# taindp98/Endoscopy-Image-Classification

Hardware: AMD Instinct MI355X
Metric: unlabeled images/sec/node (FixMatch ViT-S, 224², μ=7) (higher is better)
Workload: dtype bf16; 1 GPU; F1: FixMatch ViT-S/16 step, global B=64 labeled + mu*B=448 unlabeled weak/strong pairs (64 + 448 per GPU, strong scaling), 224^2, C=23, tau=0.95, lambda_u=1, Adam 1e-3, EMA 0.999; global_batch=960, seq_len=197, parallelism=dp1, hipgraph=False

## Files before the change

endoscopy-image-classification_amd/csrc/attention.hip:

```cpp
#include <type_traits>

#include "common.h"

namespace {

struct AttnArgs {
  const bf16* qkv; bf16* o; float* lse; float* delta;
  const bf16* dout; bf16* dqkv;
  int ldqkv, ldo, lddo, lddqkv;
  int T, H;
  float scale;
};

__device__ __forceinline__ int aswz(int r, int c) { return c ^ (((r >> 1) & 3) << 1); }

template <int NW = 4>
__device__ __forceinline__ void stage_head(char* lds, const bf16* src, int ld, int T, int TP) {
  const int lane = threadIdx.x & 63, w = threadIdx.x >> 6;
  for (int i = w; i < TP / 8; i += NW) {
    const int row = i * 8 + (lane >> 3);
    const int sr = row < T ? row : T - 1;
    glds16(src + (size_t)sr * ld + aswz(row, lane & 7) * 8, lds + i * 1024);
  }
}
// ... 1276 lines not shown
      bf16x4 tk4[NDT];
#pragma unroll
      for (int dt = 0; dt < NDT; ++dt) tk4[dt] = lds_trT4(Ks, t * 16, (d0 + dt) * 16, g, r);
      const bf16x4 dsf = lds_trS4(img, t * 16, seg, half, g, r);
#pragma unroll
      for (int dt = 0; dt < NDT; ++dt) dq[dt] = mfma16k16(tk4[dt], dsf, dq[dt]);
    }
    const int img_i = bh / a.H, h = bh - img_i * a.H, q0 = tile * 16;
    bf16* dst = a.dqkv + ((size_t)img_i * T + q0) * a.lddqkv + h * 64 + d0 * 16;
    if constexpr (NDT == 4) tile_rows_out(slot, dq, a.scale, dst, a.lddqkv, T - q0);
    else half_rows_out(slot, dq, a.scale, dst, a.lddqkv, T - q0);
  };
  using Whole = std::integral_constant<int, 4>;
  using Half = std::integral_constant<int, 2>;

  int bh = blockIdx.x;
  stage_qdo(bh, 0, NG, 0, 8);
  stage_k(bh);
  Pre pre = prefetch(bh);
  const int nk = (NG - w + 7) / 8;
  for (;;) {
    const int img = bh / a.H, h = bh - img * a.H;
    const int nx = bh + gridDim.x;
    const bool more = nx < nbh;
    if (nk == 4) asm volatile("s_waitcnt vmcnt(4)" ::: "memory");
    else asm volatile("s_waitcnt vmcnt(3)" ::: "memory");
    lds_barrier();
    deltas(pre);
    __builtin_amdgcn_s_waitcnt(0x0F70);
    lds_barrier();
    f32x4 dk[2][4], dv[2][4];
#pragma unroll
    for (int t = 0; t < 2; ++t)
#pragma unroll
      for (int dt = 0; dt < 4; ++dt) dk[t][dt] = dv[t][dt] = f32x4{0.f, 0.f, 0.f, 0.f};
    bf16x8 kv[8];
    {
      const int l = fresh_lane(), g = l >> 4, r = l & 15;
#pragma unroll
      for (int t = 0; t < 2; ++t) {
        const int key = w * 32 + 16 * t + r;
        const bf16x8 k0 = lds_row8(Ks, key < TP ? key : 0, g), k1 = lds_row8(Ks, key < TP ? key : 0, 4 + g);
        kv[4 * t + 0] = key < T ? k0 : zero8;
        kv[4 * t + 1] = key < T ? k1 : zero8;
        kv[4 * t + 2] = pre.v[2 * t];
        kv[4 * t + 3] = pre.v[2 * t + 1];
      }
    }
    if (w < (NT16 + 1) / 2) phase1(kv, dk, dv, 0, PA, false, 0);
    lds_barrier();
    if (more) stage_qdo(nx, 0, PA * 32 / 8, 0, 8);
    phase2(Whole{}, bh, w, 0, 0);
    lds_barrier();
    if (w < (NT16 + 1) / 2) phase1(kv, dk, dv, PA, NP, true, 2 * PA * 16);
    lds_barrier();
    if (more) stage_qdo(nx, PA * 32 / 8, NG, 0, 8);
    pre = prefetch(more ? nx : bh);
    static_assert(2 * (NT16 - 2 * PA) == 10, "ten half tiles");
    if (w < 7) {
      phase2(Half{}, bh, 2 * PA + (w >> 1), w & 1, 2 * PA * 16);
    } else {
      phase2(Half{}, bh, 2 * PA + 3, 1, 2 * PA * 16);
      phase2(Half{}, bh, 2 * PA + 4, 0, 2 * PA * 16);
      phase2(Half{}, bh, 2 * PA + 4, 1, 2 * PA * 16);
    }
    if (w < (NT16 + 1) / 2) {
      bf16* d0 = a.dqkv + ((size_t)img * T + w * 32) * a.lddqkv + D + h * 64;
      tile_rows_out(slot, dk[0], a.scale, d0, a.lddqkv, T - w * 32);
      tile_rows_out(slot, dv[0], 1.0f, d0 + D, a.lddqkv, T - w * 32);
      tile_rows_out(slot, dk[1], a.scale, d0 + 16 * (size_t)a.lddqkv, a.lddqkv, T - w * 32 - 16);
      tile_rows_out(slot, dv[1], 1.0f, d0 + 16 * (size_t)a.lddqkv + D, a.lddqkv, T - w * 32 - 16);
    }
    lds_barrier();
    if (!more) break;
    stage_k(nx);
    bh = nx;
  }
}

constexpr int CLS_KMAX = 32;
constexpr int CLS_KMAX_LONG = 80;

__device__ __forceinline__ float grp8_sum(float v) {
  v += __shfl_xor(v, 1, 64);
  v += __shfl_xor(v, 2, 64);
  v += __shfl_xor(v, 4, 64);
  return v;
}

__device__ __forceinline__ void ld8f(const bf16* p, float* f) {
  const bf16x8 v = *(const bf16x8*)p;
#pragma unroll
  for (int i = 0; i < 8; ++i) f[i] = (float)v[i];
}

template <int KMAX>
__global__ __launch_bounds__(64) void attn_cls_fwd_kernel(const bf16* __restrict__ qkv, int ldqkv, bf16* __restrict__ o,
                                                          int ldo, float* __restrict__ lse, int T, int H, float scale) {
  const int bh = blockIdx.x, img = bh / H, h = bh - img * H, D = H * 64;
  const int lane = threadIdx.x, c = lane & 7, jg = lane >> 3;
  const bf16* base = qkv + (size_t)img * T * ldqkv;
  float q[8];
  ld8f(base + h * 64 + 8 * c, q);
  const float sl = scale * 1.44269504088896341f;
  float s[KMAX];
  float mx = -INFINITY;
#pragma unroll
  for (int it = 0; it < KMAX; ++it) {
    const int j = it * 8 + jg;
    float part = 0.f;
    if (j < T) {
      float k[8];
      ld8f(base + (size_t)j * ldqkv + D + h * 64 + 8 * c, k);
#pragma unroll
      for (int i = 0; i < 8; ++i) part = fmaf(q[i], k[i], part);
    }
    const float dot = grp8_sum(part);
    s[it] = j < T ? dot * sl : -INFINITY;
    mx = fmaxf(mx, s[it]);
  }
  mx = fmaxf(mx, __shfl_xor(mx, 8, 64));
  mx = fmaxf(mx, __shfl_xor(mx, 16, 64));
  mx = fmaxf(mx, __shfl_xor(mx, 32, 64));
  float l = 0.f, acc[8] = {0.f, 0.f, 0.f, 0.f, 0.f, 0.f, 0.f, 0.f};
#pragma unroll
  for (int it = 0; it < KMAX; ++it) {
    const int j = it * 8 + jg;
    if (j < T) {
      const float p = __builtin_amdgcn_exp2f(s[it] - mx);
      l += p;
      const float pb = (float)(bf16)p;
      float v[8];
      ld8f(base + (size_t)j * ldqkv + 2 * D + h * 64 + 8 * c, v);
#pragma unroll
      for (int i = 0; i < 8; ++i) acc[i] = fmaf(pb, v[i], acc[i]);
    }
  }
#pragma unroll
  for (int m = 8; m < 64; m <<= 1) {
    l += __shfl_xor(l, m, 64);
#pragma unroll
    for (int i = 0; i < 8; ++i) acc[i] += __shfl_xor(acc[i], m, 64);
  }
  if (jg == 0) {
    const float inv = 1.0f / l;
    bf16x8 ov;
#pragma unroll
    for (int i = 0; i < 8; ++i) ov[i] = (bf16)(acc[i] * inv);
    *(bf16x8*)(o + (size_t)img * ldo + h * 64 + 8 * c) = ov;
    if (c == 0) lse[bh] = (mx + __log2f(l)) * 0.69314718055994531f;
  }
}

template <int KMAX>
__global__ __launch_bounds__(64) void attn_cls_bwd_kernel(const bf16* __restrict__ qkv, int ldqkv,
                                                          const bf16* __restrict__ o, int ldo,
                                                          const float* __restrict__ lse,
                                                          const bf16* __restrict__ dout, int lddo,
                                                          bf16* __restrict__ dqkv, int lddqkv, int T, int H,
                                                          float scale) {
  const int bh = blockIdx.x, img = bh / H, h = bh - img * H, D = H * 64;
  const int lane = threadIdx.x, c = lane & 7, jg = lane >> 3;
  const bf16* base = qkv + (size_t)img * T * ldqkv;
  bf16* dbase = dqkv + (size_t)img * T * lddqkv;
  float q[8], dq_o[8], ov[8];
  ld8f(base + h * 64 + 8 * c, q);
  ld8f(dout + (size_t)img * lddo + h * 64 + 8 * c, dq_o);
  ld8f(o + (size_t)img * ldo + h * 64 + 8 * c, ov);
  float dpart = 0.f;
#pragma unroll
  for (int i = 0; i < 8; ++i) dpart += dq_o[i] * ov[i];
  const float delta = grp8_sum(dpart);
  const float sl = scale * 1.44269504088896341f;
  const float lq = lse[bh] * 1.44269504088896341f;
  float dqa[8] = {0.f, 0.f, 0.f, 0.f, 0.f, 0.f, 0.f, 0.f};
  const bf16x8 zero8 = {};
  for (int it = 0; it < KMAX; ++it) {
    const int j = it * 8 + jg;
    if (it * 8 >= T) break;
    float k[8], v[8];
    float sp = 0.f, dpp = 0.f;
    if (j < T) {
      ld8f(base + (size_t)j * ldqkv + D + h * 64 + 8 * c, k);
      ld8f(base + (size_t)j * ldqkv + 2 * D + h * 64 + 8 * c, v);
#pragma unroll
      for (int i = 0; i < 8; ++i) {
        sp = fmaf(q[i], k[i], sp);
        dpp = fmaf(dq_o[i], v[i], dpp);
      }
    }
    const float sv = grp8_sum(sp), dp = grp8_sum(dpp);
    if (j < T) {
      const float p = __builtin_amdgcn_exp2f(sv * sl - lq);
      const float ds = p * (dp - delta);
      const float pb = (float)(bf16)p, dsb = (float)(bf16)ds;
      bf16x8 dk8, dv8;
#pragma unroll
      for (int i = 0; i < 8; ++i) {
        dk8[i] = (bf16)(dsb * q[i] * scale);
        dv8[i] = (bf16)(pb * dq_o[i]);
        dqa[i] = fmaf(dsb, k[i], dqa[i]);
      }
      bf16* drow = dbase + (size_t)j * lddqkv + h * 64 + 8 * c;
      *(bf16x8*)(drow + D) = dk8;
      *(bf16x8*)(drow + 2 * D) = dv8;
      if (j > 0) *(bf16x8*)drow = zero8;
    }
  }
#pragma unroll
  for (int m = 8; m < 64; m <<= 1)
#pragma unroll
    for (int i = 0; i < 8; ++i) dqa[i] += __shfl_xor(dqa[i], m, 64);
  if (jg == 0) {
    bf16x8 d8;
#pragma unroll
    for (int i = 0; i < 8; ++i) d8[i] = (bf16)(dqa[i] * scale);
    *(bf16x8*)(dbase + h * 64 + 8 * c) = d8;
  }
}

#define ATTN_CASE(KERNEL, N_, GRID, LDS, STREAM, ARGS) \
  case N_: allow_lds(KERNEL<N_>, LDS); hipLaunchKernelGGL(KERNEL<N_>, GRID, 256, LDS, STREAM, ARGS); break;

#define ATTN_DISPATCH(KERNEL, NT16_, GRID, LDS, STREAM, ARGS)                                               \
  switch (NT16_) {                                                                                        \
    ATTN_CASE(KERNEL, 1, GRID, LDS, STREAM, ARGS) ATTN_CASE(KERNEL, 2, GRID, LDS, STREAM, ARGS)            \
    ATTN_CASE(KERNEL, 3, GRID, LDS, STREAM, ARGS) ATTN_CASE(KERNEL, 4, GRID, LDS, STREAM, ARGS)            \
    ATTN_CASE(KERNEL, 5, GRID, LDS, STREAM, ARGS) ATTN_CASE(KERNEL, 6, GRID, LDS, STREAM, ARGS)            \
    ATTN_CASE(KERNEL, 7, GRID, LDS, STREAM, ARGS) ATTN_CASE(KERNEL, 8, GRID, LDS, STREAM, ARGS)            \
    ATTN_CASE(KERNEL, 9, GRID, LDS, STREAM, ARGS) ATTN_CASE(KERNEL, 10, GRID, LDS, STREAM, ARGS)           \
    ATTN_CASE(KERNEL, 11, GRID, LDS, STREAM, ARGS) ATTN_CASE(KERNEL, 12, GRID, LDS, STREAM, ARGS)          \
    ATTN_CASE(KERNEL, 13, GRID, LDS, STREAM, ARGS) ATTN_CASE(KERNEL, 14, GRID, LDS, STREAM, ARGS)          \
    ATTN_CASE(KERNEL, 15, GRID, LDS, STREAM, ARGS) ATTN_CASE(KERNEL, 16, GRID, LDS, STREAM, ARGS)          \
    ATTN_CASE(KERNEL, 37, GRID, LDS, STREAM, ARGS)                                                        \
    default: return ES_BAD_SHAPE;                                                                         \
  }

#define FWD_CASE(N_, OCC_, GRID, LDS, STREAM, ARGS)                                                  \
  case N_:                                                                                          \
    allow_lds(attn_fwd_kernel<N_, OCC_>, LDS);                                                      \
    hipLaunchKernelGGL(HIP_KERNEL_NAME(attn_fwd_kernel<N_, OCC_>), GRID, 256, LDS, STREAM, ARGS);   \
    break;
#define FWD_DISPATCH(NT16_, OCC_, GRID, LDS, STREAM, ARGS)                                            \
  switch (NT16_) {                                                                                  \
    FWD_CASE(1, OCC_, GRID, LDS, STREAM, ARGS) FWD_CASE(2, OCC_, GRID, LDS, STREAM, ARGS)            \
    FWD_CASE(3, OCC_, GRID, LDS, STREAM, ARGS) FWD_CASE(4, OCC_, GRID, LDS, STREAM, ARGS)            \
    FWD_CASE(5, OCC_, GRID, LDS, STREAM, ARGS) FWD_CASE(6, OCC_, GRID, LDS, STREAM, ARGS)            \
    FWD_CASE(7, OCC_, GRID, LDS, STREAM, ARGS) FWD_CASE(8, OCC_, GRID, LDS, STREAM, ARGS)            \
    FWD_CASE(9, OCC_, GRID, LDS, STREAM, ARGS) FWD_CASE(10, OCC_, GRID, LDS, STREAM, ARGS)           \
    FWD_CASE(11, OCC_, GRID, LDS, STREAM, ARGS) FWD_CASE(12, OCC_, GRID, LDS, STREAM, ARGS)          \
    FWD_CASE(13, OCC_, GRID, LDS, STREAM, ARGS) FWD_CASE(14, OCC_, GRID, LDS, STREAM, ARGS)          \
    FWD_CASE(15, OCC_, GRID, LDS, STREAM, ARGS) FWD_CASE(16, OCC_, GRID, LDS, STREAM, ARGS)          \
    default: return ES_BAD_SHAPE;                                                                   \
  }

int g_attn_fwd_occ = 7;
int g_attn_bwd_pipe = 4;
int g_attn_bwd_long = 1;
int g_attn_bwd_grid = -1;

}

extern "C" {

int es_set_attn_variant(int occ) {
  const int old = g_attn_fwd_occ;
  g_attn_fwd_occ = occ;
  return old;
}

int es_set_attn_bwd_variant(int v) {
  if (v < 0 || v > 4) return ES_BAD_ARG;
  const int old = g_attn_bwd_pipe;
  g_attn_bwd_pipe = v;
  return old;
}

int es_set_attn_bwd_grid(int workgroups) {
  const int old = g_attn_bwd_grid;
  g_attn_bwd_grid = workgroups < -1 ? -1 : workgroups;
  return old;
}

int es_set_attn_bwd_long(int v) {
  const int old = g_attn_bwd_long;
  g_attn_bwd_long = v;
  return old;
}


static int attn_tiles(int T) { return T <= 256 ? (T + 15) / 16 : 37; }
constexpr int ATTN_TMAX = 592;

int es_attn_fwd(const void* qkv, int ldqkv, void* o, int ldo, float* lse, int nimg, int T, int H, float scale,
                hipStream_t stream) {
  if (nimg <= 0 || T <= 0 || T > ATTN_TMAX || H <= 0 || ldqkv < 3 * H * 64 || ldo < H * 64 || (ldqkv % 8) ||
      (ldo % 8))
    return ES_BAD_SHAPE;
  if (!qkv || !o || !lse) return ES_BAD_ARG;
  AttnArgs a{(const bf16*)qkv, (bf16*)o, lse, nullptr, nullptr, nullptr, ldqkv, ldo, 0, 0, T, H, scale};
  if (T > 256) {
    const size_t lds = 2 * (size_t)37 * 16 * 128 + 8 * 1024;
    allow_lds(attn_fwd_long_kernel<37>, lds);
    hipLaunchKernelGGL(HIP_KERNEL_NAME(attn_fwd_long_kernel<37>), nimg * H, 512, lds, stream, a);
    return hipGetLastError() == hipSuccess ? ES_OK : ES_HIP_ERROR;
  }
  const int nt16 = (T + 15) / 16;
  const size_t lds = 3 * (size_t)nt16 * 16 * 128;
  if (g_attn_fwd_occ == 7 && nt16 == 13) {
    allow_lds(attn_fwd_kernel<13, 2, 7>, lds);
    hipLaunchKernelGGL(HIP_KERNEL_NAME(attn_fwd_kernel<13, 2, 7>), nimg * H, 448, lds, stream, a);
  } else if (g_attn_fwd_occ == 2 || g_attn_fwd_occ == 7) {
    FWD_DISPATCH(nt16, 2, nimg * H, lds, stream, a);
  } else {
    FWD_DISPATCH(nt16, 3, nimg * H, lds, stream, a);
  }
  return hipGetLastError() == hipSuccess ? ES_OK : ES_HIP_ERROR;
}

int es_attn_bwd(const void* qkv, int ldqkv, const void* o, int ldo, const float* lse, float* delta, const void* dout,
                int lddo, void* dqkv, int lddqkv, int nimg, int T, int H, float scale, hipStream_t stream) {
  if (nimg <= 0 || T <= 0 || T > ATTN_TMAX || H <= 0 || ldqkv < 3 * H * 64 || lddqkv < 3 * H * 64 || (ldqkv % 8) ||
      (lddqkv % 8) || (ldo % 8) || (lddo % 8))
    return ES_BAD_SHAPE;
  if (!qkv || !o || !lse || !delta || !dout || !dqkv) return ES_BAD_ARG;
  AttnArgs a{(const bf16*)qkv, (bf16*)o, (float*)lse, delta, (const bf16*)dout, (bf16*)dqkv, ldqkv, ldo, lddo,
             lddqkv, T, H, scale};
  const int nt16 = attn_tiles(T);
  const size_t lds_dq = 2 * (size_t)nt16 * 16 * 128;
  const size_t lds_dkv = lds_dq + 2 * (size_t)nt16 * 16 * 4;
  const int nw_dq = nt16 == 37 ? 8 : 4, nw_dkv = nt16 == 37 ? 6 : 4;
  const size_t slots_dq = nw_dq * (nw_dq == 4 ? 2048 : 1024), slots_dkv = nw_dkv * (nt16 <= 16 ? 2048 : 1024);
#define BWD_VARIANTS(N_)                                                                                    \
  if (g_attn_bwd_pipe >= 3) {                                                                               \
    if (nw_dq == 8) {                                                                                       \
      allow_lds(attn_bwd_dq2_kernel<N_, 8>, lds_dq + slots_dq);                                             \
      hipLaunchKernelGGL(HIP_KERNEL_NAME(attn_bwd_dq2_kernel<N_, 8>), nimg * H, 512, lds_dq + slots_dq, stream, a); \
    } else {                                                                                                \
      allow_lds(attn_bwd_dq2_kernel<N_>, lds_dq + slots_dq);                                                \
      hipLaunchKernelGGL(HIP_KERNEL_NAME(attn_bwd_dq2_kernel<N_>), nimg * H, 256, lds_dq + slots_dq, stream, a); \
    }                                                                                                       \
  } else {                                                                                                  \
    allow_lds(attn_bwd_dq_pipe_kernel<N_>, lds_dq);                                                         \
    hipLaunchKernelGGL(HIP_KERNEL_NAME(attn_bwd_dq_pipe_kernel<N_>), nimg * H, 256, lds_dq, stream, a);     \
  }                                                                                                         \
  if (g_attn_bwd_pipe >= 2) {                                                                               \
    if (nw_dkv == 6) {                                                                                      \
      allow_lds(attn_bwd_dkv2_kernel<N_, false, 6>, lds_dkv + slots_dkv);                                   \
      hipLaunchKernelGGL(HIP_KERNEL_NAME(attn_bwd_dkv2_kernel<N_, false, 6>), nimg * H, 384, lds_dkv + slots_dkv, \
                         stream, a);                                                                        \
    } else {                                                                                                \
      allow_lds(attn_bwd_dkv2_kernel<N_>, lds_dkv + slots_dkv);                                             \
      hipLaunchKernelGGL(HIP_KERNEL_NAME(attn_bwd_dkv2_kernel<N_>), nimg * H, 256, lds_dkv + slots_dkv, stream, a); \
    }                                                                                                       \
  } else {                                                                                                  \
    allow_lds(attn_bwd_dkv_pipe_kernel<N_>, lds_dkv);                                                       \
    hipLaunchKernelGGL(HIP_KERNEL_NAME(attn_bwd_dkv_pipe_kernel<N_>), nimg * H, 256, lds_dkv, stream, a);   \
  }                                                                                                         \
  return hipGetLastError() == hipSuccess ? ES_OK : ES_HIP_ERROR;
  if (g_attn_bwd_pipe == 4 && nt16 == 13 &&
      (size_t)nimg * T * std::max(std::max(ldqkv, ldo), lddo) * 2 < ((size_t)1 << 31)) {
    static int cus = 0;
    if (!cus) {
      int dev = 0;
      (void)hipGetDevice(&dev);
      if (hipDeviceGetAttribute(&cus, hipDeviceAttributeMultiprocessorCount, dev) != hipSuccess || cus <= 0) cus = 256;
    }
    const size_t lds = 5 * (size_t)13 * 16 * 128 + 2 * 13 * 16 * 4 + 8 * 2048;
    allow_lds(attn_bwd_fused_kernel<13>, lds);
    const int heads = nimg * H;
    const int grid = std::min(g_attn_bwd_grid > 0 ? g_attn_bwd_grid
                                                  : (g_attn_bwd_grid == 0 ? cus : std::max(cus, (heads + 3) / 4)),
                              heads);
    hipLaunchKernelGGL(HIP_KERNEL_NAME(attn_bwd_fused_kernel<13>), grid, 512, lds, stream, a, nimg * H);
    return hipGetLastError() == hipSuccess ? ES_OK : ES_HIP_ERROR;
  }
  if (g_attn_bwd_pipe && nt16 == 13) { BWD_VARIANTS(13) }
  if (g_attn_bwd_pipe && nt16 == 37 && g_attn_bwd_long) { BWD_VARIANTS(37) }
#undef BWD_VARIANTS
  ATTN_DISPATCH(attn_bwd_dq_kernel, nt16, nimg * H, lds_dq, stream, a);
  ATTN_DISPATCH(attn_bwd_dkv_kernel, nt16, nimg * H, lds_dkv, stream, a);
  return hipGetLastError() == hipSuccess ? ES_OK : ES_HIP_ERROR;
}


int es_attn_cls_fwd(const void* qkv, int ldqkv, void* o, int ldo, float* lse, int nimg, int T, int H, float scale,
                    hipStream_t stream) {
  if (nimg <= 0 || T <= 0 || T > 8 * CLS_KMAX_LONG || H <= 0 || ldqkv < 3 * H * 64 || ldo < H * 64 || (ldqkv % 8) ||
      (ldo % 8))
    return ES_BAD_SHAPE;
  if (!qkv || !o || !lse) return ES_BAD_ARG;
  if (T <= 8 * CLS_KMAX)
    hipLaunchKernelGGL(HIP_KERNEL_NAME(attn_cls_fwd_kernel<CLS_KMAX>), nimg * H, 64, 0, stream, (const bf16*)qkv, ldqkv,
                       (bf16*)o, ldo, lse, T, H, scale);
  else
    hipLaunchKernelGGL(HIP_KERNEL_NAME(attn_cls_fwd_kernel<CLS_KMAX_LONG>), nimg * H, 64, 0, stream, (const bf16*)qkv,
                       ldqkv, (bf16*)o, ldo, lse, T, H, scale);
  return hipGetLastError() == hipSuccess ? ES_OK : ES_HIP_ERROR;
}

int es_attn_cls_bwd(const void* qkv, int ldqkv, const void* o, int ldo, const float* lse, const void* dout, int lddo,
                    void* dqkv, int lddqkv, int nimg, int T, int H, float scale, hipStream_t stream) {
  if (nimg <= 0 || T <= 0 || T > 8 * CLS_KMAX_LONG || H <= 0 || ldqkv < 3 * H * 64 || lddqkv < 3 * H * 64 ||
      ldo < H * 64 || lddo < H * 64 || (ldqkv % 8) || (lddqkv % 8) || (ldo % 8) || (lddo % 8))
    return ES_BAD_SHAPE;
  if (!qkv || !o || !lse || !dout || !dqkv) return ES_BAD_ARG;
  if (T <= 8 * CLS_KMAX)
    hipLaunchKernelGGL(HIP_KERNEL_NAME(attn_cls_bwd_kernel<CLS_KMAX>), nimg * H, 64, 0, stream, (const bf16*)qkv, ldqkv,
                       (const bf16*)o, ldo, lse, (const bf16*)dout, lddo, (bf16*)dqkv, lddqkv, T, H, scale);
  else
    hipLaunchKernelGGL(HIP_KERNEL_NAME(attn_cls_bwd_kernel<CLS_KMAX_LONG>), nimg * H, 64, 0, stream, (const bf16*)qkv,
                       ldqkv, (const bf16*)o, ldo, lse, (const bf16*)dout, lddo, (bf16*)dqkv, lddqkv, T, H, scale);
  return hipGetLastError() == hipSuccess ? ES_OK : ES_HIP_ERROR;
}

}
```

endoscopy-image-classification_amd/csrc/gemm.hip:

```cpp
#include <algorithm>
#include <mutex>
#include <type_traits>

#include <hip/hip_ext.h>

#include "common.h"

namespace es_gemm {

constexpr int BM = 128, BN = 128, BK = 64;

enum Epi {
  EPI_BF16 = 0,
  EPI_GELU = 1,
  EPI_F32_RESID = 2,
  EPI_DGELU = 3,
  EPI_F32 = 4,
  EPI_PATCH = 5,
  EPI_GELU_ACT = 6,
  EPI_GELU_D = 7,
  EPI_MULAUX = 8,
};

struct NTArgs {
// ... 1400 lines not shown
        for (int j = 0; j < 3; ++j) {
          const int cc = (j * 64 + lane) >> 1;
          const float2 t = *(const float2*)(smem + lr * ROWX + ((cc ^ (lr & 15)) << 4) + (lane & 1) * 8);
          const float2 rr = rv[2 * s + q / (RPS / 2)][q % (RPS / 2)][j];
          v[j] = make_float2(t.x + rr.x, t.y + rr.y);
        }
        if constexpr (s == 0)
          if (q == RPS / 2 - 1) load_resid(std::integral_constant<int, 3>{});
        const LnRow384 o = ln_row384(v, (q & 1) == 0, l.eps, gam_lds, bet_lds, lane);
        const int m = m0 + tile_row(s, q);
        const bool ok = m < p.M;
#pragma unroll
        for (int j = 0; j < 3; ++j) {
          const int c = (j * 64 + lane) * 2;
          __builtin_amdgcn_raw_buffer_store_b64(__builtin_bit_cast(u32x2, v[j]), rx,
                                                ok ? (unsigned)(m * p.ldc + c) * 4u : ES_OOB, 0, 0);
          __builtin_amdgcn_raw_buffer_store_b32(o.h[j], rh, ok ? (unsigned)(m * l.ldh + c) * 2u : ES_OOB, 0, 0);
        }
        const bool one = ok && lane == 0;
        __builtin_amdgcn_raw_buffer_store_b32(__builtin_bit_cast(unsigned, o.mean), rm,
                                              one ? (unsigned)m * 4u : ES_OOB, 0, 0);
        __builtin_amdgcn_raw_buffer_store_b32(__builtin_bit_cast(unsigned, o.rstd), rs,
                                              one ? (unsigned)m * 4u : ES_OOB, 0, 0);
      }
    };
    slab(std::integral_constant<int, 0>{});
    asm volatile("s_waitcnt lgkmcnt(0)" ::: "memory");
    __builtin_amdgcn_s_barrier();
    slab(std::integral_constant<int, 1>{});
    if (tid == 0) qslot[0] = claimed;
    asm volatile("s_waitcnt lgkmcnt(0)" ::: "memory");
    __builtin_amdgcn_s_barrier();
    cur = __builtin_amdgcn_readfirstlane(qslot[0]);
  }
  TILE_CTR_RELEASE(ctr, tid)
}
#undef TILE_CTR_RELEASE

#define NT_LAUNCH(E, BKT_, NST_, TBM_, ...)                                             \
  {                                                                                        \
    const size_t lds = std::max((size_t)NST_ * (TBM_ + BN) * BKT_ * 2, (size_t)4 * EPI_WAVE_BYTES); \
    allow_lds(gemm_nt_kernel<E, BKT_, NST_, TBM_, ##__VA_ARGS__>, lds);                   \
    hipLaunchKernelGGL(HIP_KERNEL_NAME(gemm_nt_kernel<E, BKT_, NST_, TBM_, ##__VA_ARGS__>), dim3(grid), dim3(256), lds, stream, a); \
    return ES_OK;                                                                          \
  }
#define NT_EPIS(BKT_, NST_, TBM_, ...)                                            \
  switch (epi) {                                                                  \
    case EPI_BF16: NT_LAUNCH(EPI_BF16, BKT_, NST_, TBM_, ##__VA_ARGS__)           \
    case EPI_GELU: NT_LAUNCH(EPI_GELU, BKT_, NST_, TBM_, ##__VA_ARGS__)           \
    case EPI_F32_RESID: NT_LAUNCH(EPI_F32_RESID, BKT_, NST_, TBM_, ##__VA_ARGS__) \
    case EPI_DGELU: NT_LAUNCH(EPI_DGELU, BKT_, NST_, TBM_, ##__VA_ARGS__)         \
    case EPI_F32: NT_LAUNCH(EPI_F32, BKT_, NST_, TBM_, ##__VA_ARGS__)             \
    case EPI_PATCH: NT_LAUNCH(EPI_PATCH, BKT_, NST_, TBM_, ##__VA_ARGS__)         \
    case EPI_GELU_ACT: NT_LAUNCH(EPI_GELU_ACT, BKT_, NST_, TBM_, ##__VA_ARGS__)   \
    case EPI_GELU_D: NT_LAUNCH(EPI_GELU_D, BKT_, NST_, TBM_, ##__VA_ARGS__)       \
    case EPI_MULAUX: NT_LAUNCH(EPI_MULAUX, BKT_, NST_, TBM_, ##__VA_ARGS__)       \
    default: return ES_BAD_ARG;                                                   \
  }
int launch_nt(int cfg, int epi, int grid, hipStream_t stream, const NTArgs& a) {
  if (cfg == 11 && epi == EPI_F32_RESID) NT_LAUNCH(EPI_F32_RESID, 64, 2, 64, 0)
  switch (cfg) {
    case 0: NT_EPIS(64, 2, 128)
    case 5: NT_EPIS(32, 2, 128)
    case 11: NT_EPIS(64, 2, 64)
    default: NT_EPIS(32, 3, 128)
  }
}
#undef NT_EPIS
#undef NT_LAUNCH

#define BIG_LAUNCH(E, WM_, MF_, NF_, NST_, BKT_, OCC_, ...)                                        \
  {                                                                                                 \
    const size_t lds = (size_t)NST_ * (WM_ * MF_ * 16 + (8 / WM_) * NF_ * 16) * BKT_ * 2;            \
    allow_lds(gemm_nt_big_kernel<E, WM_, MF_, NF_, NST_, BKT_, OCC_, ##__VA_ARGS__>, lds);          \
    hipLaunchKernelGGL(HIP_KERNEL_NAME(gemm_nt_big_kernel<E, WM_, MF_, NF_, NST_, BKT_, OCC_, ##__VA_ARGS__>), dim3(grid), \
                       dim3(512), lds, stream, a);                                                  \
    return hipGetLastError() == hipSuccess ? ES_OK : ES_HIP_ERROR;                                  \
  }
#define BIG_EPIS2(WM_, MF_, NF_, NST_, BKT_, OCC_)                                        \
  switch (epi) {                                                                          \
    case EPI_BF16: BIG_LAUNCH(EPI_BF16, WM_, MF_, NF_, NST_, BKT_, OCC_)                  \
    case EPI_GELU: BIG_LAUNCH(EPI_GELU, WM_, MF_, NF_, NST_, BKT_, OCC_)                  \
    case EPI_F32_RESID: BIG_LAUNCH(EPI_F32_RESID, WM_, MF_, NF_, NST_, BKT_, OCC_)        \
    case EPI_DGELU: BIG_LAUNCH(EPI_DGELU, WM_, MF_, NF_, NST_, BKT_, OCC_)                \
    case EPI_F32: BIG_LAUNCH(EPI_F32, WM_, MF_, NF_, NST_, BKT_, OCC_)                    \
    case EPI_PATCH: BIG_LAUNCH(EPI_PATCH, WM_, MF_, NF_, NST_, BKT_, OCC_)                \
    case EPI_GELU_ACT: BIG_LAUNCH(EPI_GELU_ACT, WM_, MF_, NF_, NST_, BKT_, OCC_)          \
    case EPI_GELU_D: BIG_LAUNCH(EPI_GELU_D, WM_, MF_, NF_, NST_, BKT_, OCC_)              \
    case EPI_MULAUX: BIG_LAUNCH(EPI_MULAUX, WM_, MF_, NF_, NST_, BKT_, OCC_)              \
    default: return ES_BAD_ARG;                                                           \
  }
#define BIG_EPIS(WM_, MF_, NF_, NST_, BKT_) BIG_EPIS2(WM_, MF_, NF_, NST_, BKT_, 1)
int launch_big(int cfg, int epi, int grid, hipStream_t stream, const NTArgs& a) {
  if (cfg == 10 && epi == EPI_F32_RESID) BIG_LAUNCH(EPI_F32_RESID, 4, 4, 4, 3, 32, 4, 0)
  switch (cfg) {
    case 10: BIG_EPIS2(4, 4, 4, 3, 32, 4)
    default: BIG_EPIS(2, 8, 4, 2, 64)
  }
}
#undef BIG_EPIS
#undef BIG_EPIS2
#undef BIG_LAUNCH

static int tile_ctr_slot(hipStream_t s) {
  static std::mutex mu;
  static hipStream_t tab[CTR_SLOTS];
  static int n = 0;
  std::lock_guard<std::mutex> lock(mu);
  for (int i = 0; i < n; ++i)
    if (tab[i] == s) return i;
  if (n < CTR_SLOTS) {
    tab[n] = s;
    return n++;
  }
  return (int)(((uintptr_t)s >> 6) % CTR_SLOTS);
}
static int persistent_grid(int tiles) {
  static const int cus = [] {
    int dev = 0, n = 0;
    (void)hipGetDevice(&dev);
    return (hipDeviceGetAttribute(&n, hipDeviceAttributeMultiprocessorCount, dev) != hipSuccess || n <= 0) ? 256 : n;
  }();
  return std::max(1, std::min(cus, tiles));
}

int launch_resid_ln(hipStream_t stream, const NTArgs& a, const RLArgs& l) {
  const int grid = persistent_grid((a.M + rlg::R - 1) / rlg::R);
  allow_lds(gemm_resid_ln_kernel, (size_t)rlg::LDS);
  hipLaunchKernelGGL(gemm_resid_ln_kernel, dim3(grid), dim3(512), rlg::LDS, stream, a, l, tile_ctr_slot(stream));
  return hipGetLastError() == hipSuccess ? ES_OK : ES_HIP_ERROR;
}

int launch_nt_ln(int ring, hipStream_t stream, const NTArgs& a, const RLArgs& l) {
  const int grid = persistent_grid((a.M + nlg::TBM - 1) / nlg::TBM);
  const int slot = tile_ctr_slot(stream);
  constexpr size_t lds3 = nlg::lds<3, 32>(), lds2 = nlg::lds<2, 64>();
  if (ring == 1) {
    allow_lds(gemm_nt_ln_kernel<3, 32>, lds3);
    hipLaunchKernelGGL(HIP_KERNEL_NAME(gemm_nt_ln_kernel<3, 32>), dim3(grid), dim3(512), lds3, stream, a, l, slot);
  } else {
    allow_lds(gemm_nt_ln_kernel<2, 64>, lds2);
    hipLaunchKernelGGL(HIP_KERNEL_NAME(gemm_nt_ln_kernel<2, 64>), dim3(grid), dim3(512), lds2, stream, a, l, slot);
  }
  return hipGetLastError() == hipSuccess ? ES_OK : ES_HIP_ERROR;
}

}
using namespace es_gemm;

static int g_gemm_variant = -1;
static int g_tn_variant = -1;
static int g_small_tile = 1;

extern "C" {

int es_gemm_tn_ex(const void* A1, int ld1, const void* A2, int ld2, int M, int N1, int N2, int splits,
                  float* workspace, float* out, int accumulate, float* bias_out, int variant, hipStream_t stream);

int es_gemm_nt(int epi, const void* A, int lda, const void* B, int ldb, const float* bias, void* C,
               int ldc, void* C2, const void* aux, int ldaux, int M, int N, int K, int np,
               hipStream_t stream) {
  if (M <= 0 || N <= 0 || K <= 0 || (N % BN) || (K % BK) || (lda % 8) || (ldb % 8) || (ldc % 4))
    return ES_BAD_SHAPE;
  if (!A || !B || !C) return ES_BAD_ARG;
  if (((epi == EPI_GELU || epi == EPI_GELU_D) && !C2) ||
      ((epi == EPI_F32_RESID || epi == EPI_DGELU || epi == EPI_MULAUX || epi == EPI_PATCH) && !aux))
    return ES_BAD_ARG;
  if (epi == EPI_PATCH && np <= 0) return ES_BAD_ARG;
  if ((epi == EPI_F32_RESID || epi == EPI_PATCH) && ((ldaux % 4) || ldaux < N)) return ES_BAD_SHAPE;
  if ((epi == EPI_DGELU || epi == EPI_MULAUX) && ((ldaux % 8) || ldaux < N)) return ES_BAD_SHAPE;
  NTArgs a{(const bf16*)A, (const bf16*)B, bias, C, C2, aux, M, N, K, lda, ldb, ldc, ldaux, np};
  int variant = g_gemm_variant;
  if (variant < 0) {
    const bool gelu = epi == EPI_GELU || epi == EPI_GELU_ACT || epi == EPI_GELU_D;
    const bool plain = epi == EPI_BF16 || epi == EPI_F32 || epi == EPI_F32_RESID || epi == EPI_MULAUX;
    if (g_small_tile && N <= 384 && ((K <= 384 && epi == EPI_F32_RESID) || (M < 32768 && (plain || epi == EPI_GELU_ACT))))
      variant = 11;
    else if (g_small_tile && M < 32768 && epi == EPI_GELU_ACT)
      variant = 11;
    else if (M >= 65536 && K >= 768 && N == 384 && epi == EPI_BF16)
      variant = 0;
    else if ((plain || epi == EPI_GELU_D) && M >= 65536 && ((K <= 384 && N >= 384) || (K >= 768 && N == 384)))
      variant = 10;
    else if (K <= 384 && N % 256 == 0 && epi == EPI_MULAUX)
      variant = M < 65536 ? 0 : 6;
    else if (K >= 768 && N % 256 == 0 && epi != EPI_DGELU)
      variant = 6;
    else if (epi == EPI_PATCH)
      variant = 0;
    else if (gelu)
      variant = K <= 384 ? 5 : 1;
    else if (K <= 384)
      variant = (epi == EPI_F32_RESID || N <= 384 || M < 65536) ? 0 : (epi == EPI_DGELU ? 2 : 5);
    else
      variant = M < 65536 ? 0 : 1;
  }
  if (variant == 1) {
    const int grid = ((M + BM2 - 1) / BM2) * (N / BN);
    const size_t lds = 3 * STAGE2;
#define L2(E) allow_lds(gemm_nt256_kernel<E>, lds); hipLaunchKernelGGL(gemm_nt256_kernel<E>, grid, 512, lds, stream, a); break;
    switch (epi) {
      case EPI_BF16: L2(EPI_BF16)
      case EPI_GELU: L2(EPI_GELU)
      case EPI_F32_RESID: L2(EPI_F32_RESID)
      case EPI_DGELU: L2(EPI_DGELU)
      case EPI_F32: L2(EPI_F32)
      case EPI_PATCH: L2(EPI_PATCH)
      case EPI_GELU_ACT: L2(EPI_GELU_ACT)
      case EPI_GELU_D: L2(EPI_GELU_D)
      case EPI_MULAUX: L2(EPI_MULAUX)
      default: return ES_BAD_ARG;
    }
#undef L2
    return hipGetLastError() == hipSuccess ? ES_OK : ES_HIP_ERROR;
  }
  if (variant == 6 || variant == 10) {
    const int tbn = variant == 6 ? 256 : 128;
    if (N % tbn) return ES_BAD_SHAPE;
    return launch_big(variant, epi, ((M + 255) / 256) * (N / tbn), stream, a);
  }
  if (variant != 0 && variant != 2 && variant != 5 && variant != 11) return ES_BAD_ARG;
  const int tbm = variant == 11 ? 64 : BM;
  const int grid = ((M + tbm - 1) / tbm) * (N / BN);
  const int rc = launch_nt(variant, epi, grid, stream, a);
  if (rc) return rc;
  return hipGetLastError() == hipSuccess ? ES_OK : ES_HIP_ERROR;
}

int es_gemm_nt_resid_ln(const void* A, int lda, const void* B, int ldb, const float* bias, float* C, int ldc,
                        const float* aux, int ldaux, const float* gamma, const float* beta, void* h, int ldh,
                        float* mean, float* rstd, int M, int N, int K, float eps, hipStream_t stream) {
  if (M <= 0 || N != rlg::D || K != rlg::KD || (lda % 8) || (ldb % 8) || (ldc % 2) || (ldaux % 4) || (ldh % 2) ||
      (size_t)M * (size_t)std::max(ldc, ldaux) * 4 >= (1u << 31))
    return ES_BAD_SHAPE;
  if (!A || !B || !C || !aux || !gamma || !beta || !h || !mean || !rstd) return ES_BAD_ARG;
  if ((((uintptr_t)A | (uintptr_t)aux | (uintptr_t)B | (uintptr_t)gamma | (uintptr_t)beta) & 15) ||
      (bias && ((uintptr_t)bias & 15)) || ((uintptr_t)C & 7) || ((uintptr_t)h & 3))
    return ES_BAD_ARG;
  NTArgs a{(const bf16*)A, (const bf16*)B, bias, C, nullptr, aux, M, N, K, lda, ldb, ldc, ldaux, 0};
  RLArgs l{gamma, beta, (bf16*)h, mean, rstd, ldh, eps};
  return launch_resid_ln(stream, a, l);
}

static int g_nt_ln_ring = 0;
int es_gemm_nt_ln(const void* A, int lda, const void* B, int ldb, const float* bias, float* C, int ldc,
                  const float* aux, int ldaux, const float* gamma, const float* beta, void* h, int ldh, float* mean,
                  float* rstd, int M, int N, int K, float eps, hipStream_t stream) {
  if (M <= 0 || N != nlg::D || K <= 0 || (K % 64) || (lda % 8) || (ldb % 8) || (ldc % 2) || (ldaux % 2) || (ldh % 2) ||
      lda < K || ldb < K || ldc < N || ldaux < N || ldh < N ||
      (size_t)M * (size_t)std::max(std::max(ldc, ldaux), ldh) * 4 >= (1u << 31))
    return ES_BAD_SHAPE;
  if (!A || !B || !C || !aux || !gamma || !beta || !h || !mean || !rstd) return ES_BAD_ARG;
  if ((((uintptr_t)A | (uintptr_t)B | (uintptr_t)gamma | (uintptr_t)beta) & 15) || (bias && ((uintptr_t)bias & 15)) ||
      (((uintptr_t)C | (uintptr_t)aux) & 7) || (((uintptr_t)h | (uintptr_t)mean | (uintptr_t)rstd) & 3))
    return ES_BAD_ARG;
  NTArgs a{(const bf16*)A, (const bf16*)B, bias, C, nullptr, aux, M, N, K, lda, ldb, ldc, ldaux, 0};
  RLArgs l{gamma, beta, (bf16*)h, mean, rstd, ldh, eps};
  return launch_nt_ln(g_nt_ln_ring, stream, a, l);
}
int endossl_nt_ln_ring(int v) {
  const int old = g_nt_ln_ring;
  g_nt_ln_ring = v == 1 ? 1 : 0;
  return old;
}

static bool gemm_variant_ok(int v) {
  return v == -1 || v == 0 || v == 1 || v == 2 || v == 5 || v == 6 || v == 10 || v == 11;
}
int es_set_gemm_variant(int v) {
  if (!gemm_variant_ok(v)) return ES_BAD_ARG;
  const int old = g_gemm_variant;
  g_gemm_variant = v;
  return old;
}

int es_set_gemm_small_tile(int v) {
  const int old = g_small_tile;
  g_small_tile = v;
  return old;
}

int es_set_tn_variant(int v) {
  if (v != -1 && v != 0 && v != 7) return ES_BAD_ARG;
  const int old = g_tn_variant;
  g_tn_variant = v;
  return old;
}

constexpr int TN_MIN_SPLIT_TOKENS = 512;
static bool tn_big_ok(int N1, int N2, int ld1, int ld2) {
  return N1 % TB1 == 0 && N2 % TB2 == 0 && ld1 % 8 == 0 && ld2 % 8 == 0;
}
static int tn_pick(int M, int N1, int N2, int ld1, int ld2, int v) {
  if (!(N1 % BM == 0 && N2 % BN == 0)) return 7;
  if (v == 7) return tn_big_ok(N1, N2, ld1, ld2) ? 7 : 0;
  if (v >= 0) return 0;
  return (tn_big_ok(N1, N2, ld1, ld2) && M >= 65536) ? 7 : 0;
}
static int tn_target(int v) { return v == 7 ? 256 : 768; }
static int tn_tiles(int v, int N1, int N2) { return v == 7 ? (N1 / TB1) * (N2 / TB2) : (N1 / BM) * (N2 / BN); }
static int tn_auto_splits(int v, int M, int N1, int N2) {
  const int by_fill = std::max(1, tn_target(v) / tn_tiles(v, N1, N2));
  const int by_len = std::max(1, M / TN_MIN_SPLIT_TOKENS);
  return std::min(by_fill, by_len);
}

size_t es_gemm_tn_workspace(int N1, int N2, int splits) {
  if (splits <= 0) {
    splits = std::max(1, 768 / std::max(1, (N1 / BM) * (N2 / BN)));
    if (N1 % TB1 == 0 && N2 % TB2 == 0) splits = std::max(splits, 512 / std::max(1, (N1 / TB1) * (N2 / TB2)));
  }
  return (size_t)splits * N1 * N2 + (size_t)splits * N1;
}

int es_gemm_tn(const void* A1, int ld1, const void* A2, int ld2, int M, int N1, int N2, int splits,
               float* workspace, float* out, int accumulate, float* bias_out, hipStream_t stream) {
  return es_gemm_tn_ex(A1, ld1, A2, ld2, M, N1, N2, splits, workspace, out, accumulate, bias_out, -1, stream);
}

int es_gemm_tn_ex(const void* A1, int ld1, const void* A2, int ld2, int M, int N1, int N2, int splits,
                  float* workspace, float* out, int accumulate, float* bias_out, int variant, hipStream_t stream) {
  if (M <= 0 || (ld1 % 8) || (ld2 % 8)) return ES_BAD_SHAPE;
  if (!tn_big_ok(N1, N2, ld1, ld2) && ((N1 % BM) || (N2 % BN))) return ES_BAD_SHAPE;
  if (!A1 || !A2 || !out || !workspace) return ES_BAD_ARG;
  if (variant != -1 && variant != 0 && variant != 7) return ES_BAD_ARG;
  const int v = tn_pick(M, N1, N2, ld1, ld2, g_tn_variant >= 0 ? g_tn_variant : variant);
  const int BKM = v == 7 ? 64 : 32;
  const int msteps = (M + BKM - 1) / BKM;
  if (splits <= 0) splits = tn_auto_splits(v, M, N1, N2);
  splits = std::min(splits, msteps);
  const int per = (msteps + splits - 1) / splits;
  const int S = (msteps + per - 1) / per;
  const bool direct = (S == 1 && !accumulate);
  float* P = direct ? out : workspace;
  float* PB = bias_out ? workspace + (size_t)S * N1 * N2 : nullptr;
  TNArgs a{(const bf16*)A1, (const bf16*)A2, P, PB, M, N1, N2, ld1, ld2, per * BKM};
  const int grid = S * tn_tiles(v, N1, N2);
#define TN_LAUNCH(BKM_, NST_)                                                                           \
  {                                                                                                   \
    const size_t lds = (size_t)NST_ * 2 * BKM_ * BM * 2;                                              \
    allow_lds(gemm_tn_kernel<BKM_, NST_>, lds);                                                       \
    hipLaunchKernelGGL(HIP_KERNEL_NAME(gemm_tn_kernel<BKM_, NST_>), dim3(grid), dim3(256), lds, stream, a); \
  }
#define TNB_LAUNCH(BKM_, NST_)                                                                          \
  {                                                                                                   \
    const size_t lds = (size_t)NST_ * BKM_ * (TB1 + TB2) * 2;                                         \
    allow_lds(gemm_tn_big_kernel<BKM_, NST_>, lds);                                                   \
    hipLaunchKernelGGL(HIP_KERNEL_NAME(gemm_tn_big_kernel<BKM_, NST_>), dim3(grid), dim3(512), lds, stream, a); \
  }
  switch (v) {
    case 7: TNB_LAUNCH(64, 2) break;
    default: TN_LAUNCH(32, 2) break;
  }
#undef TN_LAUNCH
#undef TNB_LAUNCH
  if (!direct) {
    const int n = N1 * N2;
    int rg = (n / 4 + 255) / 256;
    rg = rg > 2048 ? 2048 : rg;
    hipLaunchKernelGGL(splitk_reduce_kernel, rg, 256, 0, stream, P, out, S, n, accumulate);
  }
  if (bias_out)
    launch_reduce_partials(PB, bias_out, S, N1, accumulate, stream);
  return hipGetLastError() == hipSuccess ? ES_OK : ES_HIP_ERROR;
}

static_assert(sizeof(TNGroupEntry) == 64, "es_tn_problem layout");
size_t es_tn_problem_size(void) { return sizeof(TNGroupEntry); }

int es_gemm_tn_grouped_prepare(void* host_table, int count) {
  if (!host_table || count <= 0) return ES_BAD_ARG;
  TNGroupEntry* t = (TNGroupEntry*)host_table;
  int tiles = 0;
  for (int i = 0; i < count; ++i) {
    TNArgs& a = t[i].a;
    if (!a.A1 || !a.A2 || !a.P) return ES_BAD_ARG;
    if (a.M <= 0 || a.N1 % BM || a.N2 % BN || a.ld1 % 8 || a.ld2 % 8) return ES_BAD_SHAPE;
    a.mchunk = (a.M + 31) / 32 * 32;
    t[i].tile0 = tiles;
// ... 178 lines not shown
```

endoscopy-image-classification_amd/csrc/losses.hip:

```cpp
#include "common.h"

namespace {

constexpr int MAXC = 64;

__device__ __forceinline__ float block_sum(float v, float* red) {
  v = warp_sum(v);
  const int lane = threadIdx.x & 63, w = threadIdx.x >> 6;
  __syncthreads();
  if (lane == 0) red[w] = v;
  __syncthreads();
  float s = 0.f;
  for (int i = 0; i < (int)(blockDim.x >> 6); ++i) s += red[i];
  return s;
}

__global__ __launch_bounds__(256) void fm_consistency_kernel(const float* __restrict__ lw, int ldw,
                                                             const float* __restrict__ ls, int lds_, int n, int C,
                                                             float tau, float grad_scale, int* __restrict__ pl,
                                                             uint8_t* __restrict__ mask_out,
                                                             float* __restrict__ row_loss, float* __restrict__ dls,
                                                             int lddls, float* __restrict__ out) {
  __shared__ float red[16];
  float sum_loss = 0.f, sum_mask = 0.f;
  for (int i = threadIdx.x; i < n; i += blockDim.x) {
    const float* wr = lw + (size_t)i * ldw;
    const float* sr = ls + (size_t)i * lds_;
    float mx = -INFINITY;
    for (int c = 0; c < C; ++c) mx = fmaxf(mx, wr[c]);
    float se = 0.f;
    for (int c = 0; c < C; ++c) se += __expf(wr[c] - mx);
    const float inv = 1.0f / se;
    float pmax = -1.f;
    int idx = 0;
    for (int c = 0; c < C; ++c) {
      const float p = __expf(wr[c] - mx) * inv;
      if (p > pmax) {
        pmax = p;
        idx = c;
      }
    }
    const float m = pmax >= tau ? 1.f : 0.f;
    float mxs = -INFINITY;
    for (int c = 0; c < C; ++c) mxs = fmaxf(mxs, sr[c]);
    float ses = 0.f;
    for (int c = 0; c < C; ++c) ses += __expf(sr[c] - mxs);
    const float lse = mxs + __logf(ses);
    const float ce = lse - sr[idx];
    const float rl = ce * m;
    const float invs = 1.0f / ses;
    for (int c = 0; c < C; ++c) {
      const float p = __expf(sr[c] - mxs) * invs;
      dls[(size_t)i * lddls + c] = m * (p - (c == idx ? 1.f : 0.f)) * grad_scale;
    }
    if (pl) pl[i] = idx;
    if (mask_out) mask_out[i] = (uint8_t)m;
    if (row_loss) row_loss[i] = rl;
    sum_loss += rl;
    sum_mask += m;
  }
  sum_loss = block_sum(sum_loss, red);
  sum_mask = block_sum(sum_mask, red);
  if (threadIdx.x == 0) {
    out[0] = sum_loss / (float)n;
    out[1] = sum_mask / (float)n;
  }
}

__global__ __launch_bounds__(256) void poly_ce_kernel(const float* __restrict__ l, int ldl,
                                                      const int64_t* __restrict__ y, const float* __restrict__ w,
                                                      int n, int C, float eps, float grad_scale,
                                                      float* __restrict__ dl, int lddl, float* __restrict__ out) {
  __shared__ float red[16];
  float sum = 0.f;
  for (int i = threadIdx.x; i < n; i += blockDim.x) {
    const float* lr = l + (size_t)i * ldl;
    float mx = -INFINITY;
    for (int c = 0; c < C; ++c) mx = fmaxf(mx, lr[c]);
    float se = 0.f;
    for (int c = 0; c < C; ++c) se += __expf(lr[c] - mx);
    const float lse = mx + __logf(se);
    const int yi = (int)y[i];
    if ((unsigned)yi >= (unsigned)C) {
      sum += __int_as_float(0x7fc00000);
      for (int c = 0; c < C; ++c) dl[(size_t)i * lddl + c] = 0.f;
      continue;
    }
    const float wy = w ? w[yi] : 1.f;
    const float py = __expf(lr[yi] - lse);
    sum += wy * (lse - lr[yi]) + eps * (1.f - py);
    const float coef = grad_scale * (wy + eps * py);
    for (int c = 0; c < C; ++c) {
      const float p = __expf(lr[c] - lse);
      dl[(size_t)i * lddl + c] = coef * (p - (c == yi ? 1.f : 0.f));
    }
  }
  sum = block_sum(sum, red);
  if (threadIdx.x == 0) out[0] = sum / (float)n;
}

__global__ __launch_bounds__(256) void ce_weighted_kernel(const float* __restrict__ l, int ldl,
                                                          const int64_t* __restrict__ y, const float* __restrict__ w,
                                                          const float* __restrict__ wsum_global, int n, int C,
                                                          float grad_scale, float* __restrict__ dl, int lddl,
                                                          float* __restrict__ out) {
  __shared__ float red[16];
  float ws = 0.f;
  for (int i = threadIdx.x; i < n; i += blockDim.x) {
    const int yi = (int)y[i];
    ws += (unsigned)yi >= (unsigned)C ? __int_as_float(0x7fc00000) : (w ? w[yi] : 1.f);
  }
  float W = block_sum(ws, red);
  __syncthreads();
  if (wsum_global) W = *wsum_global;
  const float invW = 1.0f / W;
  float sum = 0.f;
  for (int i = threadIdx.x; i < n; i += blockDim.x) {
    const float* lr = l + (size_t)i * ldl;
    float mx = -INFINITY;
    for (int c = 0; c < C; ++c) mx = fmaxf(mx, lr[c]);
    float se = 0.f;
    for (int c = 0; c < C; ++c) se += __expf(lr[c] - mx);
    const float lse = mx + __logf(se);
    const int yi = (int)y[i];
    if ((unsigned)yi >= (unsigned)C) {
      for (int c = 0; c < C; ++c) dl[(size_t)i * lddl + c] = 0.f;
      continue;
    }
    const float wy = w ? w[yi] : 1.f;
    sum += wy * (lse - lr[yi]);
    const float coef = grad_scale * wy * invW;
    for (int c = 0; c < C; ++c) {
      const float p = __expf(lr[c] - lse);
      dl[(size_t)i * lddl + c] = coef * (p - (c == yi ? 1.f : 0.f));
    }
  }
  sum = block_sum(sum, red);
  if (threadIdx.x == 0) out[0] = sum * invW;
}

__global__ __launch_bounds__(256) void ce_weight_sum_kernel(const int64_t* __restrict__ y, const float* __restrict__ w,
                                                            int n, int C, float* __restrict__ out) {
  __shared__ float red[16];
  float ws = 0.f;
  for (int i = threadIdx.x; i < n; i += blockDim.x) {
    const int yi = (int)y[i];
    ws += (unsigned)yi >= (unsigned)C ? __int_as_float(0x7fc00000) : (w ? w[yi] : 1.f);
  }
  ws = block_sum(ws, red);
  if (threadIdx.x == 0) out[0] = ws;
}

constexpr int TRIPLET_THREADS = 1024;

__global__ __launch_bounds__(TRIPLET_THREADS) void triplet_kernel(const float* __restrict__ z, int ldz, int bs, int L,
                                                                  float alpha, float grad_scale,
                                                                  float* __restrict__ dz, int lddz,
                                                                  float* __restrict__ out) {
  __shared__ float red[16];
  const int lane = threadIdx.x & 63, w = threadIdx.x >> 6, nw = blockDim.x >> 6;
  float s_h = 0.f, s_p = 0.f, s_n = 0.f, s_act = 0.f;
  for (int i = w; i < bs; i += nw) {
    const float* za = z + (size_t)i * ldz;
    const float* zp = z + (size_t)(bs + i) * ldz;
    const float* zn = z + (size_t)(2 * bs + i) * ldz;
    float sp = 0.f, sn = 0.f;
    for (int k = lane; k < L; k += 64) {
      const float a = za[k], ep = a - zp[k], en = a - zn[k];
      sp = fmaf(ep, ep, sp);
      sn = fmaf(en, en, sn);
    }
    const float dp = sqrtf(warp_sum(sp)), dn = sqrtf(warp_sum(sn));
    const float h = dp - dn + alpha;
    const bool act = h > 0.f;
    s_h += act ? h : 0.f;
    s_p += dp;
    s_n += dn;
    s_act += act ? 1.f : 0.f;
    const float cp = act && dp > 0.f ? grad_scale / dp : 0.f;
    const float cn = act && dn > 0.f ? grad_scale / dn : 0.f;
    float* ga = dz + (size_t)i * lddz;
    float* gp = dz + (size_t)(bs + i) * lddz;
    float* gn = dz + (size_t)(2 * bs + i) * lddz;
    for (int k = lane; k < L; k += 64) {
      const float a = za[k], up = (a - zp[k]) * cp, un = (a - zn[k]) * cn;
      ga[k] = up - un;
      gp[k] = -up;
      gn[k] = un;
    }
  }
  const float inv = 1.0f / (float)bs;
  s_h = block_sum(lane == 0 ? s_h : 0.f, red);
  s_p = block_sum(lane == 0 ? s_p : 0.f, red);
  s_n = block_sum(lane == 0 ? s_n : 0.f, red);
  s_act = block_sum(lane == 0 ? s_act : 0.f, red);
  if (threadIdx.x == 0) {
    out[0] = s_h * inv;
    out[1] = s_p * inv;
    out[2] = s_n * inv;
    out[3] = s_act * inv;
  }
}

__global__ __launch_bounds__(256) void softmax_predict_kernel(const float* __restrict__ l, int ldl, int n, int C,
                                                              float thres, int* __restrict__ pred,
                                                              float* __restrict__ conf, int* __restrict__ label) {
  const int stride = gridDim.x * blockDim.x;
  for (int i = blockIdx.x * blockDim.x + threadIdx.x; i < n; i += stride) {
    const float* lr = l + (size_t)i * ldl;
    float mx = lr[0];
    int idx = 0;
    for (int c = 1; c < C; ++c) {
      const float v = lr[c];
      if (v > mx) {
        mx = v;
        idx = c;
      }
    }
    float se = 0.f;
    for (int c = 0; c < C; ++c) se += __expf(lr[c] - mx);
    const float p = 1.0f / se;
    if (pred) pred[i] = idx;
    if (conf) conf[i] = p;
    if (label) label[i] = p > thres ? idx : 0;
  }
}

constexpr int MARGIN_THREADS = 256;
constexpr int MARGIN_MAXF = 2048;
enum { MARGIN_COSFACE = 0, MARGIN_ARCFACE = 1, MARGIN_SPHEREFACE = 2, MARGIN_ACLOSS = 3 };

struct MarginParams {
  int kind;
  float s, m, eps, lo, hi;
  float cos_m, sin_m;
  float sig1, inv_k;
  float grad_scale;
};

__device__ __forceinline__ void margin_numerator(const MarginParams& P, float t, float& num, float& dnum) {
  if (P.kind == MARGIN_COSFACE) {
    num = P.s * (t - P.m);
    dnum = P.s;
    return;
  }
  const bool inside = t >= P.lo && t <= P.hi;
  const float tc = fminf(fmaxf(t, P.lo), P.hi);
  const float om = inside ? 1.0f - tc : (t > P.hi ? P.eps : 2.0f - P.eps);
  const float op = inside ? 1.0f + tc : (t > P.hi ? 2.0f - P.eps : P.eps);
  const float sq = sqrtf(om * op);
  float d;
// ... 26 lines not shown
  for (int k = tid; k < F4; k += MARGIN_THREADS) {
    const f32x4 v = xr[k];
    ss += v[0] * v[0] + v[1] * v[1] + v[2] * v[2] + v[3] * v[3];
  }
  const float nrm = sqrtf(block_sum(ss, red));
  const float inv = 1.0f / fmaxf(nrm, 1e-12f);
  for (int k = tid; k < F4; k += MARGIN_THREADS) ((f32x4*)xs)[k] = xr[k] * inv;
  __syncthreads();
  for (int c = w; c < C; c += MARGIN_THREADS / 64) {
    const f32x4* wr = (const f32x4*)(W + (size_t)c * F);
    float acc = 0.f;
    for (int k = lane; k < F4; k += 64) {
      const f32x4 a = ((const f32x4*)xs)[k], q = wr[k];
      acc = fmaf(a[0], q[0], acc);
      acc = fmaf(a[1], q[1], acc);
      acc = fmaf(a[2], q[2], acc);
      acc = fmaf(a[3], q[3], acc);
    }
    acc = warp_sum(acc);
    if (lane == 0) zs[c] = acc + (b ? b[c] : 0.f);
  }
  __syncthreads();
  if (w == 0) {
    const int64_t y64 = y[i];
    const bool valid = y64 >= 0 && y64 < C;
    const int yi = valid ? (int)y64 : -1;
    const float wm = (valid && cw ? cw[yi] : 1.f) * (mask ? mask[i] : 1.f);
    float num = 0.f, dnum = 0.f;
    margin_numerator(P, zs[valid ? yi : 0], num, dnum);
    const bool tgt = lane == yi;
    const float v = lane < C ? (tgt ? num : P.s * zs[lane]) : -INFINITY;
    const float mx = warp_max(v);
    const float e = lane < C ? expf(v - mx) : 0.f;
    const float se = warp_sum(e);
    const float rest = warp_sum(tgt ? 0.f : e);
    const float lse = mx + logf(se);
    const float coef = P.grad_scale * wm;
    float g = tgt ? -coef * (rest / se) * dnum : coef * P.s * (e / se);
    float rl = wm * (lse - num);
    if (!valid) {
      g = 0.f;
      rl = __int_as_float(0x7fc00000);
    }
    if (lane < C) {
      gs[lane] = g;
      G[(size_t)i * C + lane] = g;
    }
    if (lane == 0) {
      inv_norm[i] = inv;
      ws_loss[i] = rl;
      if (row_loss) row_loss[i] = rl;
    }
  }
  __syncthreads();
  f32x4 acc[2];
  float dot = 0.f;
#pragma unroll
  for (int j = 0; j < 2; ++j) {
    const int k = tid + j * MARGIN_THREADS;
    acc[j] = f32x4{0.f, 0.f, 0.f, 0.f};
    if (k < F4) {
      for (int c = 0; c < C; ++c) acc[j] += ((const f32x4*)(W + (size_t)c * F))[k] * gs[c];
      const f32x4 a = ((const f32x4*)xs)[k];
      dot += a[0] * acc[j][0] + a[1] * acc[j][1] + a[2] * acc[j][2] + a[3] * acc[j][3];
    }
  }
  dot = block_sum(dot, red);
  const float proj = nrm >= 1e-12f ? dot : 0.f;
  f32x4* dr = (f32x4*)(dx + (size_t)i * lddx);
#pragma unroll
  for (int j = 0; j < 2; ++j) {
    const int k = tid + j * MARGIN_THREADS;
    if (k < F4) dr[k] = (acc[j] - ((const f32x4*)xs)[k] * proj) * inv;
  }
}

__global__ __launch_bounds__(64) void margin_reduce_kernel(const float* __restrict__ x, int ldx,
                                                           const float* __restrict__ G,
                                                           const float* __restrict__ inv_norm,
                                                           const float* __restrict__ ws_loss, int n, int F, int C,
                                                           float grad_scale, float* __restrict__ dW,
                                                           float* __restrict__ db, float* __restrict__ out) {
  const int c = blockIdx.y, lane = threadIdx.x;
  const int F4 = F >> 2, k = blockIdx.x * 64 + lane;
  if (k < F4) {
    f32x4 acc = f32x4{0.f, 0.f, 0.f, 0.f};
#pragma unroll 4
    for (int i = 0; i < n; ++i)
      acc += ((const f32x4*)(x + (size_t)i * ldx))[k] * (G[(size_t)i * C + c] * inv_norm[i]);
    ((f32x4*)(dW + (size_t)c * F))[k] = acc;
  }
  if (blockIdx.x == 0) {
    if (db) {
      float sb = 0.f;
      for (int i = lane; i < n; i += 64) sb += G[(size_t)i * C + c];
      sb = warp_sum(sb);
      if (lane == 0) db[c] = sb;
    }
    if (c == 0) {
      float sl = 0.f;
      for (int i = lane; i < n; i += 64) sl += ws_loss[i];
      sl = warp_sum(sl);
      if (lane == 0) out[0] = grad_scale * sl;
    }
  }
}

}

extern "C" {

int es_ce_weighted_fwd_bwd(const float* logits, int ldl, const int64_t* targets, const float* weights, int n, int C,
                           float grad_scale, float* dlogits, int lddl, float* out, hipStream_t stream) {
  if (n <= 0 || C <= 0) return ES_BAD_SHAPE;
  if (!logits || !targets || !dlogits || !out) return ES_BAD_ARG;
  hipLaunchKernelGGL(ce_weighted_kernel, 1, 256, 0, stream, logits, ldl, targets, weights, nullptr, n, C, grad_scale,
                     dlogits, lddl, out);
  return hipGetLastError() == hipSuccess ? ES_OK : ES_HIP_ERROR;
}

int es_ce_weight_sum(const int64_t* targets, const float* weights, int n, int C, float* out, hipStream_t stream) {
  if (n <= 0 || C <= 0) return ES_BAD_SHAPE;
  if (!targets || !out) return ES_BAD_ARG;
  hipLaunchKernelGGL(ce_weight_sum_kernel, 1, 256, 0, stream, targets, weights, n, C, out);
  return hipGetLastError() == hipSuccess ? ES_OK : ES_HIP_ERROR;
}

int es_ce_weighted_fwd_bwd_global(const float* logits, int ldl, const int64_t* targets, const float* weights,
                                  const float* wsum_global, int n, int C, float grad_scale, float* dlogits, int lddl,
                                  float* out, hipStream_t stream) {
  if (n <= 0 || C <= 0) return ES_BAD_SHAPE;
  if (!logits || !targets || !dlogits || !out || !wsum_global) return ES_BAD_ARG;
  hipLaunchKernelGGL(ce_weighted_kernel, 1, 256, 0, stream, logits, ldl, targets, weights, wsum_global, n, C,
                     grad_scale, dlogits, lddl, out);
  return hipGetLastError() == hipSuccess ? ES_OK : ES_HIP_ERROR;
}

int es_fm_consistency_fwd_bwd(const float* logits_w, int ldw, const float* logits_s, int lds, int n, int C,
                              float tau, float grad_scale, int* pseudo_label, uint8_t* mask, float* row_loss,
                              float* dlogits_s, int lddls, float* out, hipStream_t stream) {
  if (n <= 0 || C <= 0 || C > MAXC) return ES_BAD_SHAPE;
  if (!logits_w || !logits_s || !dlogits_s || !out) return ES_BAD_ARG;
  hipLaunchKernelGGL(fm_consistency_kernel, 1, 256, 0, stream, logits_w, ldw, logits_s, lds, n, C, tau, grad_scale,
                     pseudo_label, mask, row_loss, dlogits_s, lddls, out);
  return hipGetLastError() == hipSuccess ? ES_OK : ES_HIP_ERROR;
}

int es_poly_ce_fwd_bwd(const float* logits, int ldl, const int64_t* targets, const float* weights, int n, int C,
                       float epsilon, float grad_scale, float* dlogits, int lddl, float* out, hipStream_t stream) {
  if (n <= 0 || C <= 0 || C > MAXC) return ES_BAD_SHAPE;
  if (!logits || !targets || !dlogits || !out) return ES_BAD_ARG;
  hipLaunchKernelGGL(poly_ce_kernel, 1, 256, 0, stream, logits, ldl, targets, weights, n, C, epsilon, grad_scale,
                     dlogits, lddl, out);
  return hipGetLastError() == hipSuccess ? ES_OK : ES_HIP_ERROR;
}

int es_triplet_fwd_bwd(const float* z, int ldz, int bs, int L, float alpha, float grad_scale, float* dz, int lddz,
                       float* out, hipStream_t stream) {
  if (bs < 1 || bs > 0x7fffffff / 3 || L < 1 || L > 2048 || ldz < L || lddz < L) return ES_BAD_SHAPE;
  if (!z || !dz || !out) return ES_BAD_ARG;
  hipLaunchKernelGGL(triplet_kernel, 1, TRIPLET_THREADS, 0, stream, z, ldz, bs, L, alpha, grad_scale, dz, lddz, out);
  return hipGetLastError() == hipSuccess ? ES_OK : ES_HIP_ERROR;
}

size_t es_margin_softmax_workspace(int n, int C) {
  if (n < 1 || C < 1 || C > MAXC) return 0;
  return (size_t)n * (size_t)(C + 2);
}

int es_margin_softmax_fwd_bwd(const float* x, int ldx, const float* W, const float* bias, const int64_t* targets,
                              const float* class_weights, const float* mask, int n, int F, int C, int kind, float s,
                              float m, float eps, float grad_scale, float* dx, int lddx, float* dW, float* db,
                              float* out, float* row_loss, float* workspace, hipStream_t stream) {
  if (n < 1 || C < 1 || C > MAXC || F < 4 || F > MARGIN_MAXF || (F & 3) || ldx < F || lddx < F || (ldx & 3) ||
      (lddx & 3))
    return ES_BAD_ARG;
  if (kind < MARGIN_COSFACE || kind > MARGIN_ACLOSS || !(eps > 0.f && eps < 1.f)) return ES_BAD_ARG;
  if (!x || !W || !targets || !dx || !dW || !out || !workspace) return ES_BAD_ARG;
  if (((uintptr_t)x | (uintptr_t)W | (uintptr_t)dx | (uintptr_t)dW) & 15) return ES_BAD_ARG;
  if (((uintptr_t)workspace | (uintptr_t)out) & 3) return ES_BAD_ARG;
  const double k = 0.3, q = exp(-M_PI / 2.0 / k);
  MarginParams P;
  P.kind = kind;
  P.s = s;
  P.m = m;
  P.eps = eps;
  P.lo = (float)(-1.0 + (double)eps);
  P.hi = (float)(1.0 - (double)eps);
  P.cos_m = (float)cos((double)m);
  P.sin_m = (float)sin((double)m);
  P.sig1 = (float)((1.0 + q) / (1.0 - q));
  P.inv_k = (float)(1.0 / k);
  P.grad_scale = grad_scale;
  float* G = workspace;
  float* inv_norm = G + (size_t)n * C;
  float* ws_loss = inv_norm + n;
  hipLaunchKernelGGL(margin_rows_kernel, n, MARGIN_THREADS, 0, stream, x, ldx, W, bias, targets, class_weights, mask,
                     F, C, P, dx, lddx, G, inv_norm, ws_loss, row_loss);
  hipLaunchKernelGGL(margin_reduce_kernel, dim3((F / 4 + 63) / 64, C), 64, 0, stream, x, ldx, G, inv_norm, ws_loss, n,
                     F, C, grad_scale, dW, db, out);
  return hipGetLastError() == hipSuccess ? ES_OK : ES_HIP_ERROR;
}

int es_softmax_predict(const float* logits, int ldl, int n, int C, float thres, int* pred, float* conf, int* label,
                       hipStream_t stream) {
  if (n <= 0 || C <= 0 || C > MAXC || ldl < C) return ES_BAD_SHAPE;
  if (!logits || (!pred && !conf && !label)) return ES_BAD_ARG;
  const int blocks = (n + 255) / 256 < 1024 ? (n + 255) / 256 : 1024;
  hipLaunchKernelGGL(softmax_predict_kernel, blocks, 256, 0, stream, logits, ldl, n, C, thres, pred, conf, label);
  return hipGetLastError() == hipSuccess ? ES_OK : ES_HIP_ERROR;
}

}
```

endoscopy-image-classification_amd/endossl/_lib.py:

```python
import ctypes
import os

import torch

_HERE = os.path.dirname(os.path.abspath(__file__))
LIB_PATH = os.environ.get("ENDOSSL_LIB", os.path.join(_HERE, "lib", "libendossl_hip.so"))

V, I, L, F, Z = ctypes.c_void_p, ctypes.c_int, ctypes.c_long, ctypes.c_float, ctypes.c_size_t
U64 = ctypes.c_ulonglong

SIGNATURES = {
    "es_abi_version": (I, []),
    "es_gemm_nt": (I, [I, V, I, V, I, V, V, I, V, V, I, I, I, I, I, V]),
    "es_gemm_nt_resid_ln": (I, [V, I, V, I, V, V, I, V, I, V, V, V, I, V, V, I, I, I, F, V]),
    "es_gemm_nt_ln": (I, [V, I, V, I, V, V, I, V, I, V, V, V, I, V, V, I, I, I, F, V]),
    "es_set_gemm_variant": (I, [I]),
    "es_set_gemm_small_tile": (I, [I]),
    "es_gemm_tn_workspace": (Z, [I, I, I]),
    "es_gemm_tn": (I, [V, I, V, I, I, I, I, I, V, V, I, V, V]),
    "es_gemm_tn_ex": (I, [V, I, V, I, I, I, I, I, V, V, I, V, I, V]),
    "es_set_tn_variant": (I, [I]),
    "es_set_attn_variant": (I, [I]),
    "es_set_attn_bwd_variant": (I, [I]),
    "es_set_attn_bwd_grid": (I, [I]),
    "es_set_ln_fwd_grid": (I, [I]),
    "es_set_attn_bwd_long": (I, [I]),
    "es_splitk_reduce": (I, [V, V, I, I, I, V]),
    "es_tn_problem_size": (Z, []),
    "es_gemm_tn_grouped_prepare": (I, [V, I]),
    "es_gemm_tn_grouped": (I, [V, I, I, V]),
    "es_set_stem_kernels": (I, [I]),
    "es_gemm_tn_big_grouped_table_bytes": (Z, [I]),
    "es_gemm_tn_big_grouped_workspace": (Z, [V, I, I]),
    "es_gemm_tn_big_grouped_prepare": (I, [V, I, I, V, Z, V, V]),
    "es_gemm_tn_big_grouped": (I, [V, I, V, V]),
    "es_gemm_tn_big_grouped_timed": (I, [V, I, V, V, V, V]),
    "es_event_create": (I, [V]),
    "es_event_elapsed": (I, [V, V, V]),
    "es_event_destroy": (I, [V]),
    "es_colsum": (I, [V, I, I, I, V, I, V, I, V]),
    "es_attn_fwd": (I, [V, I, V, I, V, I, I, I, F, V]),
    "es_attn_bwd": (I, [V, I, V, I, V, V, V, I, V, I, I, I, I, F, V]),
    "es_attn_cls_fwd": (I, [V, I, V, I, V, I, I, I, F, V]),
    "es_attn_cls_bwd": (I, [V, I, V, I, V, V, I, V, I, I, I, I, F, V]),
    "es_reduce_partials": (I, [V, V, I, I, I, V]),
    "es_layernorm_fwd": (I, [V, I, V, V, V, I, V, V, I, I, F, V]),
    "es_layernorm_bwd": (I, [V, I, V, I, V, V, V, V, I, V, I, V, I, V, V, V, I, I, I, I, V]),
    "es_layernorm_bwd_b16": (I, [V, I, V, I, V, V, V, V, I, V, I, V, I, V, V, V, I, I, I, I, V]),
    "es_layernorm_bwd_grid": (I, [I, I]),
    "es_ln_param_grads_entry_size": (I, []),
    "es_ln_param_grads_multi": (I, [V, I, V]),
    "es_gelu_fwd": (I, [V, V, L, V]),
    "es_gelu_bwd": (I, [V, V, V, L, V]),
    "es_patch_im2col": (I, [V, V, I, I, I, V]),
    "es_patch_im2col_u8": (I, [V, F, F, F, F, F, F, V, I, I, I, V]),
    "es_cls_init": (I, [V, I, V, V, I, I, I, V]),
    "es_embed_bwd": (I, [V, I, V, I, V, V, I, I, I, I, V]),
    "es_cls_head_fwd": (I, [V, I, I, V, V, V, V, V, I, V, V, I, I, I, F, V]),
    "es_cls_head_bwd": (I, [V, I, V, V, V, V, V, V, V, I, I, V, V, V, V, I, I, I, V]),
    "es_cls_head_bwd_ex": (I, [V, I, V, V, V, V, V, V, V, I, I, V, V, V, V, I, I, I, I, V]),
    "es_cls_ln_fwd": (I, [V, I, I, V, V, V, I, V, V, I, I, F, V]),
    "es_cls_ln_bwd": (I, [V, I, V, V, V, V, I, I, V, V, I, I, V]),
    "es_dense_fwd": (I, [V, I, V, V, V, I, I, I, I, I, F, V, F, V]),
    "es_dense_bwd_workspace": (Z, [I, I]),
    "es_dense_bwd": (I, [V, I, V, I, I, F, V, F, V, I, V, V, I, I, V, V, I, I, I, V, V]),
    "es_bn1d_fwd": (I, [V, I, V, V, V, V, V, F, F, I, V, I, V, V, I, I, V]),
    "es_bn1d_bwd": (I, [V, I, V, V, V, V, I, V, V, I, I, V]),
    "es_dropout_keep": (I, [V, L, F, U64, U64, V]),
    "es_bn1d_sums": (I, [V, I, I, I, V, F, V, V]),
    "es_bn1d_fwd_global": (I, [V, I, V, V, V, V, F, V, V, V, F, F, V, I, V, V, I, I, V]),
    "es_bn1d_bwd_sums": (I, [V, I, V, I, I, V, V]),
    "es_bn1d_bwd_global": (I, [V, I, V, V, V, V, V, F, V, I, V, V, I, I, V]),
    "es_l2norm_fwd": (I, [V, I, V, I, V, I, I, V]),
    "es_l2norm_bwd": (I, [V, I, V, I, V, V, I, I, I, V]),
    "es_comatch_pseudo_workspace": (Z, [I, I, I]),
    "es_comatch_pseudo": (I, [V, I, I, I, V, I, I, I, V, I, I, V, V, I, F, F, F, V, V, V, V, V, V]),
    "es_comatch_pseudo_ex": (I, [V, I, I, I, V, I, I, I, I, V, I, I, V, V, I, F, F, F, V, V, V, V, V, V]),
    "es_softmax_colmean": (I, [V, I, I, I, V, V]),
    "es_comatch_bank_write": (I, [V, I, I, V, I, I, I, V, V, I, V, V, I, I, V]),
    "es_comatch_contrastive_workspace": (Z, [I]),
    "es_comatch_contrastive_fwd_bwd": (I, [V, I, V, I, V, I, I, I, F, F, F, V, V, I, V, I, V, V]),
    "es_comatch_contrastive_ex_workspace": (Z, [I, I]),
    "es_comatch_contrastive_fwd_bwd_ex": (I, [V, I, V, I, V, V, I, I, I, I, I, F, F, F, F, V, V, I, V, I, V, V]),
    "es_comatch_focal_fwd_bwd": (I, [V, I, V, V, I, I, F, F, V, V, I, V, V]),
    "es_fm_consistency_fwd_bwd": (I, [V, I, V, I, I, I, F, F, V, V, V, V, I, V, V]),
    "es_poly_ce_fwd_bwd": (I, [V, I, V, V, I, I, F, F, V, I, V, V]),
    "es_triplet_fwd_bwd": (I, [V, I, I, I, F, F, V, I, V, V]),
    "es_softmax_predict": (I, [V, I, I, I, F, V, V, V, V]),
    "es_margin_softmax_workspace": (Z, [I, I]),
    "es_margin_softmax_fwd_bwd": (I, [V, I, V, V, V, V, V, I, I, I, I, F, F, F, F, V, I, V, V, V, V, V, V]),
    "es_ezbm_sample_mix": (I, [V, I, V, I, I, I, V, V, V, V, U64, U64, V, V, I, V, I, V, V, V, V, V, V]),
    "es_bn1d_groups_fwd": (I, [V, I, V, V, V, V, V, F, F, V, I, V, V, I, I, I, V]),
    "es_bn1d_groups_bwd": (I, [V, I, V, V, V, V, I, V, V, I, I, I, V]),
    "es_ezbm_ce_fwd_bwd": (I, [V, I, V, V, I, I, F, F, V, I, V, V]),
    "es_conv2d_fwd": (I, [V, I, I, I, I, L, L, L, L, V, V, I, I, I, I, I, V, L, L, L, I, V]),
    "es_conv2d_bwd_data": (I, [V, L, L, L, V, I, I, I, I, I, I, I, I, I, V, L, L, L, L, I, V]),
    "es_conv2d_dw_tiles": (I, [I, I, I, I]),
    "es_conv2d_bwd_weight_workspace": (Z, [I, I, I, I, I]),
    "es_conv2d_bwd_weight": (I, [V, I, I, I, I, L, L, L, L, V, L, L, L, I, I, I, I, I, I, V, V, I, V]),
    "es_conv2d_bf16_eligible": (I, [I, I, I, I]),
    "es_set_conv_dw_target": (I, [I]),
    "es_conv2d_pack_bf16": (I, [V, I, I, I, I, V, V, V]),
    "es_conv_pack_entry_size": (I, []),
    "es_set_conv_ring": (I, [I]),
    "es_set_conv_dw_buf": (I, [I]),
    "es_set_conv_small": (I, [I]),
    "es_conv2d_pack_bf16_multi": (I, [V, I, L, V]),
    "es_conv2d_fwd_bf16": (I, [V, I, I, I, I, L, L, L, L, V, V, I, I, I, I, I, V, L, L, L, I, V]),
    "es_conv2d_bwd_data_bf16": (I, [V, L, L, L, V, I, I, I, I, I, I, I, I, I, V, L, L, L, L, I, V]),
    "es_conv2d_bnstats_size": (Z, [I, I]),
    "es_conv2d_fwd_bf16_bnstats": (I, [V, I, I, I, I, L, L, L, L, V, V, I, I, I, I, I, V, L, L, L, V, V]),
    "es_bn2d_fwd_partials": (I, [V, I, I, V, V, V, V, V, V, F, F, V, I, V, V, V, V]),
    "es_conv2d_bwd_weight_bf16_workspace": (Z, [I, I, I, I, I, I]),
    "es_conv2d_bwd_weight_bf16": (I, [V, I, I, I, I, L, L, L, L, V, L, L, L, I, I, I, I, I, I, V, V, I, V]),
    "es_chan_workspace": (Z, [I, I]),
    "es_chan_sum": (I, [V, I, I, L, L, I, V, V, I, V]),
    "es_bn2d_fwd": (I, [V, I, I, V, V, V, V, V, F, F, I, V, I, V, V, V, V, V]),
    "es_bn2d_bwd": (I, [V, V, V, I, I, I, V, V, V, I, V, F, V, V, V, V, I, V, V]),
    "es_bn2d_sums": (I, [V, I, I, I, V, I, V, V, V]),
    "es_bn2d_fwd_global": (I, [V, I, I, V, V, V, V, V, F, F, V, V, I, V, I, V, V, V, V]),
    "es_bn2d_bwd_sums": (I, [V, V, V, I, I, I, V, V, V, V, V]),
    "es_bn2d_bwd_global": (I, [V, V, V, I, I, I, V, V, V, V, V, I, V, V, V, V, I, V]),
    "es_maxpool2d_fwd": (I, [V, I, I, I, I, I, I, I, V, V, V]),
    "es_maxpool2d_bwd": (I, [V, V, I, I, I, I, I, I, I, V, V]),
    "es_avgpool2d_fwd": (I, [V, I, I, I, I, I, V, V]),
    "es_avgpool2d_bwd": (I, [V, I, I, I, I, I, V, I, V]),
    "es_upsample_add_fwd": (I, [V, V, I, I, I, I, I, V, V]),
    "es_upsample_bwd": (I, [V, I, I, I, I, I, V, V]),
    "es_conv2d_fwd_bf16_ex": (I, [V, I, I, I, I, L, L, L, L, V, V, I, I, I, I, I, V, L, L, L, I, V, I, V]),
    "es_conv2d_bwd_data_bf16_ex": (I, [V, L, L, L, V, I, I, I, I, I, I, I, I, I, V, L, L, L, L, I, I, V]),
    "es_conv2d_bwd_weight_bf16_ex": (I, [V, I, I, I, I, L, L, L, L, V, L, L, L, I, I, I, I, I, I, V, V, I, I, V]),
    "es_conv2d_fwd_bf16_bnin_ex": (I, [V, I, I, I, I, L, L, L, L, V, V, I, I, I, I, I, V, L, L, L, I, V, I, V, V, V, V, V]),
    "es_conv2d_bwd_weight_bf16_bnin_ex": (I, [V, I, I, I, I, L, L, L, L, V, L, L, L, I, I, I, I, I, I, V, V, I, I,
                                             V, V, V, V, V]),
    "es_conv1x1_fwd_bf16_ex": (I, [V, I, I, V, V, I, V, I, V, I, V]),
    "es_conv1x1_fwd_bf16_bnin_ex": (I, [V, I, I, V, V, I, V, I, V, I, V, V, V, V, V]),
    "es_conv1x1_bwd_data_bf16_ex": (I, [V, I, I, V, I, V, I, I, V]),
    "es_set_conv_1x1": (I, [I]),
    "es_conv1x1_bf16_select": (I, [I, I, I, I]),
    "es_chan_sum_ex": (I, [V, I, I, L, L, I, V, V, I, I, V]),
    "es_set_bn_cs": (I, [I]),
    "es_set_bn_sum8": (I, [I]),
    "es_bn2d_fwd_ex": (I, [V, I, I, V, V, V, V, V, F, F, I, V, I, V, V, V, V, I, V]),
    "es_bn2d_bwd_ex": (I, [V, V, V, I, I, I, V, V, V, I, V, F, V, V, V, V, I, V, I, V]),
    "es_bn2d_bwd_recompute_ex": (I, [V, V, I, I, V, V, V, V, V, V, V, I, V, I, V]),
    "es_bn2d_fwd_partials_ex": (I, [V, I, I, V, V, V, V, V, V, F, F, V, I, V, V, V, I, V]),
    "es_bn2d_sums_ex": (I, [V, I, I, I, V, I, V, V, I, V]),
    "es_bn2d_fwd_global_ex": (I, [V, I, I, V, V, V, V, V, F, F, V, V, I, V, I, V, V, V, I, V]),
    "es_bn2d_bwd_sums_ex": (I, [V, V, V, I, I, I, V, V, V, V, I, V]),
    "es_bn2d_bwd_global_ex": (I, [V, V, V, I, I, I, V, V, V, V, V, I, V, V, V, V, I, I, V]),
    "es_maxpool2d_fwd_ex": (I, [V, I, I, I, I, I, I, I, V, V, I, V]),
    "es_maxpool2d_bwd_ex": (I, [V, V, I, I, I, I, I, I, I, V, I, V]),
    "es_avgpool2d_fwd_ex": (I, [V, I, I, I, I, I, V, I, V]),
    "es_avgpool2d_bwd_ex": (I, [V, I, I, I, I, I, V, I, I, V]),
    "es_upsample_add_fwd_ex": (I, [V, V, I, I, I, I, I, V, I, V]),
    "es_upsample_bwd_ex": (I, [V, I, I, I, I, I, V, I, V]),
    "es_fcu_down_tokens_fwd": (I, [V, V, V, V, V, V, V, I, I, I, F, V]),
    "es_fcu_down_workspace": (Z, [I, I, I]),
    "es_fcu_down_tokens_bwd": (I, [V, V, V, V, V, V, V, V, V, V, I, I, I, I, V, V]),
    "es_fcu_down_tokens_bwd_ex": (I, [V, V, V, V, V, V, V, V, V, V, I, I, I, I, V, I, V]),
    "es_tokens_cls_set": (I, [V, I, I, I, V, V]),
    "es_ce_weighted_fwd_bwd": (I, [V, I, V, V, I, I, F, V, I, V, V]),
    "es_ce_weight_sum": (I, [V, V, I, I, V, V]),
    "es_ce_weighted_fwd_bwd_global": (I, [V, I, V, V, V, I, I, F, V, I, V, V]),
    "es_se_bn_stats": (I, [V, V, I, I, F, F, I, V, V, V, V, V, V]),
    "es_se_squeeze_workspace": (Z, [I, I, I, I]),
    "es_se_bn_bwd_sums_workspace": (Z, [I, I, I, I]),
    "es_se_gate_bwd_workspace": (Z, [I, I, I]),
    "es_se_squeeze_ex": (I, [V, I, I, I, V, V, V, V, V, V, V, I, V]),
    "es_se_gate_fwd": (I, [V, V, V, I, I, I, V, V, V]),
    "es_se_bn_apply_ex": (I, [V, V, V, I, I, I, V, V, V, V, V, I, V]),
    "es_se_bn_bwd_sums_ex": (I, [V, V, V, I, I, I, V, V, V, V, V, I, V]),
    "es_se_gate_bwd": (I, [V, V, V, V, V, V, V, V, V, V, V, V, I, I, I, V, V, V, V, V, V, V]),
    "es_se_bn_bwd_dx_ex": (I, [V, V, V, V, V, I, I, I, V, V, V, V, V, I, V, V, I, I, V]),
    "es_adam_ema_step": (I, [V, V, V, V, V, L, F, F, F, F, F, F, F, F, V]),
    "es_adamw_ema_step": (I, [V, V, V, V, V, V, L, F, F, F, F, F, F, F, F, F, F, F, F, F, V]),
    "es_sgd_ema_step": (I, [V, V, V, V, V, L, F, F, F, F, F, I, F, F, F, V]),
    "es_ema_entry_size": (I, []),
    "es_ema_update_multi": (I, [V, V, I, F, F, V]),
    "es_pack_entry_size": (I, []),
    "es_pack_weights": (I, [V, V, I, V]),
    "es_cast_f32_bf16": (I, [V, V, L, V]),
    "es_add_f32": (I, [V, V, L, V]),
    "es_gemm_nt_f32": (I, [I, V, I, V, I, V, V, I, V, V, I, I, I, I, I, V]),
    "es_gemm_tn_f32_workspace": (Z, [I, I, I]),
    "es_gemm_tn_f32": (I, [V, I, V, I, I, I, I, I, V, V, I, V, V]),
    "es_attn_fwd_f32": (I, [V, I, V, I, V, I, I, I, F, V]),
    "es_attn_bwd_f32": (I, [V, I, V, I, V, V, V, I, V, I, I, I, I, F, V]),
    "es_attn_cls_fwd_f32": (I, [V, I, V, I, V, I, I, I, F, V]),
    "es_attn_cls_bwd_f32": (I, [V, I, V, I, V, V, I, V, I, I, I, I, F, V]),
    "es_layernorm_fwd_f32": (I, [V, I, V, V, V, I, V, V, I, I, F, V]),
    "es_layernorm_bwd_f32": (I, [V, I, V, I, V, V, V, V, I, V, I, V, I, V, V, V, I, I, I, I, V]),
    "es_patch_im2col_f32": (I, [V, V, I, I, I, V]),
    "es_patch_im2col_u8_f32": (I, [V, F, F, F, F, F, F, V, I, I, I, V]),
    "es_embed_bwd_f32": (I, [V, I, V, I, V, V, I, I, I, I, V]),
    "es_pack_weights_f32": (I, [V, V, I, V]),
    "es_copy_f32": (I, [V, V, L, V]),
# ... 101 lines not shown
```

endoscopy-image-classification_amd/endossl/block.py:

```python
import contextlib
import ctypes

import torch

from . import _lib
from ._lib import ptr, stream

EPI_BF16, EPI_GELU, EPI_F32_RESID, EPI_DGELU, EPI_F32, EPI_PATCH, EPI_GELU_ACT, EPI_GELU_D, EPI_MULAUX = range(9)
ATTN_SCALE = 64 ** -0.5


def gemm_nt(call, epi, a, w, bias, c, M, N, K, c2=None, aux=None, ldc=None, ldaux=None, npatch=0, s=None):
    call("es_gemm_nt", epi, ptr(a), a.stride(0), ptr(w), w.stride(0), ptr(bias), ptr(c), ldc or c.stride(0), ptr(c2),
         ptr(aux), 0 if aux is None else ldaux or aux.stride(0), M, N, K, npatch, stream() if s is None else s)


def gemm_nt_resid_ln(call, a, w, bias, xmid, xin, gamma, beta, h, mean, rstd, M, N, K, eps, s=None):
    call("es_gemm_nt_resid_ln", ptr(a), a.stride(0), ptr(w), w.stride(0), ptr(bias), ptr(xmid), xmid.stride(0),
         ptr(xin), xin.stride(0), ptr(gamma), ptr(beta), ptr(h), h.stride(0), ptr(mean), ptr(rstd), M, N, K, eps,
         stream() if s is None else s)


def gemm_nt_ln(call, a, w, bias, xout, xmid, gamma, beta, h, mean, rstd, M, N, K, eps, s=None):
    call("es_gemm_nt_ln", ptr(a), a.stride(0), ptr(w), w.stride(0), ptr(bias), ptr(xout), xout.stride(0), ptr(xmid),
         xmid.stride(0), ptr(gamma), ptr(beta), ptr(h), h.stride(0), ptr(mean), ptr(rstd), M, N, K, eps,
         stream() if s is None else s)


def layernorm_fwd(call, x, gamma, beta, y, mean, rstd, M, D, eps, s=None):
    call("es_layernorm_fwd", ptr(x), x.stride(0), ptr(gamma), ptr(beta), ptr(y), y.stride(0), ptr(mean), ptr(rstd), M,
         D, eps, stream() if s is None else s)


def layernorm_bwd(call, dy, x, mean, rstd, gamma, dres, dx, dxb, dgamma, dbeta, ws, blocks, M, D, accumulate,
                  lddx=None, s=None):
    call("es_layernorm_bwd_b16" if dy.dtype == torch.bfloat16 else "es_layernorm_bwd", ptr(dy), dy.stride(0), ptr(x),
         x.stride(0), ptr(mean), ptr(rstd), ptr(gamma), ptr(dres), dres.stride(0), ptr(dx), lddx or dx.stride(0),
         ptr(dxb), 0 if dxb is None else dxb.stride(0), ptr(dgamma), ptr(dbeta), ptr(ws), blocks, M, D, accumulate,
         stream() if s is None else s)


def attn_fwd(call, qkv, o, lse, n, T, H, s=None, cls=False):
    call("es_attn_cls_fwd" if cls else "es_attn_fwd", ptr(qkv), qkv.stride(0), ptr(o), o.stride(0), ptr(lse), n, T, H,
         ATTN_SCALE, stream() if s is None else s)


def attn_bwd(call, qkv, o, lse, delta, do, dqkv, n, T, H, s=None):
    call("es_attn_bwd", ptr(qkv), qkv.stride(0), ptr(o), o.stride(0), ptr(lse), ptr(delta), ptr(do), do.stride(0),
         ptr(dqkv), dqkv.stride(0), n, T, H, ATTN_SCALE, stream() if s is None else s)


def attn_cls_bwd(call, qkv, o, lse, do, dqkv, n, T, H, s=None):
    call("es_attn_cls_bwd", ptr(qkv), qkv.stride(0), ptr(o), o.stride(0), ptr(lse), ptr(do), do.stride(0), ptr(dqkv),
         dqkv.stride(0), n, T, H, ATTN_SCALE, stream() if s is None else s)


def cast_f32_bf16(call, src, dst, numel, s=None):
    call("es_cast_f32_bf16", ptr(src), ptr(dst), numel, stream() if s is None else s)


nop = lambda *args: None


class Rows:

    def __init__(self, n, T, H, ldx=None, lddxm=None, **bufs):
        self.n, self.T, self.rows, self.ldx, self.lddxm = n, T, n * T, ldx, lddxm
        self.__dict__.update(bufs)


class Chain:

    def __init__(self, call, p, g, wb, wt, heads, eps, gelu_d=True, dh_bf16=True, bracket=lambda lb, fl, f: f()):
        self.call, self.p, self.g, self.wb, self.wt, self.heads, self.eps = call, p, g, wb, wt, heads, eps
        self.gelu_d = gelu_d
        self.epi_dh = EPI_BF16 if dh_bf16 else EPI_F32
        self.bracket = bracket

    def attn_fwd(self, b, R, cls=None, split_q=False, ln_done=False):
        call, p, s, M, D = self.call, self.p, stream(), R.rows, R.h1.shape[1]
        if not ln_done:
            layernorm_fwd(call, R.x, p(b + "norm1.weight"), p(b + "norm1.bias"), R.h1, R.mean1, R.rstd1, M, D,
                          self.eps, s)
        w, bias = self.wb[b + "attn.qkv.weight"], p(b + "attn.qkv.bias")
        if cls is not None and split_q:
            gemm_nt(call, EPI_BF16, R.h1, w[D:], bias[D:], R.qkv[:, D:], M, 2 * D, D, s=s)
            cls.h1[:R.n].copy_(R.h1[:M].view(R.n, R.T, D)[:, 0])
            gemm_nt(call, EPI_BF16, cls.h1, w[:D], bias[:D], R.qkv, R.n, D, D, ldc=R.T * 3 * D, s=s)
        else:
            gemm_nt(call, EPI_BF16, R.h1, w, bias, R.qkv, M, 3 * D, D, s=s)
        Ro = R if cls is None else cls
        attn_fwd(call, R.qkv, Ro.o, Ro.lse, R.n, R.T, self.heads, s, cls is not None)

    def mlp_fwd(self, b, R, train, fused=False, label=None, next_ln=None):
        call, p, wb, s, M = self.call, self.p, self.wb, stream(), R.rows
        D, Hd = R.h2.shape[1], R.act.shape[1]
        if fused:
            gemm_nt_resid_ln(call, R.o, wb[b + "attn.proj.weight"], p(b + "attn.proj.bias"), R.xmid, R.x,
                             p(b + "norm2.weight"), p(b + "norm2.bias"), R.h2, R.mean2, R.rstd2, M, D, D, self.eps, s)
        else:
            gemm_nt(call, EPI_F32_RESID, R.o, wb[b + "attn.proj.weight"], p(b + "attn.proj.bias"), R.xmid, M, D, D,
                    aux=R.x, ldaux=R.ldx, s=s)
            layernorm_fwd(call, R.xmid, p(b + "norm2.weight"), p(b + "norm2.bias"), R.h2, R.mean2, R.rstd2, M, D,
                          self.eps, s)
        epi, c, c2 = (EPI_GELU_D if self.gelu_d else EPI_GELU, R.pre, R.act) if train else (EPI_GELU_ACT, R.act, None)
        fc1 = lambda: gemm_nt(call, epi, R.h2, wb[b + "mlp.fc1.weight"], p(b + "mlp.fc1.bias"), c, M, Hd, D,
                              c2=c2, s=s)
        self.bracket(label, 2.0 * M * Hd * D, fc1)
        if next_ln is not None:
            gamma, beta, h1, mean1, rstd1 = next_ln
            gemm_nt_ln(call, R.act, wb[b + "mlp.fc2.weight"], p(b + "mlp.fc2.bias"), R.out, R.xmid, gamma, beta, h1,
                       mean1, rstd1, M, D, Hd, self.eps, s)
            return
        gemm_nt(call, EPI_F32_RESID, R.act, wb[b + "mlp.fc2.weight"], p(b + "mlp.fc2.bias"), R.out, M, D, Hd,
                aux=R.xmid, s=s)

    def mlp_bwd(self, b, R, ln_bwd, wgrad=None, cap=nop, label=None):
        call, p, g, wt, s, M = self.call, self.p, self.g, self.wt, stream(), R.rows
        D, Hd = R.dxb.shape[1], R.dpre.shape[1]
        cap("b_dxb", R.dxb)
        gemm_nt(call, EPI_MULAUX if self.gelu_d else EPI_DGELU, R.dxb, wt[b + "mlp.fc2.weight"], None, R.dpre, M, Hd, D,
                aux=R.pre, s=s)
        if wgrad is not None:
            wgrad(R.dxb, D, R.act, Hd, M, g(b + "mlp.fc2.weight"), g(b + "mlp.fc2.bias"))
        gemm_nt(call, self.epi_dh, R.dpre, wt[b + "mlp.fc1.weight"], None, R.dh, M, D, Hd, s=s)
        if wgrad is not None:
            wgrad(R.dpre, Hd, R.h2, D, M, g(b + "mlp.fc1.weight"), g(b + "mlp.fc1.bias"), label=label)
        cap("b_dpre", R.dpre)
        cap("b_dh2", R.dh)
        ln_bwd(R.dh, R.xmid, R.mean2, R.rstd2, p(b + "norm2.weight"), R.dres, R.dxm, R.dxmb, g(b + "norm2.weight"),
               g(b + "norm2.bias"), M, lddx=R.lddxm)
        gemm_nt(call, EPI_BF16, R.dxmb, wt[b + "attn.proj.weight"], None, R.do, M, D, D, s=s)
        if wgrad is not None:
            wgrad(R.dxmb, D, R.o, D, M, g(b + "attn.proj.weight"), g(b + "attn.proj.bias"))
        cap("b_dxm", R.dxm, R.dxmb)
        cap("b_do", R.do)

    def attn_bwd(self, b, R, ln_bwd, wgrad=None, before_ln1=nop, cap=nop, cls=None, split_q=False):
        call, p, g, s, M, T = self.call, self.p, self.g, stream(), R.rows, R.T
        D = R.dh1.shape[1]
        if cls is None:
            attn_bwd(call, R.qkv, R.o, R.lse, R.delta, R.do, R.dqkv, R.n, T, self.heads, s)
        else:
            attn_cls_bwd(call, R.qkv, cls.o, cls.lse, cls.do, R.dqkv, R.n, T, self.heads, s)
        gemm_nt(call, self.epi_dh, R.dqkv, self.wt[b + "attn.qkv.weight"], None, R.dh1, M, D, 3 * D, s=s)
        if wgrad is not None:
            gw, gb = g(b + "attn.qkv.weight"), g(b + "attn.qkv.bias")
            if cls is not None and split_q:
                wgrad(R.dqkv[:, D:], 2 * D, R.h1, D, M, gw[D * D:], gb[D:], ld1=3 * D)
                wgrad(R.dqkv, D, R.h1, D, R.n, gw[:D * D], gb[:D], ld1=T * 3 * D, ld2=T * D)
            else:
                wgrad(R.dqkv, 3 * D, R.h1, D, M, gw, gb)
        cap("b_dqkv", R.dqkv)
        cap("b_dh1", R.dh1)
        before_ln1()
        ln_bwd(R.dh1, R.x, R.mean1, R.rstd1, p(b + "norm1.weight"), R.dxm, R.dx, R.dxb_next, g(b + "norm1.weight"),
               g(b + "norm1.bias"), M)


class _TNProblem(ctypes.Structure):
    _fields_ = [("dy", ctypes.c_void_p), ("x", ctypes.c_void_p), ("out", ctypes.c_void_p),
                ("bias_out", ctypes.c_void_p), ("M", ctypes.c_int), ("N1", ctypes.c_int), ("N2", ctypes.c_int),
                ("ld1", ctypes.c_int), ("ld2", ctypes.c_int), ("mchunk", ctypes.c_int), ("tile0", ctypes.c_int),
                ("pad", ctypes.c_int)]


def on_stream(st, *after):
    if st is None:
        return contextlib.nullcontext()
    for w in after:
        st.wait_stream(w)
    return torch.cuda.stream(st)


def tn_table(problems):
    tab = (_TNProblem * len(problems))()
    for e, q in zip(tab, problems):
        e.dy, e.x, e.out, e.bias_out = ptr(q[0]), ptr(q[2]), ptr(q[5]), ptr(q[6])
        e.N1, e.N2, e.M, e.ld1, e.ld2 = q[1], q[3], q[4], q[7], q[8]
    return tab


def tn_big_grouped(problems, target, workspace, timed=None):
    lib = _lib.load()
    n, tab = len(problems), tn_table(problems)
    need = lib.es_gemm_tn_big_grouped_workspace(ctypes.byref(tab), n, target)
    ws = workspace(need)
    if need > ws.numel():
        raise RuntimeError(f"grouped weight-gradient workspace too small: {need} > {ws.numel()} floats")
    raw = ctypes.create_string_buffer(lib.es_gemm_tn_big_grouped_table_bytes(n))
    dims = (ctypes.c_int * 3)()
    rc = lib.es_gemm_tn_big_grouped_prepare(ctypes.byref(tab), n, target, ptr(ws), ws.numel(), raw, dims)
    if rc != 0:
        raise _lib.EndosslLibraryError(f"es_gemm_tn_big_grouped_prepare: status {rc}")
    if timed is None:
        _lib.call("es_gemm_tn_big_grouped", raw, n, dims, stream())
    else:
        _lib.call("es_gemm_tn_big_grouped_timed", raw, n, dims, timed[0].handle, timed[1].handle, stream())
    return dims
```

endoscopy-image-classification_amd/endossl/fixmatch.py:

```python
import os

import torch

from . import _lib, dist
from ._lib import call, ptr
from .conformer import join_wgrad_stream
from .loss import ce_loss
from .trainer import Trainer, _next
from .utils import AverageMeter


class FixMatch(Trainer):
    INFLIGHT_DEPTH = 2
    EMA_BUFFERS = False
    CKPT_SIZE_SUFFIX = True

    overlap_allreduce = os.environ.get("ENDOSSL_OVERLAP_AR", "0") == "1"

    def __init__(self, model, opt_func="Adam", lr=1e-3, device='cpu'):
        super().__init__(model, opt_func=opt_func, lr=lr, device=device)
        self.epoch_start = 1
        self._dlogits = None
        self._stats = None
        self.cnn = not hasattr(model, "engine")
        if self.cnn:
            self.EMA_BUFFERS = True

    def _trainable_when_frozen(self):
        return [self.model.fc]

    def get_config(self, config):
        self.frozen = bool(config.TRAIN.IS_FREEZE)
        for p in self.model.parameters():
            p.requires_grad = not self.frozen
        if self.frozen:
            for mod in self._trainable_when_frozen():
                mod.requires_grad_(True)
        if self.cnn:
            self.model.frozen_trunk = self.frozen
        self._setup_model(config)
        self._setup_optim(config, config.TRAIN.EVAL_STEP, self.train_labeled_dl)

    use_graph = os.environ.get("ENDOSSL_GRAPH", "0") == "1"

    def _compute(self, inputs_x, targets_x, inputs_u_w, inputs_u_s):
        cfg = self.config
        m = self.model
        eng = m.engine()
        dev = m.flat.device
        B, nu = int(inputs_x.shape[0]), int(inputs_u_w.shape[0])
        C = m.cfg.num_classes
        s = _lib.stream()
        if self._dlogits is None or self._dlogits.shape[0] != B + nu:
            self._dlogits = torch.empty(B + nu, C, dtype=torch.float32, device=dev)
            self._pl = torch.empty(nu, dtype=torch.int32, device=dev)
            self._mask = torch.empty(nu, dtype=torch.uint8, device=dev)
        stats = torch.empty(4, dtype=torch.float32, device=dev)
        frozen = getattr(self, "frozen", False)
        if eng.overlap_fwd:
            main, side = torch.cuda.current_stream(dev), eng.side_stream((B + nu) * m.cfg.T)
            side.wait_stream(main)
            with torch.cuda.stream(side):
                logits_w = eng.forward(m.flat, [inputs_u_w], train=False)
            logits = eng.forward(m.flat, [inputs_x, inputs_u_s], train=not frozen)
            main.wait_stream(side)
        else:
            logits_w = eng.forward(m.flat, [inputs_u_w], train=False)
            logits = eng.forward(m.flat, [inputs_x, inputs_u_s], train=not frozen)
        dl = self._dlogits
        call("es_poly_ce_fwd_bwd", ptr(logits), C, ptr(targets_x), ptr(self.class_weights), B, C, 2.0, 1.0 / B,
             ptr(dl), C, ptr(stats[0:1]), s)
        lam = float(cfg.TRAIN.LAMBDA_U)
        call("es_fm_consistency_fwd_bwd", ptr(logits_w), C, ptr(logits[B:]), C, nu, C, float(cfg.TRAIN.THRES),
             lam / nu, ptr(self._pl), ptr(self._mask), None, ptr(dl[B:]), C, ptr(stats[1:3]), s)
        torch.add(stats[0], stats[1], alpha=lam, out=stats[3])
        if frozen:
            eng.head_backward(m.flat, m.flat_grad, dl, train=False)
            return stats, None
        gb = dist.GradBuckets(m.flat_grad) if dist.world_size() > 1 and self.overlap_allreduce else None
        eng.backward(m.flat, m.flat_grad, dl, grad_ready=gb.ready if gb is not None else None)
        return stats, gb

    def _graphable(self):
        eng = self.model.engine()
        return (self.use_graph and eng.probe is None and not (dist.world_size() > 1 and self.overlap_allreduce))

    def static_batch(self):
        if getattr(self, "_graph", None) is None:
            return None
        x, y, uw, us = self._gin
        return ((x, y), ((uw, us), None))

    def _run_graph(self, inputs):
        key = tuple((tuple(t.shape), t.dtype) for t in inputs)
        if getattr(self, "_graph", None) is None or self._gkey != key:
            self._graph = None
            stats, _ = self._compute(*inputs)
            gin = [t.clone() for t in inputs]
            g = torch.cuda.CUDAGraph()
            with torch.cuda.graph(g):
                gstats, _ = self._compute(*gin)
            self._graph, self._gkey, self._gin, self._gstats = g, key, gin, gstats
            return stats
        for dst, src in zip(self._gin, inputs):
            if dst.data_ptr() != src.data_ptr():
                dst.copy_(src, non_blocking=True)
        self._graph.replay()
        return self._gstats

    def _step_cnn(self, batch):
        (inputs_x, targets_x), ((inputs_u_w, inputs_u_s), _) = batch
        m, cfg = self.model, self.config
        dev = m.flat.device
        self._inflight.wait()
        B, nu = int(inputs_x.shape[0]), int(inputs_u_w.shape[0])
        targets_x = targets_x.to(dev, non_blocking=True).to(torch.int64).contiguous()
        inputs = torch.cat((inputs_x.to(dev, non_blocking=True), inputs_u_w.to(dev, non_blocking=True),
                            inputs_u_s.to(dev, non_blocking=True)))
        m.train()
        out = m(inputs)
        logits = out.detach()
        C = int(logits.shape[1])
        s = _lib.stream()
        dl = torch.zeros_like(logits)
        self._pl = torch.empty(nu, dtype=torch.int32, device=dev)
        self._mask = torch.empty(nu, dtype=torch.uint8, device=dev)
        stats = torch.empty(4, dtype=torch.float32, device=dev)
        call("es_poly_ce_fwd_bwd", ptr(logits), C, ptr(targets_x), ptr(self.class_weights), B, C, 2.0, 1.0 / B,
             ptr(dl), C, ptr(stats[0:1]), s)
        lam = float(cfg.TRAIN.LAMBDA_U)
        call("es_fm_consistency_fwd_bwd", ptr(logits[B:B + nu]), C, ptr(logits[B + nu:]), C, nu, C,
             float(cfg.TRAIN.THRES), lam / nu, ptr(self._pl), ptr(self._mask), None, ptr(dl[B + nu:]), C,
             ptr(stats[1:3]), s)
        torch.add(stats[0], stats[1], alpha=lam, out=stats[3])
        self.optimizer.zero_grad()
        torch.autograd.backward([out], [dl])
        join_wgrad_stream(dev)
        self._finish_step()
        return {"loss": stats[3], "lx": stats[0], "lu": stats[1], "mask_mean": stats[2],
                "pseudo_label": self._pl, "mask": self._mask}

    def step(self, batch):
        if self.cnn:
            return self._step_cnn(batch)
        (inputs_x, targets_x), ((inputs_u_w, inputs_u_s), _) = batch
        dev = self.model.flat.device
        self._inflight.wait()
        inputs = (inputs_x.to(dev, non_blocking=True), targets_x.to(dev, non_blocking=True).to(torch.int64),
                  inputs_u_w.to(dev, non_blocking=True), inputs_u_s.to(dev, non_blocking=True))
        m = self.model
        eng = m.engine()
        eng.pack(m.flat, m.version)
        gb = None
        if self._graphable():
            stats = self._run_graph(inputs)
        else:
            stats, gb = self._compute(*inputs)
        self._finish_step(gb.finish() if gb is not None else None)
        return {"loss": stats[3], "lx": stats[0], "lu": stats[1], "mask_mean": stats[2],
                "pseudo_label": self._pl, "mask": self._mask}

    def train_one(self, epoch):
        n = self.config.TRAIN.EVAL_STEP
        return self._train_steps(self.step, self._paired_batches(n), epoch * n)

    def evaluate_one(self, show_metric=False, show_report=False, show_cf_matrix=False):
        eval_model = self._eval_model()
        summary_loss = AverageMeter()
        outs, tgts = [], []
        with torch.no_grad():
            for images, targets in self.valid_dl:
                images = images.to(self.model.flat.device, non_blocking=True)
                targets = targets.to(self.model.flat.device, non_blocking=True)
                outputs = self._first(eval_model(images))
                losses = ce_loss(outputs, targets, reduction='mean')
                summary_loss.update(losses.item(), self.config.DATA.BATCH_SIZE)
                outs.append(outputs.argmax(1).cpu().numpy())
                tgts.append(targets.cpu().numpy())
        return summary_loss, self._metrics(outs, tgts, show_metric, show_report)

    def _set_trainable(self, is_train):
        frozen = getattr(self, "frozen", False)
        for p in self.model.parameters():
            p.requires_grad = bool(is_train) and not frozen
        if is_train and frozen:
            for mod in self._trainable_when_frozen():
                mod.requires_grad_(True)

    def fit(self):
        if self.epoch_start == self.config.TRAIN.EPOCHS:
            valid_loss, valid_metric = self.evaluate_one()
            print(f'\tValid Loss: {valid_loss.avg:.3f}')
            print(f'\tMetric: {valid_metric}')
            return
        for epoch in range(self.epoch_start, self.config.TRAIN.EPOCHS + 1):
            self._fit_epoch(epoch)
```

endoscopy-image-classification_amd/endossl/vit.py:

```python
import ctypes
import functools
import math
import os

import torch
import torch.nn as nn

from . import _lib, block
from ._lib import call, ptr
from .block import (EPI_BF16, EPI_DGELU, EPI_F32, EPI_F32_RESID, EPI_GELU, EPI_GELU_ACT,
                    EPI_GELU_D, EPI_MULAUX, EPI_PATCH, Rows, _TNProblem)

LN_BWD_BLOCKS = 1024
SIDE_PRIORITY = -1
SIDE_PRIORITY_MIN_M = 65536


IMAGENET_MEAN = (0.485, 0.456, 0.406)
IMAGENET_STD = (0.229, 0.224, 0.225)


def _rup(x, m):
    return (x + m - 1) // m * m

# ... 93 lines not shown

class _Acts:

    def __init__(self, cfg, n, train, device, b16=torch.bfloat16):
        D, Hd, L = cfg.dim, cfg.hidden, cfg.depth
        self.n, self.train = n, train
        self.M = n * cfg.T
        Mp = _rup(self.M, 256) + 256
        self.Mp = Mp
        Lk = L if train else 1
        f32 = torch.float32
        z = lambda *s, dt=f32: torch.zeros(*s, dtype=dt, device=device)
        self.patches = z(_rup(n * cfg.np, 256), 3 * cfg.patch * cfg.patch, dt=b16)
        self.x = z(L + 1 if train else 2, Mp, D)
        self.xmid = z(Lk, Mp, D)
        self.h1 = z(Lk, Mp, D, dt=b16)
        self.h2 = z(Lk, Mp, D, dt=b16)
        self.mean1, self.rstd1 = z(Lk, Mp), z(Lk, Mp)
        self.mean2, self.rstd2 = z(Lk, Mp), z(Lk, Mp)
        self.qkv = z(Lk, Mp, 3 * D, dt=b16)
        self.o = z(Lk, Mp, D, dt=b16)
        self.lse = z(Lk, n * cfg.heads * cfg.T)
        self.pre = z(Lk if train else 0, Mp, Hd, dt=b16)
        self.act = z(Lk, Mp, Hd, dt=b16)
        Mc = _rup(n, 256)
        self.c_o, self.c_lse = z(Mc, D, dt=b16), z(n * cfg.heads)
        self.c_h1 = z(Mc, D, dt=b16)
        self.c_xmid, self.c_h2 = z(Mc, D), z(Mc, D, dt=b16)
        self.c_mean2, self.c_rstd2 = z(Mc), z(Mc)
        self.c_pre = z(Mc, Hd, dt=b16) if train else None
        self.c_act, self.c_xout = z(Mc, Hd, dt=b16), z(Mc, D)
        self.xhat = z(n, D)
        self.rstd_cls = z(n)
        self.logits = z(n, cfg.num_classes)
        self.fts = z(n, D) if cfg.head == "emb" else None


class _Grads:

    def __init__(self, cfg, n, device, b16=torch.bfloat16):
        D, Hd = cfg.dim, cfg.hidden
        Mp = _rup(n * cfg.T, 256) + 256
        f32 = torch.float32
        z = lambda *s, dt=f32: torch.zeros(*s, dtype=dt, device=device)
        self.n = n
        self.dx, self.dxb = z(Mp, D), z(Mp, D, dt=b16)
        self.dxm, self.dxmb = z(Mp, D), z(Mp, D, dt=b16)
        self.dh = z(Mp, D, dt=b16) if Engine.DH_BF16 else z(Mp, D)
        self.dpre = z(Mp, Hd, dt=b16)
        self.dqkv = z(Mp, 3 * D, dt=b16)
        self.do = z(Mp, D, dt=b16)
        self.dpatch = z(_rup(n * cfg.np, 256), D, dt=b16)
        self.dyn = z(n, D)
        self.delta = z(n * cfg.heads * cfg.T)
        Mc = _rup(n, 256)
        self.c_dx, self.c_dxb = z(Mc, D), z(Mc, D, dt=b16)
        self.c_dpre, self.c_dxmb, self.c_do = z(Mc, Hd, dt=b16), z(Mc, D, dt=b16), z(Mc, D, dt=b16)
        self.c_dh = z(Mc, D, dt=b16) if Engine.DH_BF16 else z(Mc, D)
        self.dxm_cls = z(Mp, D)


class _WgradSchedule:

    def __init__(self, sets, M, depth, grouped, *, layer_wgrad, defer_ln, bf16, capture, group_layers, min_m, main,
                 side, wgrad, wgrad_layer, launch_grouped, ln_flush, grad_ready=None, block_range=None,
                 on_stream=block.on_stream):
        self.mode = "grouped" if grouped else "layer" if layer_wgrad and bf16 and M >= min_m else "each"
        self.defer = [] if defer_ln and grad_ready is None and not capture and self.mode != "each" else None
        self.sets, self.depth, self.group_layers, self.min_m = sets, depth, group_layers, min_m
        self.main, self.side, self.on_stream = main, side, on_stream
        self._wgrad, self._wgrad_layer, self._launch_grouped, self._ln_flush = wgrad, wgrad_layer, launch_grouped, ln_flush
        self.grad_ready, self.block_range = grad_ready, block_range
        self.problems = []
        self.done = {}

    def grad_sets(self, i):
        if self.mode == "grouped":
            return self.sets[i], self.sets[i - 1] if i > 0 else self.sets[self.depth]
        return self.sets[i % 2], self.sets[(i - 1) % 2]

    def wgrad(self, dy, N1, x, N2, M, out, bias_out=None, ld1=None, ld2=None, label=None):
        l1, l2 = ld1 or N1, ld2 or N2
        if self.mode == "grouped" or (self.mode == "layer" and M >= self.min_m and N1 % 384 == 0 and N2 % 192 == 0
                                      and l1 % 8 == 0 and l2 % 8 == 0):
            self.problems.append((dy, N1, x, N2, M, out, bias_out, l1, l2, label))
            return
        with self.on_stream(self.side, self.main):
            self._wgrad(dy, N1, x, N2, M, out, bias_out, ld1=ld1, ld2=ld2, label=label)

    def _flush_layer(self, i):
        if self.mode != "layer" or not (self.problems or self.defer):
            return
        with self.on_stream(self.side, self.main):
            if self.problems:
                self._wgrad_layer(self.problems, i)
                self.problems.clear()
            if self.defer:
                self._ln_flush(self.defer)

    def before_ln1(self, i):
        self._flush_layer(i)
        if self.side is not None and self.mode != "grouped":
            self.done[i] = self.side.record_event()
            if i + 1 in self.done:
                self.main.wait_event(self.done.pop(i + 1))

    def block_done(self, i):
        if self.mode == "grouped" and i > 0 and i % self.group_layers == 0 and self.problems:
            with self.on_stream(self.side, self.main):
                self._launch_grouped(self.problems, i)
                if self.defer:
                    self._ln_flush(self.defer)
            self.problems.clear()
        if self.grad_ready is not None:
            evs = [self.main.record_event()] + ([self.done[i]] if i in self.done else [])
            self.grad_ready(*self.block_range(i), evs)

    def finish(self):
        self._flush_layer(-1)
        if self.mode == "grouped":
            self._launch_grouped(self.problems, 0)
        if self.defer:
            self._ln_flush(self.defer)
        if self.side is not None:
            self.main.wait_stream(self.side)


class Engine:

    TN_TARGET_BLOCKS = 768
    TN_SHARE = 0.5
    TN_SHARE_MIN_M = 16384
    TN_MAX_SPLITS = 128
    GROUP_WGRAD = "auto"
    GROUP_WGRAD_MAX_M = 16384
    GROUP_LAYERS = 6
    DEFER_LN_GRADS = True
    LN_MULTI_MAX = 32
    LAYER_WGRAD = True
    LAYER_TN_SHARE = 0.375
    _OV = os.environ.get("ENDOSSL_OVERLAP", "1")
    OVERLAP_FWD = _OV in ("1", "fwd")
    OVERLAP = _OV in ("1", "bwd")
    DH_BF16 = True
    GELU_D = True
    PRUNE_LAST = True
    PRUNE_Q = True
    RESID_LN = os.environ.get("ENDOSSL_RESID_LN", "1") == "1"
    RESID_LN_MIN_M = 40000
    FC2_LN = os.environ.get("ENDOSSL_FC2_LN", "1") == "1"
    FC2_LN_MIN_M = 50000
    FC2_LN_TRAIN = True
    FC2_LN_WEAK = True

    PARITY_NAMES = {n: n + "_f32" for n in (
        "es_gemm_nt", "es_gemm_tn", "es_attn_fwd", "es_attn_bwd", "es_attn_cls_fwd", "es_attn_cls_bwd",
        "es_layernorm_fwd", "es_layernorm_bwd", "es_patch_im2col", "es_patch_im2col_u8", "es_embed_bwd",
        "es_pack_weights")}
    PARITY_NAMES.update({"es_layernorm_bwd_b16": "es_layernorm_bwd_f32", "es_cast_f32_bf16": "es_copy_f32"})

    def __init__(self, cfg, device, precision="bf16"):
        if precision not in ("bf16", "fp32"):
            raise ValueError(f"precision must be 'bf16' (production) or 'fp32' (parity mode), got {precision!r}")
        self.cfg, self.device = cfg, device
        self.precision = precision
        self.op_dtype = torch.bfloat16 if precision == "bf16" else torch.float32
        self.layout, self.offs, self.numel = param_layout(cfg)
        self.shapes = dict(self.layout)
        self._acts = {}
        self._grads = {}
        self._ws = None
        self._ws_ln = None
        self._ws_lnp = None
        self._lnp_next = 0
        self._side = None
        self._ncu_cache = None
        self._gtab = {}
        self._grad_b = None
        self.overlap = self.OVERLAP
        self.overlap_fwd = self.OVERLAP_FWD
        self._packed_version = -1
        D, Hd = cfg.dim, cfg.hidden
        b16 = self.op_dtype
        mats = [("patch_embed.proj.weight", D, 3 * cfg.patch * cfg.patch, False)]
        for i in range(cfg.depth):
            b = f"blocks.{i}."
            mats += [(b + "attn.qkv.weight", 3 * D, D, True), (b + "attn.proj.weight", D, D, True),
                     (b + "mlp.fc1.weight", Hd, D, True), (b + "mlp.fc2.weight", D, Hd, True)]
        self.wb, self.wt = {}, {}
        esz = _lib.load().es_pack_entry_size()
        raw = bytearray(esz * len(mats))
        for j, (name, N, K, need_t) in enumerate(mats):
            self.wb[name] = torch.zeros(N, K, dtype=b16, device=device)
            if need_t:
                self.wt[name] = torch.zeros(K, N, dtype=b16, device=device)
            dst_t = self.wt[name].data_ptr() if need_t else 0
            entry = (ctypes.c_long(self.offs[name]), ctypes.c_void_p(self.wb[name].data_ptr()),
                     ctypes.c_void_p(dst_t), ctypes.c_int(N), ctypes.c_int(K))
            buf = b"".join(bytes(e) for e in entry)
            raw[j * esz:j * esz + len(buf)] = buf
        self._pack_tab = torch.frombuffer(raw, dtype=torch.uint8).to(device)
        self._nmat = len(mats)
        self.probe = None
        self.capture = None

    def _call(self, name, *args):
        if self.precision == "fp32":
            name = self.PARITY_NAMES.get(name, name)
        return call(name, *args)

    def _bracket(self, label, flop, launch):
        pr = self.probe
        if pr is None or pr["label"] != label:
            launch()
            return None
        e0, e1 = torch.cuda.Event(enable_timing=True), torch.cuda.Event(enable_timing=True)
        e0.record()
        launch()
        e1.record()
        pr["events"].append((e0, e1, flop))
        return pr

    def _chain(self, flat, grad=None):
        return block.Chain(self._call, lambda name: self.view(flat, name), lambda name: self.view(grad, name),
                           self.wb, self.wt, self.cfg.heads, self.cfg.eps, gelu_d=self.GELU_D, dh_bf16=self.DH_BF16,
                           bracket=self._bracket)

    def view(self, flat, name):
        o = self.offs[name]
        return flat[o:o + math.prod(self.shapes[name])]

    def pack(self, flat, version=None):
        if version is not None and version == self._packed_version:
            return
        self._call("es_pack_weights", ptr(flat), ptr(self._pack_tab), self._nmat, _lib.stream())
        self._packed_version = version if version is not None else -1

    def acts(self, n, train):
        key = (n, train)
        if key not in self._acts:
            self._acts[key] = _Acts(self.cfg, n, train, self.device, self.op_dtype)
        return self._acts[key]

    def workspace(self):
        if self._ws is None:
            cfg = self.cfg
            D, Hd = cfg.dim, cfg.hidden
            n_tn = max(a * b for a, b in ((3 * D, D), (D, D), (Hd, D), (D, Hd), (D, 3 * cfg.patch * cfg.patch)))
            self._ws = torch.empty(self.TN_MAX_SPLITS * n_tn + 2 * 1024 * max(Hd, 3 * D), dtype=torch.float32,
                                   device=self.device)
        return self._ws

    def ln_workspace(self):
        if self._ws_ln is None:
            self._ws_ln = torch.empty(2 * LN_BWD_BLOCKS * self.cfg.dim, dtype=torch.float32, device=self.device)
        return self._ws_ln

    def _ncu(self):
        if self._ncu_cache is None:
            self._ncu_cache = torch.cuda.get_device_properties(self.device).multi_processor_count
        return self._ncu_cache

    def side_stream(self, tokens=0):
        prio = SIDE_PRIORITY if tokens >= SIDE_PRIORITY_MIN_M else 0
        if self._side is None:
            self._side = {}
        if prio not in self._side:
            self._side[prio] = torch.cuda.Stream(device=self.device, priority=prio)
        return self._side[prio]

    def forward(self, flat, images_list, train):
        cfg = self.cfg
        s = _lib.stream()
        n = sum(int(t.shape[0]) for t in images_list)
        A = self.acts(n, train)
        D, T, H = cfg.dim, cfg.T, cfg.heads
        K0 = 3 * cfg.patch * cfg.patch
        row = 0
        for t in images_list:
            if t.shape[1:] != (3, cfg.img_size, cfg.img_size) or t.dtype not in (torch.float32, torch.uint8):
                raise ValueError(f"expected fp32 (normalised) or uint8 (raw) [n,3,{cfg.img_size},{cfg.img_size}] "
                                 f"images, got {tuple(t.shape)} {t.dtype}")
            t = t.contiguous()
            if t.dtype == torch.uint8:
                self._call("es_patch_im2col_u8", ptr(t), *IMAGENET_MEAN, *IMAGENET_STD, ptr(A.patches[row * cfg.np:]),
                     int(t.shape[0]), cfg.img_size, cfg.patch, s)
            else:
                self._call("es_patch_im2col", ptr(t), ptr(A.patches[row * cfg.np:]), int(t.shape[0]), cfg.img_size,
                     cfg.patch, s)
            row += int(t.shape[0])
        x0 = A.x[0]
        pos = self.view(flat, "pos_embed")
        block.gemm_nt(self._call, EPI_PATCH, A.patches, self.wb["patch_embed.proj.weight"],
                      self.view(flat, "patch_embed.proj.bias"), x0, n * cfg.np, D, K0, aux=pos, ldaux=D, npatch=cfg.np)
        self._call("es_cls_init", ptr(x0), D, ptr(self.view(flat, "cls_token")), ptr(pos), n, T, D, s)
        M = A.M
        prune = self._prune()
        ch = self._chain(flat)
        fused = self.RESID_LN and D == 384 and self.precision == "bf16" and M >= self.RESID_LN_MIN_M
        fc2_ln = (self.FC2_LN and (self.FC2_LN_TRAIN if train else self.FC2_LN_WEAK) and D == 384
                  and self.precision == "bf16" and M >= self.FC2_LN_MIN_M)
        ln_done = False
        for i in range(cfg.depth):
            b = f"blocks.{i}."
            li = i if train else 0
            xin = A.x[i] if train else A.x[i & 1]
            xout = A.x[i + 1] if train else A.x[(i + 1) & 1]
            R = Rows(n, T, H, x=xin, h1=A.h1[li], mean1=A.mean1[li], rstd1=A.rstd1[li], qkv=A.qkv[li], o=A.o[li],
                     lse=A.lse[li], xmid=A.xmid[li], h2=A.h2[li], mean2=A.mean2[li], rstd2=A.rstd2[li],
                     pre=A.pre[li] if train else None, act=A.act[li], out=xout)
            if prune and i == cfg.depth - 1:
                Rc = self._cls_rows(A, n, xin)
                ch.attn_fwd(b, R, cls=Rc, split_q=self.PRUNE_Q, ln_done=ln_done)
                ch.mlp_fwd(b, Rc, train)
                if self.capture is not None:
                    self.capture("fwd_cls", train, i, xin[:M], A.c_xout[:n])
                break
            ch.attn_fwd(b, R, ln_done=ln_done)
            next_ln = None
            if fc2_ln and i + 1 < cfg.depth:
                nb, ni = f"blocks.{i + 1}.", i + 1 if train else 0
                next_ln = (self.view(flat, nb + "norm1.weight"), self.view(flat, nb + "norm1.bias"), A.h1[ni],
                           A.mean1[ni], A.rstd1[ni])
            ch.mlp_fwd(b, R, train, fused=fused, label="fc1_fwd" if train else "fc1_fwd_weak", next_ln=next_ln)
            ln_done = next_ln is not None
            if self.capture is not None:
                self.capture("fwd", train, i, xin[:M], xout[:M])
        xl = A.x[cfg.depth] if train else A.x[cfg.depth & 1]
        Tl = T
        if prune:
            xl, Tl = A.c_xout, 1
        if cfg.head == "emb":
            self._call("es_cls_ln_fwd", ptr(xl), D, Tl, ptr(self.view(flat, "norm.weight")),
                 ptr(self.view(flat, "norm.bias")), ptr(A.fts), D, ptr(A.xhat), ptr(A.rstd_cls), n, D, cfg.eps, s)
            return A.fts
        self._call("es_cls_head_fwd", ptr(xl), D, Tl, ptr(self.view(flat, "norm.weight")), ptr(self.view(flat, "norm.bias")),
             ptr(self.view(flat, "head.weight")), ptr(self.view(flat, "head.bias")), ptr(A.logits),
             cfg.num_classes, ptr(A.xhat), ptr(A.rstd_cls), n, D, cfg.num_classes, cfg.eps, s)
        return A.logits

    def _prune(self):
        return self.PRUNE_LAST

    def _cls_rows(self, A, n, xin=None, G=None):
        T, D = self.cfg.T, self.cfg.dim
        R = Rows(n, 1, self.cfg.heads, ldx=T * D, lddxm=T * D, x=xin, h1=A.c_h1, o=A.c_o, lse=A.c_lse, xmid=A.c_xmid,
                 h2=A.c_h2, mean2=A.c_mean2, rstd2=A.c_rstd2, pre=A.c_pre, act=A.c_act, out=A.c_xout)
        if G is not None:
            R.dxb, R.dpre, R.dh, R.dres, R.dxmb, R.do = G.c_dxb, G.c_dpre, G.c_dh, G.c_dx, G.c_dxmb, G.c_do
            R.dxm = G.dxm_cls
        return R

    def _tn_splits(self, M, N1, N2):
        if self._tn_shared(M, N1, N2):
            tiles = (N1 // 384) * (N2 // 192)
            return max(1, int(self._ncu() * self.TN_SHARE) // tiles)
        return 0

    def _tn_shared(self, M, N1, N2):
        return (self.TN_SHARE < 1.0 and self.overlap and M >= self.TN_SHARE_MIN_M and N1 % 384 == 0
                and N2 % 192 == 0 and self.precision == "bf16")

    def _split_q_rows(self, n, tn_pin):
        if n % 32:
            return False
        D = self.cfg.dim
        big = self.precision == "bf16" and D % 384 == 0 and (
            tn_pin == 7 or (tn_pin < 0 and (n >= 65536 or self._tn_shared(n, D, D))))
        return n % 64 == 0 or not big

    def _wgrad(self, dy, N1, x, N2, M, out, bias_out=None, ld1=None, ld2=None, label=None):
        ws = self.workspace()
        splits = self._tn_splits(M, N1, N2)
        need = getattr(_lib.load(), "es_gemm_tn_f32_workspace" if self.precision == "fp32" else "es_gemm_tn_workspace")
        if need(N1, N2, splits) > ws.numel():
            raise RuntimeError(f"wgrad workspace too small for {N1}x{N2} x {splits} splits")
        variant = 7 if splits and self._tn_shared(M, N1, N2) else -1
        args = (ptr(dy), ld1 or N1, ptr(x), ld2 or N2, M, N1, N2, splits, ptr(ws), ptr(out), 0, ptr(bias_out))
        if self.precision == "fp32":
            fn, args = "es_gemm_tn", args + (_lib.stream(),)
        else:
            fn, args = "es_gemm_tn_ex", args + (variant, _lib.stream())
        self._bracket(label, 2.0 * M * N1 * N2, lambda: self._call(fn, *args))

    def _ln_bwd(self, dy, x, mean, rstd, gamma, dres, dx, dxb, dgamma, dbeta, M, lddx=None, defer=None):
        D = self.cfg.dim
        grid = _lib.load().es_layernorm_bwd_grid(LN_BWD_BLOCKS, M)
        if defer is not None and grid >= 64:
            ws = self.ln_part_workspace(self._lnp_next)
            self._lnp_next += 1
            block.layernorm_bwd(self._call, dy, x, mean, rstd, gamma, dres, dx, dxb, None, None, ws, LN_BWD_BLOCKS, M,
                                D, 0, lddx)
            defer.append((ws, dgamma, dbeta, grid, 0))
            return
        block.layernorm_bwd(self._call, dy, x, mean, rstd, gamma, dres, dx, dxb, dgamma, dbeta, self.ln_workspace(),
                            LN_BWD_BLOCKS, M, D, 0, lddx)

    def ln_part_workspace(self, k):
        if self._ws_lnp is None:
            self._ws_lnp = []
        while len(self._ws_lnp) <= k:
            self._ws_lnp.append(torch.empty(2 * LN_BWD_BLOCKS * self.cfg.dim, dtype=torch.float32, device=self.device))
        return self._ws_lnp[k]

    def _ln_grads_flush(self, pending):
        if not pending:
            return
        lib = _lib.load()
        esz = lib.es_ln_param_grads_entry_size()
        for c0 in range(0, len(pending), self.LN_MULTI_MAX):
            chunk = pending[c0:c0 + self.LN_MULTI_MAX]
            raw = (ctypes.c_char * (esz * len(chunk)))()
            for j, (ws, dg, db, grid, acc) in enumerate(chunk):
                ent = (ctypes.c_void_p(ptr(ws)), ctypes.c_void_p(ptr(dg)), ctypes.c_void_p(ptr(db)),
                       ctypes.c_int(grid), ctypes.c_int(self.cfg.dim), ctypes.c_int(acc), ctypes.c_int(0))
                buf = b"".join(bytes(e) for e in ent)
                ctypes.memmove(ctypes.byref(raw, j * esz), buf, len(buf))
            self._call("es_ln_param_grads_multi", ctypes.addressof(raw), len(chunk), _lib.stream())
        pending.clear()

    def backward(self, flat, grad, dlogits=None, dfts=None, zero_grad=True, grad_ready=None):
        cfg = self.cfg
        s = _lib.stream()
        top = dfts if cfg.head == "emb" else dlogits
        if top is None:
            raise ValueError("Engine.backward needs dlogits (cls head) or dfts (emb head)")
        n = int(top.shape[0])
        A = self.acts(n, True)
        D, T, M = cfg.dim, cfg.T, A.M
        gv = lambda name: self.view(grad, name)
        fv = lambda name: self.view(flat, name)
        grouped = self._grouped_wgrad(M, grad_ready)
        GS = self._grad_sets(n, grouped)
        G = GS[0]
        sched = _WgradSchedule(
            GS, M, cfg.depth, grouped, layer_wgrad=self.LAYER_WGRAD, defer_ln=self.DEFER_LN_GRADS,
            bf16=self.precision == "bf16", capture=self.capture is not None, group_layers=self.GROUP_LAYERS,
            min_m=self.TN_SHARE_MIN_M, main=torch.cuda.current_stream(self.device),
            side=self.side_stream(M) if self.overlap else None, wgrad=self._wgrad, wgrad_layer=self._wgrad_layer,
            launch_grouped=self._launch_grouped, ln_flush=self._ln_grads_flush, grad_ready=grad_ready,
            block_range=self._block_range)
        self._lnp_next = 0
        ln_bwd = functools.partial(self._ln_bwd, defer=sched.defer)
        if zero_grad and cfg.head == "emb":
            grad.zero_()
        prune = self._prune()
        GL = sched.grad_sets(cfg.depth - 1)[0]
        dtop, Tt = (GL.c_dx, 1) if prune else (G.dx, T)
        if not prune:
            G.dx.zero_()
        if cfg.head == "emb":
            dfts = dfts.contiguous()
            self._call("es_cls_ln_bwd", ptr(dfts), D, ptr(fv("norm.weight")), ptr(A.xhat), ptr(A.rstd_cls), ptr(dtop), D, Tt,
                 ptr(gv("norm.weight")), ptr(gv("norm.bias")), n, D, s)
        else:
            dlogits = dlogits.contiguous()
            self._call("es_cls_head_bwd_ex", ptr(dlogits), cfg.num_classes, ptr(fv("head.weight")), ptr(fv("norm.weight")),
                 ptr(fv("norm.bias")), ptr(A.xhat), ptr(A.rstd_cls), ptr(G.dyn), ptr(dtop), D, Tt,
                 ptr(gv("head.weight")), ptr(gv("head.bias")), ptr(gv("norm.weight")), ptr(gv("norm.bias")), n, D,
                 cfg.num_classes, 0 if zero_grad else 1, s)
        if self.capture is not None:
            self.capture("dtop", True, cfg.depth - 1, dtop[:n] if prune else G.dx[:M])
        if prune:
            block.cast_f32_bf16(self._call, GL.c_dx, GL.c_dxb, n * D)
        else:
            block.cast_f32_bf16(self._call, G.dx, GL.dxb, M * D)
        ch = self._chain(flat, grad)
        cap = block.nop
        for i in reversed(range(cfg.depth)):
            b = f"blocks.{i}."
            Gi, Gn = sched.grad_sets(i)
            before_ln1 = functools.partial(sched.before_ln1, i)
            if self.capture is not None:
                cap = functools.partial(self._capture_rows, i, M)
            R = self._bwd_rows(A, G, Gi, Gn, i, n)
            if prune and i == cfg.depth - 1:
                Rc, R.dxm = self._cls_rows(A, n, G=Gi), Gi.dxm_cls
                ch.mlp_bwd(b, Rc, ln_bwd, sched.wgrad)
                split_q = self.PRUNE_Q and self._split_q_rows(n, _lib.tn_variant())
                ch.attn_bwd(b, R, ln_bwd, sched.wgrad, before_ln1, cls=Rc, split_q=split_q)
            else:
                ch.mlp_bwd(b, R, ln_bwd, sched.wgrad, cap, label="fc1_wgrad")
                ch.attn_bwd(b, R, ln_bwd, sched.wgrad, before_ln1, cap)
            if self.capture is not None:
                self.capture("bwd", True, i, G.dx[:M])
            sched.block_done(i)
        self._call("es_embed_bwd", ptr(G.dx), D, ptr(G.dpatch), D, ptr(gv("pos_embed")), ptr(gv("cls_token")), n, T, D, 0,
             s)
        sched.wgrad(G.dpatch, D, A.patches, 3 * cfg.patch * cfg.patch, n * cfg.np, gv("patch_embed.proj.weight"),
                    gv("patch_embed.proj.bias"))
        sched.finish()
        return grad

    def _grad_sets(self, n, grouped):
        mk = lambda: _Grads(self.cfg, n, self.device, self.op_dtype)
        if n not in self._grads:
            self._grads[n] = (mk(), mk())
        if not grouped:
            return self._grads[n]
        key = (n, "grouped")
        if key not in self._grads:
            self._grads[key] = [self._grads[n][0]] + [mk() for _ in range(self.cfg.depth)]
        return self._grads[key]

    def _block_range(self, i):
        nxt = f"blocks.{i + 1}.norm1.weight" if i + 1 < self.cfg.depth else "norm.weight"
        return self.offs[f"blocks.{i}.norm1.weight"], self.offs[nxt]

    def _capture_rows(self, i, M, kind, *ts):
        self.capture(kind, True, i, *(t[:M] for t in ts))

    def _bwd_rows(self, A, G, Gi, Gn, i, n):
        return Rows(n, self.cfg.T, self.cfg.heads, dxb=Gi.dxb, pre=A.pre[i], act=A.act[i], dpre=Gi.dpre, dh=G.dh,
                    h2=A.h2[i], xmid=A.xmid[i], mean2=A.mean2[i], rstd2=A.rstd2[i], dres=G.dx, dxm=G.dxm, dxmb=Gi.dxmb,
                    do=G.do, o=A.o[i], qkv=A.qkv[i], lse=A.lse[i], delta=G.delta, dqkv=Gi.dqkv, dh1=G.dh, h1=A.h1[i],
                    x=A.x[i], mean1=A.mean1[i], rstd1=A.rstd1[i], dx=G.dx, dxb_next=Gn.dxb)

    def _wgrad_layer(self, problems, layer):
        share = self.LAYER_TN_SHARE if (self.overlap and layer > 0) else 1.0
        target = max(1, int(self._ncu() * share))
        n, workspace = len(problems), lambda need: self.workspace()
        pr = self.probe
        if pr is not None and any(q[9] == pr["label"] for q in problems) and (layer > 0 or not self.overlap):
            flop = sum(2.0 * q[4] * q[1] * q[3] for q in problems)
            e0, e1 = _lib.KernelEvent(), _lib.KernelEvent()
            dims = block.tn_big_grouped(problems, target, workspace, timed=(e0, e1))
            pr["events"].append((e0, e1, flop))
            pr["layer_kernel"] = (f"es_gemm_tn_big_grouped: one block's {n} weight-gradient GEMMs "
                                  f"({'+'.join(str(q[1]) + 'x' + str(q[3]) for q in problems)}) over M={problems[0][4]} "
                                  f"tokens, {dims[0]} workgroups of 384x192, then one reduce launch")
            pr["layer_bytes"] = sum(2.0 * q[4] * (q[1] + q[3]) + 4.0 * q[1] * q[3] + (4.0 * q[1] if q[6] is not None else 0)
                                    for q in problems)
        else:
            block.tn_big_grouped(problems, target, workspace)

    def _grouped_wgrad(self, M, grad_ready):
        if self.precision != "bf16" or grad_ready is not None:
            return False
        return self.GROUP_WGRAD == "1" or (self.GROUP_WGRAD == "auto" and M < self.GROUP_WGRAD_MAX_M)

    def _launch_grouped(self, problems, slot):
        problems = sorted(problems, key=lambda q: -q[4])
        tab = block.tn_table(problems)
        lib = _lib.load()
        tiles = lib.es_gemm_tn_grouped_prepare(ctypes.byref(tab), len(problems))
        if tiles <= 0:
            raise _lib.EndosslLibraryError(f"es_gemm_tn_grouped_prepare: status {tiles}")
        raw = bytes(tab)
        cache = self._gtab.get(slot)
        if cache is None or cache[0] != raw:
            if torch.cuda.is_current_stream_capturing():
                raise RuntimeError("grouped weight-gradient table changed during hipGraph capture; run one eager "
                                   "step of this shape first")
            dev = torch.frombuffer(bytearray(raw), dtype=torch.uint8).to(self.device, non_blocking=False)
            self._gtab[slot] = cache = (raw, dev)
        pr = self._bracket("fc1_wgrad", sum(2.0 * q[4] * q[1] * q[3] for q in problems),
                           lambda: call("es_gemm_tn_grouped", ptr(cache[1]), len(problems), tiles, _lib.stream()))
        if pr is not None:
            pr["kernel"] = f"es_gemm_tn_grouped ({len(problems)} weight-gradient GEMMs, {tiles} tiles)"

    def head_backward(self, flat, grad, dlogits, train=False):
        cfg = self.cfg
        if cfg.head != "cls":
            raise ValueError("head_backward is the classifier-head model's; the emb-head model runs its heads' "
                             "backward in comatch_model.EmbHeads")
        n, D, C = int(dlogits.shape[0]), cfg.dim, cfg.num_classes
        A = self.acts(n, train)
        if getattr(self, "_hb", None) is None or self._hb[0].shape[0] < n:
            z = lambda *sh: torch.zeros(*sh, dtype=torch.float32, device=self.device)
            self._hb = (z(n, D), z(n, D), z(D), z(D))
        dyn, dx, gnw, gnb = self._hb
        grad.zero_()
        self._call("es_cls_head_bwd", ptr(dlogits.contiguous()), C, ptr(self.view(flat, "head.weight")),
                   ptr(self.view(flat, "norm.weight")), ptr(self.view(flat, "norm.bias")), ptr(A.xhat),
                   ptr(A.rstd_cls), ptr(dyn), ptr(dx), D, 1, ptr(self.view(grad, "head.weight")),
                   ptr(self.view(grad, "head.bias")), ptr(gnw), ptr(gnb), n, D, C, _lib.stream())
        return grad


class _ViTFunction(torch.autograd.Function):
    @staticmethod
    def forward(ctx, x, module, *params):
        ctx.module = module
        ctx.n = int(x.shape[0])
        logits = module.engine().forward(module.flat, [x], train=True)
        return logits.clone()

    @staticmethod
    def backward(ctx, dlogits):
        m = ctx.module
        g = m.engine().backward(m.flat, m.flat_grad, dlogits.float())
        return (None, None) + tuple(m.engine().view(g, name).view(shape) for name, shape in m.layout)


class NativeViT(nn.Module):

    def __init__(self, cfg=None, seed=None, **kw):
        super().__init__()
        self.cfg = cfg if cfg is not None else ViTConfig(**kw)
        self.layout, self.offs, self.numel = param_layout(self.cfg)
        flat = torch.zeros(self.numel, dtype=torch.float32)
        gen = torch.Generator().manual_seed(seed) if seed is not None else None
        timm_init_(flat, self.cfg, self.layout, self.offs, generator=gen)
        self._set_flat(flat)
        self._engine = None
        self.precision = "bf16"
        self.version = 0

    def _set_flat(self, flat):
        self.flat = flat
        self.flat_grad = torch.zeros_like(flat)
        for name, shape in self.layout:
            view = flat[self.offs[name]:self.offs[name] + math.prod(shape)].view(shape)
            mod, attr = self._resolve(name)
            p = nn.Parameter(view, requires_grad=True)
            mod._parameters[attr] = p

    def _resolve(self, name):
        parts = name.split(".")
        mod = self
        for p in parts[:-1]:
            if p not in mod._modules:
                mod._modules[p] = nn.Module()
            mod = mod._modules[p]
        return mod, parts[-1]

    def _apply(self, fn, recurse=True):
        new = fn(self.flat)
        if new is not self.flat:
            self._set_flat(new.contiguous())
            self._engine = None
        return self

# ... 48 lines not shown
```

include/endossl.h:

```cpp
#ifndef ENDOSSL_H
#define ENDOSSL_H
#include <stddef.h>
#include <stdint.h>
#include <hip/hip_runtime_api.h>

#ifdef __cplusplus
extern "C" {
#endif

int es_abi_version(void);

int es_gemm_nt(int epi, const void* A, int lda, const void* B, int ldb, const float* bias, void* C, int ldc,
               void* C2, const void* aux, int ldaux, int M, int N, int K, int np, hipStream_t stream);
int es_gemm_nt_resid_ln(const void* A, int lda, const void* B, int ldb, const float* bias, float* C, int ldc,
                        const float* aux, int ldaux, const float* gamma, const float* beta, void* h, int ldh,
                        float* mean, float* rstd, int M, int N, int K, float eps, hipStream_t stream);
int es_gemm_nt_ln(const void* A, int lda, const void* B, int ldb, const float* bias, float* C, int ldc,
                  const float* aux, int ldaux, const float* gamma, const float* beta, void* h, int ldh, float* mean,
                  float* rstd, int M, int N, int K, float eps, hipStream_t stream);
int es_set_gemm_variant(int variant);
int es_set_gemm_small_tile(int v);
int es_set_tn_variant(int variant);
size_t es_gemm_tn_workspace(int N1, int N2, int splits);
int es_gemm_tn(const void* A1, int ld1, const void* A2, int ld2, int M, int N1, int N2, int splits,
               float* workspace, float* out, int accumulate, float* bias_out, hipStream_t stream);
int es_gemm_tn_ex(const void* A1, int ld1, const void* A2, int ld2, int M, int N1, int N2, int splits,
                  float* workspace, float* out, int accumulate, float* bias_out, int variant, hipStream_t stream);
int es_splitk_reduce(const float* P, float* out, int S, int n, int accumulate, hipStream_t stream);
typedef struct {
  const void* dy;
  const void* x;
  float* out;
  float* bias_out;
  int M, N1, N2, ld1, ld2;
  int mchunk, tile0, pad;
} es_tn_problem;
size_t es_tn_problem_size(void);
int es_gemm_tn_grouped_prepare(void* host_table, int count);
int es_gemm_tn_grouped(const void* device_table, int count, int total_tiles, hipStream_t stream);
size_t es_gemm_tn_big_grouped_table_bytes(int count);
size_t es_gemm_tn_big_grouped_workspace(const void* problems, int count, int target_wgs);
int es_gemm_tn_big_grouped_prepare(const void* problems, int count, int target_wgs, float* workspace,
                                   size_t workspace_floats, void* table, int* dims);
int es_gemm_tn_big_grouped(const void* table, int count, const int* dims, hipStream_t stream);
int es_gemm_tn_big_grouped_timed(const void* table, int count, const int* dims, void* start, void* stop,
                                 hipStream_t stream);
int es_event_create(void** ev);
int es_event_elapsed(void* start, void* stop, float* ms);
int es_event_destroy(void* ev);
int es_colsum(const void* Y, int ld, int M, int N, float* workspace, int blocks, float* out, int accumulate,
              hipStream_t stream);
int es_reduce_partials(const float* P, float* out, int G, int N, int accumulate, hipStream_t stream);

int es_set_attn_variant(int occ);
int es_set_attn_bwd_variant(int v);
int es_set_attn_bwd_grid(int workgroups);
int es_set_attn_bwd_long(int v);
int es_attn_fwd(const void* qkv, int ldqkv, void* o, int ldo, float* lse, int nimg, int T, int H, float scale,
                hipStream_t stream);
int es_attn_bwd(const void* qkv, int ldqkv, const void* o, int ldo, const float* lse, float* delta, const void* dout,
                int lddo, void* dqkv, int lddqkv, int nimg, int T, int H, float scale, hipStream_t stream);
int es_attn_cls_fwd(const void* qkv, int ldqkv, void* o, int ldo, float* lse, int nimg, int T, int H, float scale,
                    hipStream_t stream);
int es_attn_cls_bwd(const void* qkv, int ldqkv, const void* o, int ldo, const float* lse, const void* dout, int lddo,
                    void* dqkv, int lddqkv, int nimg, int T, int H, float scale, hipStream_t stream);

int es_set_ln_fwd_grid(int workgroups);
int es_layernorm_fwd(const float* x, int ldx, const float* gamma, const float* beta, void* y, int ldy, float* mean,
                     float* rstd, int M, int D, float eps, hipStream_t stream);
int es_layernorm_bwd(const float* dy, int lddy, const float* x, int ldx, const float* mean, const float* rstd,
                     const float* gamma, const float* dres, int ldres, float* dx, int lddx, void* dxb, int lddxb,
                     float* dgamma, float* dbeta, float* workspace, int blocks, int M, int D, int accumulate,
                     hipStream_t stream);
int es_layernorm_bwd_b16(const void* dy, int lddy, const float* x, int ldx, const float* mean, const float* rstd,
                         const float* gamma, const float* dres, int ldres, float* dx, int lddx, void* dxb, int lddxb,
                         float* dgamma, float* dbeta, float* workspace, int blocks, int M, int D, int accumulate,
                         hipStream_t stream);
int es_layernorm_bwd_grid(int blocks, int M);
int es_ln_param_grads_entry_size(void);
int es_ln_param_grads_multi(const void* table, int n, hipStream_t stream);

int es_gelu_fwd(const void* x, void* y, long n, hipStream_t stream);
int es_gelu_bwd(const void* x, const void* dy, void* dx, long n, hipStream_t stream);

size_t es_aug_entry_size(void);
size_t es_aug_strong_workspace(int n, int S);
size_t es_aug_fixmatch_workspace(int n, int S, int is_crop, int max_w, int max_h);
int es_aug_fixmatch_u8(const uint8_t* frames, size_t frames_bytes, const void* entries, const int32_t* coeffs,
                       size_t coeff_count, int n, int S, int is_crop, int max_h, uint8_t* weak, uint8_t* strong,
                       void* workspace, size_t workspace_bytes, hipStream_t stream);
int es_aug_strong_u8(const uint8_t* weak, const void* entries, int n, int S, uint8_t* strong, void* workspace,
                     size_t workspace_bytes, hipStream_t stream);

size_t es_aug_comatch_entry_size(void);
size_t es_aug_labeled_entry_size(void);
size_t es_aug_comatch_workspace(int n, int S, int is_crop, int max_w, int max_h);
size_t es_aug_labeled_workspace(int n, int S, int is_crop, int max_w, int max_h);
int es_aug_comatch_u8(const uint8_t* frames, size_t frames_bytes, const void* entries, const int32_t* coeffs,
                      size_t coeff_count, int n, int S, int is_crop, int max_h, uint8_t* weak, uint8_t* strong0,
                      uint8_t* strong1, void* workspace, size_t workspace_bytes, hipStream_t stream);
int es_aug_labeled_u8(const uint8_t* frames, size_t frames_bytes, const void* entries, const int32_t* coeffs,
                      size_t coeff_count, int n, int S, int is_crop, int max_h, uint8_t* out, void* workspace,
                      size_t workspace_bytes, hipStream_t stream);
int es_aug_jitter_u8(const uint8_t* x, const void* plans, int n, int S, uint8_t* out, hipStream_t stream);


int es_patch_im2col(const float* img, void* patches, int n, int S, int P, hipStream_t stream);

int es_patch_im2col_u8(const void* img, float mean0, float mean1, float mean2, float std0, float std1, float std2,
                       void* patches, int n, int S, int P, hipStream_t stream);
int es_cls_init(float* x, int ldx, const float* cls, const float* pos, int n, int T, int D, hipStream_t stream);
int es_embed_bwd(const float* dx, int lddx, void* dpatch, int ldp, float* dpos, float* dcls, int n, int T, int D,
                 int accumulate, hipStream_t stream);
int es_cls_head_fwd(const float* x, int ldx, int T, const float* gamma, const float* beta, const float* W,
                    const float* b, float* logits, int ldl, float* xhat, float* rstd, int n, int D, int C, float eps,
                    hipStream_t stream);
int es_cls_head_bwd(const float* dl, int lddl, const float* W, const float* gamma, const float* beta,
                    const float* xhat, const float* rstd, float* dyn, float* dx, int lddx, int T, float* dW, float* db,
                    float* dgamma, float* dbeta, int n, int D, int C, hipStream_t stream);
int es_cls_head_bwd_ex(const float* dl, int lddl, const float* W, const float* gamma, const float* beta,
                       const float* xhat, const float* rstd, float* dyn, float* dx, int lddx, int T, float* dW,
                       float* db, float* dgamma, float* dbeta, int n, int D, int C, int accumulate, hipStream_t stream);

int es_cls_ln_fwd(const float* x, int ldx, int T, const float* gamma, const float* beta, float* fts, int ldf,
                  float* xhat, float* rstd, int n, int D, float eps, hipStream_t stream);
int es_cls_ln_bwd(const float* dfts, int lddf, const float* gamma, const float* xhat, const float* rstd, float* dx,
                  int lddx, int T, float* dgamma, float* dbeta, int n, int D, hipStream_t stream);

int es_dense_fwd(const float* X, int ldx, const float* W, const float* b, float* Y, int ldy, int n, int K, int N,
                 int act, float slope, const void* keep, float keep_scale, hipStream_t stream);
size_t es_dense_bwd_workspace(int n, int N);
int es_dense_bwd(const float* dY, int lddy, const float* Yact, int ldya, int act, float slope, const void* keep,
                 float keep_scale, const float* X, int ldx, const float* W, float* dX, int lddx, int accumulate_dx,
                 float* dW, float* db, int n, int K, int N, float* workspace, hipStream_t stream);
int es_bn1d_fwd(const float* U, int ldu, const float* gamma, const float* beta, float* running_mean, float* running_var,
                void* num_batches_tracked, float momentum, float eps, int train, float* Y, int ldy, float* xhat,
                float* rstd, int n, int F, hipStream_t stream);
int es_bn1d_bwd(const float* dY, int lddy, const float* xhat, const float* rstd, const float* gamma, float* dU,
                int lddu, float* dgamma, float* dbeta, int n, int F, hipStream_t stream);
int es_bn1d_sums(const float* U, int ldu, int n, int F, const float* S1, float N, float* out, hipStream_t stream);
int es_bn1d_fwd_global(const float* U, int ldu, const float* gamma, const float* beta, const float* S1,
                       const float* S2, float N, float* running_mean, float* running_var, void* num_batches_tracked,
                       float momentum, float eps, float* Y, int ldy, float* xhat, float* rstd, int n, int F,
                       hipStream_t stream);
int es_bn1d_bwd_sums(const float* dY, int lddy, const float* xhat, int n, int F, float* out, hipStream_t stream);
int es_bn1d_bwd_global(const float* dY, int lddy, const float* xhat, const float* rstd, const float* gamma,
                       const float* sums_global, const float* sums_local, float N, float* dU, int lddu,
                       float* dgamma, float* dbeta, int n, int F, hipStream_t stream);
int es_dropout_keep(void* keep, long n, float p, unsigned long long seed, unsigned long long offset,
                    hipStream_t stream);
int es_l2norm_fwd(const float* V, int ldv, float* Z, int ldz, float* norm, int n, int L, hipStream_t stream);
int es_l2norm_bwd(const float* dZ, int lddz, const float* Z, int ldz, const float* norm, float* dV, int lddv, int n,
                  int L, hipStream_t stream);

size_t es_comatch_pseudo_workspace(int nu, int C, int Q);
int es_comatch_pseudo(const float* logits_w, int ldl, int nu, int C, float* hist, int hist_cap, int hist_len,
                      int hist_pos, const float* z_w, int ldz, int L, const float* bank_feats, const float* bank_probs,
                      int Q, float temperature, float alpha, float thres, float* probs, float* probs_orig, int* pl,
                      float* mask, float* workspace, hipStream_t stream);
int es_comatch_pseudo_ex(const float* logits_w, int ldl, int nu, int C, float* hist, int hist_cap, int hist_len,
                         int hist_pos, int hist_given, const float* z_w, int ldz, int L, const float* bank_feats,
                         const float* bank_probs, int Q, float temperature, float alpha, float thres, float* probs,
                         float* probs_orig, int* pl, float* mask, float* workspace, hipStream_t stream);
int es_softmax_colmean(const float* logits, int ldl, int n, int C, float* out, hipStream_t stream);
int es_comatch_bank_write(const float* z_w, int ldzw, int nu, const float* z_x, int ldzx, int bt, int L,
                          const float* probs_orig, const void* y_int64, int C, float* bank_feats, float* bank_probs,
                          int ptr, int Q, hipStream_t stream);
size_t es_comatch_contrastive_workspace(int nu);
int es_comatch_contrastive_fwd_bwd(const float* z0, int ldz0, const float* z1, int ldz1, const float* probs, int nu,
                                   int L, int C, float temperature, float contrast_th, float grad_scale,
                                   float* loss_out, float* dz0, int lddz0, float* dz1, int lddz1, float* workspace,
                                   hipStream_t stream);
size_t es_comatch_contrastive_ex_workspace(int nr, int nc);
int es_comatch_contrastive_fwd_bwd_ex(const float* z0, int ldz0, const float* z1_all, int ldz1,
                                      const float* probs_rows, const float* probs_all, int nr, int nc, int row_off,
                                      int L, int C, float temperature, float contrast_th, float grad_scale,
                                      float loss_div, float* loss_out, float* dz0, int lddz0, float* dz1_all,
                                      int lddz1, float* workspace, hipStream_t stream);
int es_comatch_focal_fwd_bwd(const float* ls, int ldl, const float* probs, const float* mask, int nu, int C,
                             float gamma, float grad_scale, float* loss_out, float* dls, int lddl, float* workspace,
                             hipStream_t stream);

int es_fm_consistency_fwd_bwd(const float* logits_w, int ldw, const float* logits_s, int lds, int n, int C,
                              float tau, float grad_scale, int* pseudo_label, uint8_t* mask, float* row_loss,
                              float* dlogits_s, int lddls, float* out, hipStream_t stream);
int es_poly_ce_fwd_bwd(const float* logits, int ldl, const int64_t* targets, const float* weights, int n, int C,
                       float epsilon, float grad_scale, float* dlogits, int lddl, float* out, hipStream_t stream);

int es_triplet_fwd_bwd(const float* z, int ldz, int bs, int L, float alpha, float grad_scale, float* dz, int lddz,
                       float* out, hipStream_t stream);
int es_softmax_predict(const float* logits, int ldl, int n, int C, float thres, int* pred, float* conf, int* label,
                       hipStream_t stream);

size_t es_margin_softmax_workspace(int n, int C);
int es_margin_softmax_fwd_bwd(const float* x, int ldx, const float* W, const float* bias, const int64_t* targets,
                              const float* class_weights, const float* mask, int n, int F, int C, int kind, float s,
                              float m, float eps, float grad_scale, float* dx, int lddx, float* dW, float* db,
                              float* out, float* row_loss, float* workspace, hipStream_t stream);

int es_ezbm_sample_mix(const float* mem, int ldm, const int64_t* mem_y, int N, int D, int C, const int* cls_off,
                       const int* cls_idx, const float* cdf, const float* lam_table, unsigned long long seed,
                       unsigned long long offset, const int* idx_in, const int* dual_in, int n, float* X, int ldx,
                       int64_t* t, int64_t* td, float* lam, int* idx, int* dual, hipStream_t stream);
int es_bn1d_groups_fwd(const float* U, int ldu, const float* gamma, const float* beta, float* running_mean,
                       float* running_var, void* num_batches_tracked, float momentum, float eps, float* Y, int ldy,
                       float* xhat, float* rstd, int n, int G, int F, hipStream_t stream);
int es_bn1d_groups_bwd(const float* dY, int lddy, const float* xhat, const float* rstd, const float* gamma, float* dU,
                       int lddu, float* dgamma, float* dbeta, int n, int G, int F, hipStream_t stream);
int es_ezbm_ce_fwd_bwd(const float* logits, int ldl, const int64_t* t, const int64_t* td, int n, int C, float lambda_c,
                       float grad_scale, float* dlogits, int lddl, float* out, hipStream_t stream);

int es_set_stem_kernels(int v);
int es_conv2d_fwd(const float* x, int N, int H, int W, int Cin, long sxn, long sxh, long sxw, long sxc,
                  const float* w, const float* bias, int Cout, int kh, int kw, int stride, int pad, float* y, long syn,
                  long syh, long syw, int accumulate, hipStream_t stream);
int es_conv2d_bwd_data(const float* dy, long syn, long syh, long syw, const float* w, int N, int H, int W, int Cin,
                       int Cout, int kh, int kw, int stride, int pad, float* dx, long sxn, long sxh, long sxw, long sxc,
                       int accumulate, hipStream_t stream);
int es_conv2d_dw_tiles(int Cout, int Cin, int kh, int kw);
size_t es_conv2d_bwd_weight_workspace(int Cout, int Cin, int kh, int kw, int splits);
int es_conv2d_bwd_weight(const float* x, int N, int H, int W, int Cin, long sxn, long sxh, long sxw, long sxc,
                         const float* dy, long syn, long syh, long syw, int Cout, int kh, int kw, int stride, int pad,
                         int splits, float* workspace, float* dw, int accumulate, hipStream_t stream);
int es_conv2d_bf16_eligible(int Cin, int Cout, int kh, int kw);
int es_set_conv_dw_target(int v);
int es_set_conv_ring(int stages);
int es_set_conv_dw_buf(int v);
int es_set_conv_small(int wgs);
int es_conv2d_pack_bf16(const float* w, int Cout, int Cin, int kh, int kw, void* wp, void* wt, hipStream_t stream);
int es_conv_pack_entry_size(void);
int es_conv2d_pack_bf16_multi(const void* table, int n, long max_elems, hipStream_t stream);
int es_conv2d_fwd_bf16(const float* x, int N, int H, int W, int Cin, long sxn, long sxh, long sxw, long sxc,
                       const void* wp, const float* bias, int Cout, int kh, int kw, int stride, int pad, float* y,
                       long syn, long syh, long syw, int accumulate, hipStream_t stream);
int es_conv2d_bwd_data_bf16(const float* dy, long syn, long syh, long syw, const void* wt, int N, int H, int W,
                            int Cin, int Cout, int kh, int kw, int stride, int pad, float* dx, long sxn, long sxh,
                            long sxw, long sxc, int accumulate, hipStream_t stream);
size_t es_conv2d_bnstats_size(int M, int Cout);
int es_conv2d_fwd_bf16_bnstats(const float* x, int N, int H, int W, int Cin, long sxn, long sxh, long sxw, long sxc,
                               const void* wp, const float* bias, int Cout, int kh, int kw, int stride, int pad,
                               float* y, long syn, long syh, long syw, float* partials, hipStream_t stream);
size_t es_conv2d_bwd_weight_bf16_workspace(int M, int Cout, int Cin, int kh, int kw, int splits);
int es_conv2d_bwd_weight_bf16(const float* x, int N, int H, int W, int Cin, long sxn, long sxh, long sxw, long sxc,
                              const float* dy, long syn, long syh, long syw, int Cout, int kh, int kw, int stride,
                              int pad, int splits, float* workspace, float* dw, int accumulate, hipStream_t stream);
size_t es_chan_workspace(int rows, int C);
int es_chan_sum(const float* v, int rows, int C, long sn, long sp, int HW, float* workspace, float* out,
                int accumulate, hipStream_t stream);
int es_bn2d_fwd(const float* x, int rows, int C, const float* gamma, const float* beta, float* running_mean,
                float* running_var, void* num_batches_tracked, float momentum, float eps, int train, const float* res,
                int relu, float* y, float* mean, float* rstd, float* workspace, hipStream_t stream);
int es_bn2d_bwd(const float* x, const float* y, const float* dy, int rows, int C, int relu, const float* gamma,
                const float* mean, const float* rstd, int train, const float* running_var, float eps, float* dx,
                float* gout, float* dgamma, float* dbeta, int accumulate, float* workspace, hipStream_t stream);
int es_bn2d_fwd_partials(const float* x, int rows, int C, float* partials, const float* gamma,
                         const float* beta, float* running_mean, float* running_var, void* num_batches_tracked,
                         float momentum, float eps, const float* res, int relu, float* y, float* mean, float* rstd,
                         hipStream_t stream);
int es_bn2d_sums(const float* x, int rows, int C, int mode, const float* sum_g, int rows_g, float* out,
                 float* workspace, hipStream_t stream);
int es_bn2d_fwd_global(const float* x, int rows, int C, const float* gamma, const float* beta, float* running_mean,
                       float* running_var, void* num_batches_tracked, float momentum, float eps, const float* sum_g,
                       const float* sq_g, int rows_g, const float* res, int relu, float* y, float* mean, float* rstd,
                       hipStream_t stream);
int es_bn2d_bwd_sums(const float* x, const float* y, const float* dy, int rows, int C, int relu, const float* mean,
                     const float* rstd, float* out, float* workspace, hipStream_t stream);
int es_bn2d_bwd_global(const float* x, const float* y, const float* dy, int rows, int C, int relu, const float* gamma,
                       const float* mean, const float* rstd, const float* sums_local, const float* sums_g, int rows_g,
                       float* dx, float* gout, float* dgamma, float* dbeta, int accumulate, hipStream_t stream);
int es_maxpool2d_fwd(const float* x, int N, int H, int W, int C, int k, int s, int p, float* y, void* arg,
                     hipStream_t stream);
int es_maxpool2d_bwd(const float* dy, const void* arg, int N, int H, int W, int C, int k, int s, int p, float* dx,
                     hipStream_t stream);
int es_avgpool2d_fwd(const float* x, int N, int H, int W, int C, int k, float* y, hipStream_t stream);
int es_avgpool2d_bwd(const float* dy, int N, int H, int W, int C, int k, float* dx, int accumulate,
                     hipStream_t stream);
int es_upsample_add_fwd(const float* base, const float* src, int N, int H, int W, int C, int s, float* out,
                        hipStream_t stream);
int es_upsample_bwd(const float* dout, int N, int H, int W, int C, int s, float* dsrc, hipStream_t stream);

int es_conv2d_fwd_bf16_ex(const void* x, int N, int H, int W, int Cin, long sxn, long sxh, long sxw, long sxc,
                          const void* wp, const float* bias, int Cout, int kh, int kw, int stride, int pad, void* y,
                          long syn, long syh, long syw, int accumulate, float* bn_partials, int flags,
                          hipStream_t stream);
int es_conv2d_bwd_data_bf16_ex(const void* dy, long syn, long syh, long syw, const void* wt, int N, int H, int W,
                               int Cin, int Cout, int kh, int kw, int stride, int pad, void* dx, long sxn, long sxh,
                               long sxw, long sxc, int accumulate, int flags, hipStream_t stream);
int es_conv2d_bwd_weight_bf16_ex(const void* x, int N, int H, int W, int Cin, long sxn, long sxh, long sxw, long sxc,
                                 const void* dy, long syn, long syh, long syw, int Cout, int kh, int kw, int stride,
                                 int pad, int splits, float* workspace, float* dw, int accumulate, int flags,
                                 hipStream_t stream);
int es_conv2d_fwd_bf16_bnin_ex(const void* x, int N, int H, int W, int Cin, long sxn, long sxh, long sxw, long sxc,
                               const void* wp, const float* bias, int Cout, int kh, int kw, int stride, int pad,
                               void* y, long syn, long syh, long syw, int accumulate, float* bn_partials, int flags,
                               const float* in_mean, const float* in_rstd, const float* in_gamma,
                               const float* in_beta, hipStream_t stream);
int es_conv2d_bwd_weight_bf16_bnin_ex(const void* x, int N, int H, int W, int Cin, long sxn, long sxh, long sxw,
                                      long sxc, const void* dy, long syn, long syh, long syw, int Cout, int kh, int kw,
                                      int stride, int pad, int splits, float* workspace, float* dw, int accumulate,
                                      int flags, const float* in_mean, const float* in_rstd, const float* in_gamma,
                                      const float* in_beta, hipStream_t stream);
int es_conv1x1_fwd_bf16_ex(const void* x, int M, int Cin, const void* wp, const float* bias, int Cout, void* y,
                           int accumulate, float* bn_partials, int flags, hipStream_t stream);
int es_conv1x1_fwd_bf16_bnin_ex(const void* x, int M, int Cin, const void* wp, const float* bias, int Cout, void* y,
                                int accumulate, float* bn_partials, int flags, const float* in_mean,
                                const float* in_rstd, const float* in_gamma, const float* in_beta,
                                hipStream_t stream);
int es_conv1x1_bwd_data_bf16_ex(const void* dy, int M, int Cout, const void* wt, int Cin, void* dx, int accumulate,
                                int flags, hipStream_t stream);
int es_set_conv_1x1(int v);
int es_conv1x1_bf16_select(int kind, int M, int Cin, int Cout);
int es_chan_sum_ex(const void* v, int rows, int C, long sn, long sp, int HW, float* workspace, float* out,
                   int accumulate, int flags, hipStream_t stream);
int es_set_bn_cs(int v);
int es_set_bn_sum8(int v);
int es_bn2d_fwd_ex(const void* x, int rows, int C, const float* gamma, const float* beta, float* running_mean,
                   float* running_var, void* num_batches_tracked, float momentum, float eps, int train, const void* res,
                   int relu, void* y, float* mean, float* rstd, float* workspace, int flags, hipStream_t stream);
int es_bn2d_bwd_ex(const void* x, const void* y, const void* dy, int rows, int C, int relu, const float* gamma,
                   const float* mean, const float* rstd, int train, const float* running_var, float eps, void* dx,
                   void* gout, float* dgamma, float* dbeta, int accumulate, float* workspace, int flags,
                   hipStream_t stream);
int es_bn2d_bwd_recompute_ex(const void* x, const void* dy, int rows, int C, const float* gamma, const float* beta,
                             const float* mean, const float* rstd, void* dx, float* dgamma, float* dbeta, int accumulate,
                             float* workspace, int flags, hipStream_t stream);
int es_bn2d_fwd_partials_ex(const void* x, int rows, int C, float* partials, const float* gamma, const float* beta,
                            float* running_mean, float* running_var, void* num_batches_tracked, float momentum,
                            float eps, const void* res, int relu, void* y, float* mean, float* rstd, int flags,
                            hipStream_t stream);
int es_bn2d_sums_ex(const void* x, int rows, int C, int mode, const float* sum_g, int rows_g, float* out,
                    float* workspace, int flags, hipStream_t stream);
int es_bn2d_fwd_global_ex(const void* x, int rows, int C, const float* gamma, const float* beta, float* running_mean,
                          float* running_var, void* num_batches_tracked, float momentum, float eps, const float* sum_g,
                          const float* sq_g, int rows_g, const void* res, int relu, void* y, float* mean, float* rstd,
                          int flags, hipStream_t stream);
int es_bn2d_bwd_sums_ex(const void* x, const void* y, const void* dy, int rows, int C, int relu, const float* mean,
                        const float* rstd, float* out, float* workspace, int flags, hipStream_t stream);
int es_bn2d_bwd_global_ex(const void* x, const void* y, const void* dy, int rows, int C, int relu, const float* gamma,
                          const float* mean, const float* rstd, const float* sums_local, const float* sums_g, int rows_g,
                          void* dx, void* gout, float* dgamma, float* dbeta, int accumulate, int flags,
// ... 105 lines not shown
```

Before: 15230 unlabeled images/s.

## Fuse FixMatch losses and trim CLS-tail copies and dgrad work

Three changes share a CLS_TAIL flag. The poly-CE and consistency loss kernels plus the torch.add become one two-block launch, with a last-arriver atomic that writes the combined loss. The last block's Q projection reads CLS rows through a strided lda instead of copying them out first. In the last-layer attention backward, the Q-gradient zero fill is skipped and dgrad is split into a full-M K/V GEMM and a CLS-only Q GEMM. Each path is used only when the GEMM tile divides n, and the global arrival counter adds cross-block sync risk.

```diff
diff --git a/endoscopy-image-classification_amd/csrc/attention.hip b/endoscopy-image-classification_amd/csrc/attention.hip
--- a/endoscopy-image-classification_amd/csrc/attention.hip
+++ b/endoscopy-image-classification_amd/csrc/attention.hip
@@ -1452,7 +1452,7 @@
   }
 }
 
-template <int KMAX>
+template <int KMAX, bool ZQ>
 __global__ __launch_bounds__(64) void attn_cls_bwd_kernel(const bf16* __restrict__ qkv, int ldqkv,
                                                           const bf16* __restrict__ o, int ldo,
                                                           const float* __restrict__ lse,
@@ -1504,7 +1504,7 @@
       bf16* drow = dbase + (size_t)j * lddqkv + h * 64 + 8 * c;
       *(bf16x8*)(drow + D) = dk8;
       *(bf16x8*)(drow + 2 * D) = dv8;
-      if (j > 0) *(bf16x8*)drow = zero8;
+      if (ZQ && j > 0) *(bf16x8*)drow = zero8;
     }
   }
 #pragma unroll
@@ -1559,6 +1559,24 @@
 int g_attn_bwd_long = 1;
 int g_attn_bwd_grid = -1;
 
+}
+
+template <bool ZQ>
+static int attn_cls_bwd_launch(const void* qkv, int ldqkv, const void* o, int ldo, const float* lse, const void* dout,
+                               int lddo, void* dqkv, int lddqkv, int nimg, int T, int H, float scale,
+                               hipStream_t stream) {
+  if (nimg <= 0 || T <= 0 || T > 8 * CLS_KMAX_LONG || H <= 0 || ldqkv < 3 * H * 64 || lddqkv < 3 * H * 64 ||
+      ldo < H * 64 || lddo < H * 64 || (ldqkv % 8) || (lddqkv % 8) || (ldo % 8) || (lddo % 8))
+    return ES_BAD_SHAPE;
+  if (!qkv || !o || !lse || !dout || !dqkv) return ES_BAD_ARG;
+  if (T <= 8 * CLS_KMAX)
+    hipLaunchKernelGGL(HIP_KERNEL_NAME(attn_cls_bwd_kernel<CLS_KMAX, ZQ>), nimg * H, 64, 0, stream, (const bf16*)qkv,
+                       ldqkv, (const bf16*)o, ldo, lse, (const bf16*)dout, lddo, (bf16*)dqkv, lddqkv, T, H, scale);
+  else
+    hipLaunchKernelGGL(HIP_KERNEL_NAME(attn_cls_bwd_kernel<CLS_KMAX_LONG, ZQ>), nimg * H, 64, 0, stream,
+                       (const bf16*)qkv, ldqkv, (const bf16*)o, ldo, lse, (const bf16*)dout, lddo, (bf16*)dqkv, lddqkv,
+                       T, H, scale);
+  return hipGetLastError() == hipSuccess ? ES_OK : ES_HIP_ERROR;
 }
 
 extern "C" {
@@ -1701,17 +1719,12 @@
 
 int es_attn_cls_bwd(const void* qkv, int ldqkv, const void* o, int ldo, const float* lse, const void* dout, int lddo,
                     void* dqkv, int lddqkv, int nimg, int T, int H, float scale, hipStream_t stream) {
-  if (nimg <= 0 || T <= 0 || T > 8 * CLS_KMAX_LONG || H <= 0 || ldqkv < 3 * H * 64 || lddqkv < 3 * H * 64 ||
-      ldo < H * 64 || lddo < H * 64 || (ldqkv % 8) || (lddqkv % 8) || (ldo % 8) || (lddo % 8))
-    return ES_BAD_SHAPE;
-  if (!qkv || !o || !lse || !dout || !dqkv) return ES_BAD_ARG;
-  if (T <= 8 * CLS_KMAX)
-    hipLaunchKernelGGL(HIP_KERNEL_NAME(attn_cls_bwd_kernel<CLS_KMAX>), nimg * H, 64, 0, stream, (const bf16*)qkv, ldqkv,
-                       (const bf16*)o, ldo, lse, (const bf16*)dout, lddo, (bf16*)dqkv, lddqkv, T, H, scale);
-  else
-    hipLaunchKernelGGL(HIP_KERNEL_NAME(attn_cls_bwd_kernel<CLS_KMAX_LONG>), nimg * H, 64, 0, stream, (const bf16*)qkv,
-                       ldqkv, (const bf16*)o, ldo, lse, (const bf16*)dout, lddo, (bf16*)dqkv, lddqkv, T, H, scale);
-  return hipGetLastError() == hipSuccess ? ES_OK : ES_HIP_ERROR;
-}
-
-}
+  return attn_cls_bwd_launch<true>(qkv, ldqkv, o, ldo, lse, dout, lddo, dqkv, lddqkv, nimg, T, H, scale, stream);
+}
+
+int es_attn_cls_bwd_kv(const void* qkv, int ldqkv, const void* o, int ldo, const float* lse, const void* dout,
+                       int lddo, void* dqkv, int lddqkv, int nimg, int T, int H, float scale, hipStream_t stream) {
+  return attn_cls_bwd_launch<false>(qkv, ldqkv, o, ldo, lse, dout, lddo, dqkv, lddqkv, nimg, T, H, scale, stream);
+}
+
+}
diff --git a/endoscopy-image-classification_amd/csrc/gemm.hip b/endoscopy-image-classification_amd/csrc/gemm.hip
--- a/endoscopy-image-classification_amd/csrc/gemm.hip
+++ b/endoscopy-image-classification_amd/csrc/gemm.hip
@@ -1576,24 +1576,7 @@
 static int g_tn_variant = -1;
 static int g_small_tile = 1;
 
-extern "C" {
-
-int es_gemm_tn_ex(const void* A1, int ld1, const void* A2, int ld2, int M, int N1, int N2, int splits,
-                  float* workspace, float* out, int accumulate, float* bias_out, int variant, hipStream_t stream);
-
-int es_gemm_nt(int epi, const void* A, int lda, const void* B, int ldb, const float* bias, void* C,
-               int ldc, void* C2, const void* aux, int ldaux, int M, int N, int K, int np,
-               hipStream_t stream) {
-  if (M <= 0 || N <= 0 || K <= 0 || (N % BN) || (K % BK) || (lda % 8) || (ldb % 8) || (ldc % 4))
-    return ES_BAD_SHAPE;
-  if (!A || !B || !C) return ES_BAD_ARG;
-  if (((epi == EPI_GELU || epi == EPI_GELU_D) && !C2) ||
-      ((epi == EPI_F32_RESID || epi == EPI_DGELU || epi == EPI_MULAUX || epi == EPI_PATCH) && !aux))
-    return ES_BAD_ARG;
-  if (epi == EPI_PATCH && np <= 0) return ES_BAD_ARG;
-  if ((epi == EPI_F32_RESID || epi == EPI_PATCH) && ((ldaux % 4) || ldaux < N)) return ES_BAD_SHAPE;
-  if ((epi == EPI_DGELU || epi == EPI_MULAUX) && ((ldaux % 8) || ldaux < N)) return ES_BAD_SHAPE;
-  NTArgs a{(const bf16*)A, (const bf16*)B, bias, C, C2, aux, M, N, K, lda, ldb, ldc, ldaux, np};
+static int nt_pick(int epi, int M, int N, int K) {
   int variant = g_gemm_variant;
   if (variant < 0) {
     const bool gelu = epi == EPI_GELU || epi == EPI_GELU_ACT || epi == EPI_GELU_D;
@@ -1619,6 +1602,28 @@
     else
       variant = M < 65536 ? 0 : 1;
   }
+  return variant;
+}
+
+extern "C" {
+
+int es_gemm_tn_ex(const void* A1, int ld1, const void* A2, int ld2, int M, int N1, int N2, int splits,
+                  float* workspace, float* out, int accumulate, float* bias_out, int variant, hipStream_t stream);
+
+int es_gemm_nt(int epi, const void* A, int lda, const void* B, int ldb, const float* bias, void* C,
+               int ldc, void* C2, const void* aux, int ldaux, int M, int N, int K, int np,
+               hipStream_t stream) {
+  if (M <= 0 || N <= 0 || K <= 0 || (N % BN) || (K % BK) || (lda % 8) || (ldb % 8) || (ldc % 4))
+    return ES_BAD_SHAPE;
+  if (!A || !B || !C) return ES_BAD_ARG;
+  if (((epi == EPI_GELU || epi == EPI_GELU_D) && !C2) ||
+      ((epi == EPI_F32_RESID || epi == EPI_DGELU || epi == EPI_MULAUX || epi == EPI_PATCH) && !aux))
+    return ES_BAD_ARG;
+  if (epi == EPI_PATCH && np <= 0) return ES_BAD_ARG;
+  if ((epi == EPI_F32_RESID || epi == EPI_PATCH) && ((ldaux % 4) || ldaux < N)) return ES_BAD_SHAPE;
+  if ((epi == EPI_DGELU || epi == EPI_MULAUX) && ((ldaux % 8) || ldaux < N)) return ES_BAD_SHAPE;
+  NTArgs a{(const bf16*)A, (const bf16*)B, bias, C, C2, aux, M, N, K, lda, ldb, ldc, ldaux, np};
+  const int variant = nt_pick(epi, M, N, K);
   if (variant == 1) {
     const int grid = ((M + BM2 - 1) / BM2) * (N / BN);
     const size_t lds = 3 * STAGE2;
@@ -1649,6 +1654,12 @@
   const int rc = launch_nt(variant, epi, grid, stream, a);
   if (rc) return rc;
   return hipGetLastError() == hipSuccess ? ES_OK : ES_HIP_ERROR;
+}
+
+int es_gemm_nt_tile_rows(int epi, int M, int N, int K) {
+  if (M <= 0 || N <= 0 || K <= 0 || (N % BN) || (K % BK)) return 0;
+  const int v = nt_pick(epi, M, N, K);
+  return v == 1 ? BM2 : (v == 6 || v == 10) ? 256 : v == 11 ? 64 : BM;
 }
 
 int es_gemm_nt_resid_ln(const void* A, int lda, const void* B, int ldb, const float* bias, float* C, int ldc,
diff --git a/endoscopy-image-classification_amd/csrc/losses.hip b/endoscopy-image-classification_amd/csrc/losses.hip
--- a/endoscopy-image-classification_amd/csrc/losses.hip
+++ b/endoscopy-image-classification_amd/csrc/losses.hip
@@ -1,3 +1,5 @@
+#include <mutex>
+
 #include "common.h"
 
 namespace {
@@ -15,13 +17,12 @@
   return s;
 }
 
-__global__ __launch_bounds__(256) void fm_consistency_kernel(const float* __restrict__ lw, int ldw,
-                                                             const float* __restrict__ ls, int lds_, int n, int C,
-                                                             float tau, float grad_scale, int* __restrict__ pl,
-                                                             uint8_t* __restrict__ mask_out,
-                                                             float* __restrict__ row_loss, float* __restrict__ dls,
-                                                             int lddls, float* __restrict__ out) {
-  __shared__ float red[16];
+__device__ __forceinline__ void fm_consistency_rows(const float* __restrict__ lw, int ldw,
+                                                    const float* __restrict__ ls, int lds_, int n, int C, float tau,
+                                                    float grad_scale, int* __restrict__ pl,
+                                                    uint8_t* __restrict__ mask_out, float* __restrict__ row_loss,
+                                                    float* __restrict__ dls, int lddls, float* __restrict__ out,
+                                                    float* red) {
   float sum_loss = 0.f, sum_mask = 0.f;
   for (int i = threadIdx.x; i < n; i += blockDim.x) {
     const float* wr = lw + (size_t)i * ldw;
@@ -67,11 +68,19 @@
   }
 }
 
-__global__ __launch_bounds__(256) void poly_ce_kernel(const float* __restrict__ l, int ldl,
-                                                      const int64_t* __restrict__ y, const float* __restrict__ w,
-                                                      int n, int C, float eps, float grad_scale,
-                                                      float* __restrict__ dl, int lddl, float* __restrict__ out) {
+__global__ __launch_bounds__(256) void fm_consistency_kernel(const float* __restrict__ lw, int ldw,
+                                                             const float* __restrict__ ls, int lds_, int n, int C,
+                                                             float tau, float grad_scale, int* __restrict__ pl,
+                                                             uint8_t* __restrict__ mask_out,
+                                                             float* __restrict__ row_loss, float* __restrict__ dls,
+                                                             int lddls, float* __restrict__ out) {
   __shared__ float red[16];
+  fm_consistency_rows(lw, ldw, ls, lds_, n, C, tau, grad_scale, pl, mask_out, row_loss, dls, lddls, out, red);
+}
+
+__device__ __forceinline__ void poly_ce_rows(const float* __restrict__ l, int ldl, const int64_t* __restrict__ y,
+                                             const float* __restrict__ w, int n, int C, float eps, float grad_scale,
+                                             float* __restrict__ dl, int lddl, float* __restrict__ out, float* red) {
   float sum = 0.f;
   for (int i = threadIdx.x; i < n; i += blockDim.x) {
     const float* lr = l + (size_t)i * ldl;
@@ -97,6 +106,44 @@
   }
   sum = block_sum(sum, red);
   if (threadIdx.x == 0) out[0] = sum / (float)n;
+}
+
+__global__ __launch_bounds__(256) void poly_ce_kernel(const float* __restrict__ l, int ldl,
+                                                      const int64_t* __restrict__ y, const float* __restrict__ w,
+                                                      int n, int C, float eps, float grad_scale,
+                                                      float* __restrict__ dl, int lddl, float* __restrict__ out) {
+  __shared__ float red[16];
+  poly_ce_rows(l, ldl, y, w, n, C, eps, grad_scale, dl, lddl, out, red);
+}
+
+constexpr int FML_SLOTS = 64;
+__device__ unsigned g_fml_arrived[FML_SLOTS];
+
+struct FMLArgs {
+  const float* lx; const int64_t* y; const float* w; float* dlx;
+  const float* lw; const float* ls; int* pl; uint8_t* mask; float* dls;
+  float* stats;
+  int ldx, lddlx, ldw, lds, lddls, B, nu, C, slot;
+  float eps, gs_x, tau, gs_u, lam;
+};
+
+__global__ __launch_bounds__(256) void fixmatch_losses_kernel(const FMLArgs a) {
+  __shared__ float red[16];
+  if (blockIdx.x == 0)
+    poly_ce_rows(a.lx, a.ldx, a.y, a.w, a.B, a.C, a.eps, a.gs_x, a.dlx, a.lddlx, a.stats, red);
+  else
+    fm_consistency_rows(a.lw, a.ldw, a.ls, a.lds, a.nu, a.C, a.tau, a.gs_u, a.pl, a.mask, nullptr, a.dls, a.lddls,
+                        a.stats + 1, red);
+  if (threadIdx.x == 0) {
+    __threadfence();
+    if (atomicAdd(&g_fml_arrived[a.slot], 1u) == 1u) {
+      __threadfence();
+      const float lx = __hip_atomic_load(a.stats, __ATOMIC_RELAXED, __HIP_MEMORY_SCOPE_AGENT);
+      const float lu = __hip_atomic_load(a.stats + 1, __ATOMIC_RELAXED, __HIP_MEMORY_SCOPE_AGENT);
+      a.stats[3] = fmaf(a.lam, lu, lx);
+      __hip_atomic_store(&g_fml_arrived[a.slot], 0u, __ATOMIC_RELAXED, __HIP_MEMORY_SCOPE_AGENT);
+    }
+  }
 }
 
 __global__ __launch_bounds__(256) void ce_weighted_kernel(const float* __restrict__ l, int ldl,
@@ -429,6 +476,33 @@
   if (!logits || !targets || !dlogits || !out) return ES_BAD_ARG;
   hipLaunchKernelGGL(poly_ce_kernel, 1, 256, 0, stream, logits, ldl, targets, weights, n, C, epsilon, grad_scale,
                      dlogits, lddl, out);
+  return hipGetLastError() == hipSuccess ? ES_OK : ES_HIP_ERROR;
+}
+
+int es_fixmatch_losses(const float* logits_x, int ldx, const int64_t* targets, const float* weights, int B,
+                       float epsilon, float grad_scale_x, float* dlogits_x, int lddlx, const float* logits_w, int ldw,
+                       const float* logits_s, int lds, int nu, float tau, float grad_scale_u, int* pseudo_label,
+                       uint8_t* mask, float* dlogits_s, int lddls, int C, float lambda_u, float* stats,
+                       hipStream_t stream) {
+  if (B <= 0 || nu <= 0 || C <= 0 || C > MAXC) return ES_BAD_SHAPE;
+  if (!logits_x || !targets || !dlogits_x || !logits_w || !logits_s || !dlogits_s || !stats) return ES_BAD_ARG;
+  static std::mutex mu;
+  static hipStream_t tab[FML_SLOTS];
+  static int nslots = 0;
+  int slot = -1;
+  {
+    std::lock_guard<std::mutex> lock(mu);
+    for (int i = 0; i < nslots && slot < 0; ++i)
+      if (tab[i] == stream) slot = i;
+    if (slot < 0 && nslots < FML_SLOTS) {
+      tab[nslots] = stream;
+      slot = nslots++;
+    }
+  }
+  if (slot < 0) slot = (int)(((uintptr_t)stream >> 6) % FML_SLOTS);
+  const FMLArgs a{logits_x, targets, weights, dlogits_x, logits_w, logits_s, pseudo_label, mask, dlogits_s, stats,
+                  ldx, lddlx, ldw, lds, lddls, B, nu, C, slot, epsilon, grad_scale_x, tau, grad_scale_u, lambda_u};
+  hipLaunchKernelGGL(fixmatch_losses_kernel, 2, 256, 0, stream, a);
   return hipGetLastError() == hipSuccess ? ES_OK : ES_HIP_ERROR;
 }
 
diff --git a/endoscopy-image-classification_amd/endossl/_lib.py b/endoscopy-image-classification_amd/endossl/_lib.py
--- a/endoscopy-image-classification_amd/endossl/_lib.py
+++ b/endoscopy-image-classification_amd/endossl/_lib.py
@@ -43,6 +43,9 @@
     "es_attn_bwd": (I, [V, I, V, I, V, V, V, I, V, I, I, I, I, F, V]),
     "es_attn_cls_fwd": (I, [V, I, V, I, V, I, I, I, F, V]),
     "es_attn_cls_bwd": (I, [V, I, V, I, V, V, I, V, I, I, I, I, F, V]),
+    "es_attn_cls_bwd_kv": (I, [V, I, V, I, V, V, I, V, I, I, I, I, F, V]),
+    "es_gemm_nt_tile_rows": (I, [I, I, I, I]),
+    "es_fixmatch_losses": (I, [V, I, V, V, I, F, F, V, I, V, I, V, I, I, F, F, V, V, V, I, I, F, V, V]),
     "es_reduce_partials": (I, [V, V, I, I, I, V]),
     "es_layernorm_fwd": (I, [V, I, V, V, V, I, V, V, I, I, F, V]),
     "es_layernorm_bwd": (I, [V, I, V, I, V, V, V, V, I, V, I, V, I, V, V, V, I, I, I, I, V]),
diff --git a/endoscopy-image-classification_amd/endossl/block.py b/endoscopy-image-classification_amd/endossl/block.py
--- a/endoscopy-image-classification_amd/endossl/block.py
+++ b/endoscopy-image-classification_amd/endossl/block.py
@@ -10,9 +10,11 @@
 ATTN_SCALE = 64 ** -0.5
 
 
-def gemm_nt(call, epi, a, w, bias, c, M, N, K, c2=None, aux=None, ldc=None, ldaux=None, npatch=0, s=None):
-    call("es_gemm_nt", epi, ptr(a), a.stride(0), ptr(w), w.stride(0), ptr(bias), ptr(c), ldc or c.stride(0), ptr(c2),
-         ptr(aux), 0 if aux is None else ldaux or aux.stride(0), M, N, K, npatch, stream() if s is None else s)
+def gemm_nt(call, epi, a, w, bias, c, M, N, K, c2=None, aux=None, ldc=None, ldaux=None, npatch=0, s=None,
+            lda=None):
+    call("es_gemm_nt", epi, ptr(a), lda or a.stride(0), ptr(w), w.stride(0), ptr(bias), ptr(c), ldc or c.stride(0),
+         ptr(c2), ptr(aux), 0 if aux is None else ldaux or aux.stride(0), M, N, K, npatch,
+         stream() if s is None else s)
 
 
 def gemm_nt_resid_ln(call, a, w, bias, xmid, xin, gamma, beta, h, mean, rstd, M, N, K, eps, s=None):
@@ -50,9 +52,9 @@
          ptr(dqkv), dqkv.stride(0), n, T, H, ATTN_SCALE, stream() if s is None else s)
 
 
-def attn_cls_bwd(call, qkv, o, lse, do, dqkv, n, T, H, s=None):
-    call("es_attn_cls_bwd", ptr(qkv), qkv.stride(0), ptr(o), o.stride(0), ptr(lse), ptr(do), do.stride(0), ptr(dqkv),
-         dqkv.stride(0), n, T, H, ATTN_SCALE, stream() if s is None else s)
+def attn_cls_bwd(call, qkv, o, lse, do, dqkv, n, T, H, s=None, zero_q=True):
+    call("es_attn_cls_bwd" if zero_q else "es_attn_cls_bwd_kv", ptr(qkv), qkv.stride(0), ptr(o), o.stride(0), ptr(lse),
+         ptr(do), do.stride(0), ptr(dqkv), dqkv.stride(0), n, T, H, ATTN_SCALE, stream() if s is None else s)
 
 
 def cast_f32_bf16(call, src, dst, numel, s=None):
@@ -77,7 +79,7 @@
         self.epi_dh = EPI_BF16 if dh_bf16 else EPI_F32
         self.bracket = bracket
 
-    def attn_fwd(self, b, R, cls=None, split_q=False, ln_done=False):
+    def attn_fwd(self, b, R, cls=None, split_q=False, ln_done=False, q_strided=False):
         call, p, s, M, D = self.call, self.p, stream(), R.rows, R.h1.shape[1]
         if not ln_done:
             layernorm_fwd(call, R.x, p(b + "norm1.weight"), p(b + "norm1.bias"), R.h1, R.mean1, R.rstd1, M, D,
@@ -85,8 +87,11 @@
         w, bias = self.wb[b + "attn.qkv.weight"], p(b + "attn.qkv.bias")
         if cls is not None and split_q:
             gemm_nt(call, EPI_BF16, R.h1, w[D:], bias[D:], R.qkv[:, D:], M, 2 * D, D, s=s)
-            cls.h1[:R.n].copy_(R.h1[:M].view(R.n, R.T, D)[:, 0])
-            gemm_nt(call, EPI_BF16, cls.h1, w[:D], bias[:D], R.qkv, R.n, D, D, ldc=R.T * 3 * D, s=s)
+            if q_strided:
+                gemm_nt(call, EPI_BF16, R.h1, w[:D], bias[:D], R.qkv, R.n, D, D, ldc=R.T * 3 * D, s=s, lda=R.T * D)
+            else:
+                cls.h1[:R.n].copy_(R.h1[:M].view(R.n, R.T, D)[:, 0])
+                gemm_nt(call, EPI_BF16, cls.h1, w[:D], bias[:D], R.qkv, R.n, D, D, ldc=R.T * 3 * D, s=s)
         else:
             gemm_nt(call, EPI_BF16, R.h1, w, bias, R.qkv, M, 3 * D, D, s=s)
         Ro = R if cls is None else cls
@@ -136,14 +141,20 @@
         cap("b_dxm", R.dxm, R.dxmb)
         cap("b_do", R.do)
 
-    def attn_bwd(self, b, R, ln_bwd, wgrad=None, before_ln1=nop, cap=nop, cls=None, split_q=False):
+    def attn_bwd(self, b, R, ln_bwd, wgrad=None, before_ln1=nop, cap=nop, cls=None, split_q=False, kv_dgrad=False):
         call, p, g, s, M, T = self.call, self.p, self.g, stream(), R.rows, R.T
         D = R.dh1.shape[1]
         if cls is None:
             attn_bwd(call, R.qkv, R.o, R.lse, R.delta, R.do, R.dqkv, R.n, T, self.heads, s)
         else:
-            attn_cls_bwd(call, R.qkv, cls.o, cls.lse, cls.do, R.dqkv, R.n, T, self.heads, s)
-        gemm_nt(call, self.epi_dh, R.dqkv, self.wt[b + "attn.qkv.weight"], None, R.dh1, M, D, 3 * D, s=s)
+            attn_cls_bwd(call, R.qkv, cls.o, cls.lse, cls.do, R.dqkv, R.n, T, self.heads, s,
+                         zero_q=not (split_q and kv_dgrad))
+        wt = self.wt[b + "attn.qkv.weight"]
+        if cls is not None and split_q and kv_dgrad:
+            gemm_nt(call, self.epi_dh, R.dqkv[:, D:], wt[:, D:], None, R.dh1, M, D, 2 * D, s=s)
+            gemm_nt(call, self.epi_dh, R.dqkv, wt, None, R.dh1, R.n, D, 3 * D, ldc=T * D, s=s, lda=T * 3 * D)
+        else:
+            gemm_nt(call, self.epi_dh, R.dqkv, wt, None, R.dh1, M, D, 3 * D, s=s)
         if wgrad is not None:
             gw, gb = g(b + "attn.qkv.weight"), g(b + "attn.qkv.bias")
             if cls is not None and split_q:
diff --git a/endoscopy-image-classification_amd/endossl/fixmatch.py b/endoscopy-image-classification_amd/endossl/fixmatch.py
--- a/endoscopy-image-classification_amd/endossl/fixmatch.py
+++ b/endoscopy-image-classification_amd/endossl/fixmatch.py
@@ -68,12 +68,17 @@
             logits_w = eng.forward(m.flat, [inputs_u_w], train=False)
             logits = eng.forward(m.flat, [inputs_x, inputs_u_s], train=not frozen)
         dl = self._dlogits
-        call("es_poly_ce_fwd_bwd", ptr(logits), C, ptr(targets_x), ptr(self.class_weights), B, C, 2.0, 1.0 / B,
-             ptr(dl), C, ptr(stats[0:1]), s)
         lam = float(cfg.TRAIN.LAMBDA_U)
-        call("es_fm_consistency_fwd_bwd", ptr(logits_w), C, ptr(logits[B:]), C, nu, C, float(cfg.TRAIN.THRES),
-             lam / nu, ptr(self._pl), ptr(self._mask), None, ptr(dl[B:]), C, ptr(stats[1:3]), s)
-        torch.add(stats[0], stats[1], alpha=lam, out=stats[3])
+        if eng.CLS_TAIL:
+            call("es_fixmatch_losses", ptr(logits), C, ptr(targets_x), ptr(self.class_weights), B, 2.0, 1.0 / B,
+                 ptr(dl), C, ptr(logits_w), C, ptr(logits[B:]), C, nu, float(cfg.TRAIN.THRES), lam / nu,
+                 ptr(self._pl), ptr(self._mask), ptr(dl[B:]), C, C, lam, ptr(stats), s)
+        else:
+            call("es_poly_ce_fwd_bwd", ptr(logits), C, ptr(targets_x), ptr(self.class_weights), B, C, 2.0, 1.0 / B,
+                 ptr(dl), C, ptr(stats[0:1]), s)
+            call("es_fm_consistency_fwd_bwd", ptr(logits_w), C, ptr(logits[B:]), C, nu, C, float(cfg.TRAIN.THRES),
+                 lam / nu, ptr(self._pl), ptr(self._mask), None, ptr(dl[B:]), C, ptr(stats[1:3]), s)
+            torch.add(stats[0], stats[1], alpha=lam, out=stats[3])
         if frozen:
             eng.head_backward(m.flat, m.flat_grad, dl, train=False)
             return stats, None
diff --git a/endoscopy-image-classification_amd/endossl/vit.py b/endoscopy-image-classification_amd/endossl/vit.py
--- a/endoscopy-image-classification_amd/endossl/vit.py
+++ b/endoscopy-image-classification_amd/endossl/vit.py
@@ -269,6 +269,7 @@
     FC2_LN_MIN_M = 50000
     FC2_LN_TRAIN = True
     FC2_LN_WEAK = True
+    CLS_TAIL = os.environ.get("ENDOSSL_CLS_TAIL", "1") == "1"
 
     PARITY_NAMES = {n: n + "_f32" for n in (
         "es_gemm_nt", "es_gemm_tn", "es_attn_fwd", "es_attn_bwd", "es_attn_cls_fwd", "es_attn_cls_bwd",
@@ -428,7 +429,8 @@
                      pre=A.pre[li] if train else None, act=A.act[li], out=xout)
             if prune and i == cfg.depth - 1:
                 Rc = self._cls_rows(A, n, xin)
-                ch.attn_fwd(b, R, cls=Rc, split_q=self.PRUNE_Q, ln_done=ln_done)
+                q_strided = self.PRUNE_Q and self._cls_rows_fill(block.EPI_BF16, n, D, D)
+                ch.attn_fwd(b, R, cls=Rc, split_q=self.PRUNE_Q, ln_done=ln_done, q_strided=q_strided)
                 ch.mlp_fwd(b, Rc, train)
                 if self.capture is not None:
                     self.capture("fwd_cls", train, i, xin[:M], A.c_xout[:n])
@@ -458,6 +460,12 @@
 
     def _prune(self):
         return self.PRUNE_LAST
+
+    def _cls_rows_fill(self, epi, n, N, K):
+        if not self.CLS_TAIL or self.precision != "bf16":
+            return False
+        tile = _lib.load().es_gemm_nt_tile_rows(epi, n, N, K)
+        return tile > 0 and n % tile == 0
 
     def _cls_rows(self, A, n, xin=None, G=None):
         T, D = self.cfg.T, self.cfg.dim
@@ -595,7 +603,8 @@
                 Rc, R.dxm = self._cls_rows(A, n, G=Gi), Gi.dxm_cls
                 ch.mlp_bwd(b, Rc, ln_bwd, sched.wgrad)
                 split_q = self.PRUNE_Q and self._split_q_rows(n, _lib.tn_variant())
-                ch.attn_bwd(b, R, ln_bwd, sched.wgrad, before_ln1, cls=Rc, split_q=split_q)
+                kv_dgrad = split_q and self._cls_rows_fill(ch.epi_dh, n, D, 3 * D)
+                ch.attn_bwd(b, R, ln_bwd, sched.wgrad, before_ln1, cls=Rc, split_q=split_q, kv_dgrad=kv_dgrad)
             else:
                 ch.mlp_bwd(b, R, ln_bwd, sched.wgrad, cap, label="fc1_wgrad")
                 ch.attn_bwd(b, R, ln_bwd, sched.wgrad, before_ln1, cap)
diff --git a/include/endossl.h b/include/endossl.h
--- a/include/endossl.h
+++ b/include/endossl.h
@@ -12,6 +12,7 @@
 
 int es_gemm_nt(int epi, const void* A, int lda, const void* B, int ldb, const float* bias, void* C, int ldc,
                void* C2, const void* aux, int ldaux, int M, int N, int K, int np, hipStream_t stream);
+int es_gemm_nt_tile_rows(int epi, int M, int N, int K);
 int es_gemm_nt_resid_ln(const void* A, int lda, const void* B, int ldb, const float* bias, float* C, int ldc,
                         const float* aux, int ldaux, const float* gamma, const float* beta, void* h, int ldh,
                         float* mean, float* rstd, int M, int N, int K, float eps, hipStream_t stream);
@@ -64,6 +65,8 @@
                     hipStream_t stream);
 int es_attn_cls_bwd(const void* qkv, int ldqkv, const void* o, int ldo, const float* lse, const void* dout, int lddo,
                     void* dqkv, int lddqkv, int nimg, int T, int H, float scale, hipStream_t stream);
+int es_attn_cls_bwd_kv(const void* qkv, int ldqkv, const void* o, int ldo, const float* lse, const void* dout,
+                       int lddo, void* dqkv, int lddqkv, int nimg, int T, int H, float scale, hipStream_t stream);
 
 int es_set_ln_fwd_grid(int workgroups);
 int es_layernorm_fwd(const float* x, int ldx, const float* gamma, const float* beta, void* y, int ldy, float* mean,
@@ -186,6 +189,11 @@
                               float* dlogits_s, int lddls, float* out, hipStream_t stream);
 int es_poly_ce_fwd_bwd(const float* logits, int ldl, const int64_t* targets, const float* weights, int n, int C,
                        float epsilon, float grad_scale, float* dlogits, int lddl, float* out, hipStream_t stream);
+int es_fixmatch_losses(const float* logits_x, int ldx, const int64_t* targets, const float* weights, int B,
+                       float epsilon, float grad_scale_x, float* dlogits_x, int lddlx, const float* logits_w, int ldw,
+                       const float* logits_s, int lds, int nu, float tau, float grad_scale_u, int* pseudo_label,
+                       uint8_t* mask, float* dlogits_s, int lddls, int C, float lambda_u, float* stats,
+                       hipStream_t stream);
 
 int es_triplet_fwd_bwd(const float* z, int ldz, int bs, int L, float alpha, float grad_scale, float* dz, int lddz,
                        float* out, hipStream_t stream);
```

After: 15270 unlabeled images/s, median of 4. Within noise of the previous version (+0.2%).
